# automl/mdp-playground

Measured on AMD Instinct MI355X. Metric: env-steps/sec, higher is better.
Workload: dtype u8; 1 GPU; cfg2: BASELINE configs[1]: discrete 8x8, delay 4, sequence_length 3; 65536 envs/GPU, random actions, same-step autoreset; 1 bench step = 1 fused launch of 512 env steps; envs_per_gpu=65536, fuse=512, env_steps_per_bench_step=33554432, rng=numpy, collective=all_gather_into_tensor(nccl, 1 rank) after every launch

## Files before the change

### mdp_playground_amd/build.py

```python
import os
import subprocess
import sys
from concurrent.futures import ThreadPoolExecutor

HERE = os.path.dirname(os.path.abspath(__file__))
CSRC = os.path.join(HERE, "csrc")
OUT = os.path.join(CSRC, "libmdpp_hip.so")
SOURCES = ["mdpp_capi.hip", "mdpp_discrete.hip", "mdpp_discrete_wide.hip", "mdpp_discrete_long.hip", "mdpp_discrete_fast.hip", "mdpp_discrete_step1.hip", "mdpp_discrete_pipe.hip", "mdpp_discrete_lean.hip", "mdpp_discrete_lean_next.hip", "mdpp_discrete_lean_noise.hip", "mdpp_discrete_lean_npnoise.hip",
           "mdpp_discrete_quiet.hip", "mdpp_discrete_quiet_nu.hip", "mdpp_discrete_policy.hip", "mdpp_discrete_learn.hip",
           "mdpp_discrete_learn_pe.hip", "mdpp_discrete_learn_double.hip", "mdpp_discrete_learn_double_pe.hip",
           "mdpp_discrete_learn_summary.hip", "mdpp_discrete_learn_pe_summary.hip", "mdpp_discrete_learn_double_summary.hip",
           "mdpp_discrete_learn_double_pe_summary.hip", "mdpp_discrete_eval.hip", "mdpp_discrete_eval_summary.hip",
           "mdpp_discrete_learn_pe_nlev.hip", "mdpp_discrete_learn_double_pe_nlev.hip", "mdpp_discrete_learn_pe_nlev_summary.hip",
           "mdpp_discrete_learn_double_pe_nlev_summary.hip", "mdpp_discrete_eval_nlev.hip", "mdpp_discrete_eval_nlev_summary.hip",
           "mdpp_discrete_learn_pe_pm.hip", "mdpp_discrete_learn_double_pe_pm.hip", "mdpp_discrete_learn_pe_pm_summary.hip",
           "mdpp_discrete_learn_double_pe_pm_summary.hip", "mdpp_discrete_eval_pm.hip", "mdpp_discrete_eval_pm_summary.hip",
           "mdpp_discrete_learn_pe_pm_nlev.hip", "mdpp_discrete_learn_double_pe_pm_nlev.hip", "mdpp_discrete_learn_pe_pm_nlev_summary.hip",
           "mdpp_discrete_learn_double_pe_pm_nlev_summary.hip", "mdpp_discrete_eval_pm_nlev.hip", "mdpp_discrete_eval_pm_nlev_summary.hip",
           "mdpp_continuous.hip", "mdpp_continuous_line8.hip",
           "mdpp_continuous_fast.hip", "mdpp_continuous_step1.hip", "mdpp_continuous_line.hip", "mdpp_image.hip", "mdpp_grid.hip", "mdpp_imagec.hip", "mdpp_post.hip", "mdpp_peer.hip",
           "mdpp_generate.hip"]
HEADERS = ["mdpp_internal.hpp", "mdpp_rng.hpp", "mdpp_discrete_closed.hpp", "mdpp_pcg64_limbs.inc", "np_ziggurat_tables.inc",
           os.path.join("..", "..", "include", "mdpp.h")]
INCLUDED_SOURCES = {"mdpp_discrete_wide.hip": ["mdpp_discrete.hip"], "mdpp_discrete_long.hip": ["mdpp_discrete.hip"], "mdpp_discrete_lean_next.hip": ["mdpp_discrete_lean.hip"], "mdpp_discrete_lean_noise.hip": ["mdpp_discrete_lean.hip"], "mdpp_discrete_lean_npnoise.hip": ["mdpp_discrete_lean.hip"],
                    "mdpp_continuous_line8.hip": ["mdpp_continuous.hip"], "mdpp_continuous_step1.hip": ["mdpp_continuous_fast.hip"], "mdpp_discrete_quiet_nu.hip": ["mdpp_discrete_quiet.hip"],
                    **{u: ["mdpp_discrete_learn.hpp"] for u in SOURCES if u.startswith("mdpp_discrete_learn")},
                    **{u: ["mdpp_discrete_eval.hpp"] for u in SOURCES if u.startswith("mdpp_discrete_eval")}}
FLAGS = ["--offload-arch=gfx950", "-O3", "-fPIC", "-std=c++17", "-ffp-contract=off",
         "-fno-fast-math", "-Wall", "-Wno-unused-function"]
SPILL_SAFE = ["-mllvm", "-amdgpu-spill-sgpr-to-vgpr=0"]
EXTRA_FLAGS = {s: SPILL_SAFE for s in ("mdpp_continuous.hip", "mdpp_continuous_line8.hip", "mdpp_discrete.hip", "mdpp_discrete_wide.hip",
                                       "mdpp_discrete_long.hip", "mdpp_discrete_quiet.hip", "mdpp_discrete_quiet_nu.hip")}


def _hipcc():
    for c in (os.environ.get("HIPCC"), "/opt/rocm/bin/hipcc", "hipcc"):
        if c and (os.path.isabs(c) and os.path.exists(c) or not os.path.isabs(c)):
            return c
    raise RuntimeError("hipcc not found")


def _stale(target, deps, cmd=None):
    if not os.path.exists(target):
        return True
    t = os.path.getmtime(target)
    if any(os.path.getmtime(d) > t for d in deps):
        return True
    return cmd is not None and _stamp(target) != _cmd_text(cmd)


def _cmd_text(cmd):
    return " ".join(cmd) + "\n"


def _stamp(target):
    try:
        with open(target + ".cmd") as f:
            return f.read()
    except OSError:
        return None


def _write_stamp(target, cmd):
    with open(target + ".cmd", "w") as f:
        f.write(_cmd_text(cmd))


def build(force=False, verbose=False):
    hipcc = _hipcc()
    srcs = [s for s in SOURCES if os.path.exists(os.path.join(CSRC, s))]
    hdrs = [os.path.join(CSRC, h) for h in HEADERS]
    objs, jobs = [], []
    for s in srcs:
        src = os.path.join(CSRC, s)
        obj = os.path.join(CSRC, s.replace(".hip", ".o"))
        objs.append(obj)
        extra = [os.path.join(CSRC, d) for d in INCLUDED_SOURCES.get(s, []) if os.path.exists(os.path.join(CSRC, d))]
        cmd = [hipcc] + FLAGS + EXTRA_FLAGS.get(s, []) + ["-c", src, "-o", obj]
        if force or _stale(obj, [src] + extra + hdrs, cmd):
            jobs.append(cmd)

    def run(cmd):
        if verbose:
            print(" ".join(cmd), flush=True)
        out = cmd[cmd.index("-o") + 1]
        if os.path.exists(out + ".cmd"):
            os.remove(out + ".cmd")
        r = subprocess.run(cmd, stdout=subprocess.PIPE, stderr=subprocess.STDOUT, text=True)
        if r.returncode != 0:
            raise RuntimeError("hipcc failed:\n" + " ".join(cmd) + "\n" + r.stdout)
        _write_stamp(out, cmd)
        return r.stdout

    if jobs:
        heavy = ("mdpp_continuous_fast", "mdpp_discrete_lean", "mdpp_discrete_quiet", "mdpp_grid", "mdpp_continuous.", "mdpp_continuous_step1")
        jobs.sort(key=lambda c: next((k for k, h in enumerate(heavy) if h in c[-3]), len(heavy)))
        with ThreadPoolExecutor(max_workers=max(1, min(len(jobs), (os.cpu_count() or 4) - 1, 7))) as ex:
            for out in ex.map(run, jobs):
                if verbose and out.strip():
                    print(out)
    link = [hipcc, "--offload-arch=gfx950", "-shared", "-o", OUT] + objs
    if jobs or force or _stale(OUT, objs, link):
        run(link)
    return OUT


if __name__ == "__main__":
    print(build(force="--force" in sys.argv, verbose=True))
```

### mdp_playground_amd/csrc/mdpp_capi.hip

```cpp
#include <float.h>
#include <math.h>
#include <stdio.h>
#include <stdlib.h>
#include <string.h>
#include <time.h>

#include <algorithm>
#include <utility>
#include <vector>

#include "mdpp_internal.hpp"
#include "mdpp_rng.hpp"

using namespace mdpp;

static std::string g_create_err;

#define HIPCHK(h, expr)                                                                  \
    do {                                                                                 \
        hipError_t e_ = (expr);                                                          \
        if (e_ != hipSuccess) {                                                          \
            (h)->err = std::string(#expr) + ": " + hipGetErrorString(e_);                \
            return MDPP_EHIP;                                                            \
        }                                                                                \
    } while (0)

static int fail(mdpp_env *h, int code, const std::string &msg) {
    if (h) h->err = msg; else g_create_err = msg;
    return code;
}

static uint32_t align16(uint32_t x) { return (x + 15u) & ~15u; }

static unsigned __int128 pcg_mult_inverse() {
    static unsigned __int128 inv = 0;
    if (inv == 0) {
        const unsigned __int128 m = (((unsigned __int128)0x2360ED051FC65DA4ULL) << 64) | 0x4385DF649FCCF645ULL;
        unsigned __int128 x = m;
        for (int it = 0; it < 7; it++) x *= 2 - m * x;
        inv = x;
    }
    return inv;
}

extern "C" int mdpp_abi_version(void) { return MDPP_ABI_VERSION; }

extern "C" const char *mdpp_last_error(const mdpp_env *h) {
    return h ? h->err.c_str() : g_create_err.c_str();
}

static void free_all(mdpp_env *h) {
    void *ptrs[] = {h->d_P, h->d_rtable, h->d_rbits, h->d_is_term, h->d_init_cdf, h->d_noise_cdf,
                    h->d_state, h->d_ring, h->d_status, h->d_sd, h->d_cur, h->d_meta, h->d_rng_half,
                    h->d_P1, h->d_init_cdf1, h->d_noise_cdf1, h->d_irr_state,
                    h->d_img_tpl, h->d_img_tplp, h->d_img_clsx, h->d_img_clsy, h->d_img_rot, h->d_img_state_out,
                    h->d_img_state_final, h->d_img_rec, h->d_img_ctr, h->d_line_hist, h->d_line_ws, h->d_ring64, h->d_est_cur, h->d_est_last, h->d_tick_off,
                    h->d_img_near, h->d_s1_blob, h->d_imgc_boxes, h->d_hist_hi, h->d_policy_thr, h->d_learn_q, h->d_learn_carry,
                    h->d_learn_alpha, h->d_learn_gamma, h->d_learn_E,
                    h->d_nl_level, h->d_nl_sigma, h->d_nl_cdf, h->d_nl_T, h->d_nl_M};
    for (void *p : ptrs) if (p) (void)hipFree(p);
    for (int s = 0; s < MDPP_NUM_STREAMS; s++) {
        if (h->d_rng_s[s]) (void)hipFree(h->d_rng_s[s]);
        if (h->d_rng_inc[s]) (void)hipFree(h->d_rng_inc[s]);
    }
    if (h->ev0) (void)hipEventDestroy(h->ev0);
    if (h->side_stream) (void)hipStreamDestroy(h->side_stream);
    for (hipEvent_t e : {h->ev_entry, h->ev_side[0], h->ev_side[1], h->ev_render[0], h->ev_render[1]})
        if (e) (void)hipEventDestroy(e);
    if (h->ev1) (void)hipEventDestroy(h->ev1);
}

extern "C" void mdpp_destroy(mdpp_env *h) {
    if (!h) return;
    (void)hipSetDevice(h->device);
    free_all(h);
    delete h;
}

static int alloc_zero(mdpp_env *h, void **p, size_t bytes) {
    if (bytes == 0) bytes = 16;
    HIPCHK(h, hipMalloc(p, bytes));
    HIPCHK(h, hipMemset(*p, 0, bytes));
    return MDPP_OK;
}

extern "C" int mdpp_create(const mdpp_config *cfg, int device, mdpp_env **out) {
    if (!cfg || !out) return fail(nullptr, MDPP_EINVAL, "mdpp_create: null argument");
    if (cfg->abi_version != MDPP_ABI_VERSION)
        return fail(nullptr, MDPP_EINVAL, "mdpp_create: abi_version mismatch");
    if (cfg->num_envs <= 0) return fail(nullptr, MDPP_EINVAL, "mdpp_create: num_envs <= 0");
    if (cfg->delay < 0 || cfg->every_n < 1)
        return fail(nullptr, MDPP_EINVAL, "mdpp_create: need delay >= 0 and reward_every_n_steps >= 1");
    if (cfg->autoreset < MDPP_AUTORESET_DISABLED || cfg->autoreset > MDPP_AUTORESET_NEXT_STEP)
        return fail(nullptr, MDPP_EINVAL, "mdpp_create: unknown autoreset mode");
    hipError_t e = hipSetDevice(device);
    if (e != hipSuccess)
        return fail(nullptr, MDPP_EHIP, std::string("hipSetDevice: ") + hipGetErrorString(e));
    mdpp_env *h = new mdpp_env();
    memset(&h->cfg, 0, sizeof(h->cfg));
    h->cfg = *cfg;
    h->device = device;
    h->tick = 0; h->reset_tick = 0;
    h->opts = 0; h->kname[0] = 0;
    h->d_P = h->d_rtable = h->d_rbits = h->d_is_term = h->d_init_cdf = h->d_noise_cdf = nullptr;
    h->d_state = h->d_ring = h->d_status = h->d_sd = h->d_cur = h->d_meta = h->d_rng_half = nullptr;
    h->d_P1 = h->d_init_cdf1 = h->d_noise_cdf1 = h->d_irr_state = nullptr;
    h->d_line_hist = h->d_line_ws = h->d_ring64 = nullptr;
    h->d_est_cur = h->d_est_last = nullptr; h->est_nk = 0;
    h->irr_ready = false;
    h->line_hist_stale = false;
    h->graph_capture = false;
    h->d_tick_off = nullptr;
    h->d_img_tpl = h->d_img_tplp = h->d_img_clsx = h->d_img_clsy = h->d_img_rot = nullptr;
    h->d_img_near = nullptr;
    h->d_s1_blob = nullptr;
    memset(&h->s1args, 0, sizeof(h->s1args));
    h->d_policy_thr = nullptr; h->policy_seed = 0; h->policy_ready = false;
    h->d_learn_q = h->d_learn_carry = nullptr; h->learn_seed = 0; h->learn_E = 0; h->learn_alpha = h->learn_gamma = 0.0f;
    h->learn_algo = MDPP_LEARN_Q_LEARNING; h->learn_ready = false;
    h->learn_q_tables = 0; h->d_learn_alpha = h->d_learn_gamma = h->d_learn_E = nullptr; h->learn_pe = h->learn_pe_stale = 0;
    h->learn_pm = false;
    h->nl_on = false; h->nl_pm = false; h->nl_levels = 0; h->nl_fill_valid = false; h->nl_fill_alpha = h->nl_fill_gamma = 0.0f; h->nl_fill_E = 0;
    h->d_nl_level = h->d_nl_sigma = h->d_nl_cdf = h->d_nl_T = h->d_nl_M = nullptr;
    h->d_img_state_out = h->d_img_state_final = h->d_img_rec = h->d_img_ctr = nullptr;
    h->d_imgc_boxes = nullptr;
    h->d_hist_hi = nullptr;
    {
        const size_t imgs = (size_t)cfg->num_envs * (cfg->irrelevant ? 2 : 1);
        h->img_chunk = imgs <= 32768 ? 64 : imgs <= 65536 ? 32 : 16;
    }
    h->img_ready = false; h->img_fast_ok = false; h->img_lines_ready = false; h->img_colb = 64;
    for (int r = 0; r < 32; r++) h->imgc_disc_rows[r] = 0;
    h->img_n_radii = h->img_n_cls_x = h->img_n_cls_y = 0;
    for (int s = 0; s < MDPP_NUM_STREAMS; s++) { h->d_rng_s[s] = h->d_rng_inc[s] = nullptr; h->streams_ready[s] = false; }
    h->tables_ready = false;
    h->ev0 = h->ev1 = nullptr;
    h->side_stream = nullptr;
    h->ev_entry = h->ev_side[0] = h->ev_side[1] = h->ev_render[0] = h->ev_render[1] = nullptr;
    const size_t N = (size_t)cfg->num_envs;
    int rc = MDPP_OK;
#define TRY(x) do { rc = (x); if (rc != MDPP_OK) { g_create_err = h->err; free_all(h); delete h; return rc; } } while (0)
#define TRYHIP(x) do { hipError_t e2_ = (x); if (e2_ != hipSuccess) { g_create_err = std::string(#x) + ": " + hipGetErrorString(e2_); free_all(h); delete h; return MDPP_EHIP; } } while (0)
    TRYHIP(hipEventCreate(&h->ev0));
    TRYHIP(hipEventCreate(&h->ev1));
    TRY(alloc_zero(h, &h->d_status, N * sizeof(uint32_t)));
    TRY(alloc_zero(h, &h->d_tick_off, sizeof(uint64_t)));
    if (cfg->episode_stats) {
        h->est_nk = 3 + (cfg->kind == MDPP_KIND_CONTINUOUS ? cfg->D : 0);
        TRY(alloc_zero(h, &h->d_est_cur, (size_t)h->est_nk * N * sizeof(double)));
        TRY(alloc_zero(h, &h->d_est_last, (size_t)(h->est_nk + 1) * N * sizeof(double)));
    }
    if (cfg->rng_mode == MDPP_RNG_NUMPY_PCG64) {
        for (int s = 0; s < MDPP_NUM_STREAMS; s++) {
            if (s == MDPP_STREAM_IMAGE && !(cfg->image && cfg->kind == MDPP_KIND_DISCRETE)) continue;
            if (s == MDPP_STREAM_SPACE_IRR && !(cfg->kind == MDPP_KIND_DISCRETE && cfg->irrelevant)) continue;
            if (s == MDPP_STREAM_ACTION && cfg->kind != MDPP_KIND_GRID) continue;
            TRY(alloc_zero(h, &h->d_rng_s[s], N * 16));
            TRY(alloc_zero(h, &h->d_rng_inc[s], N * 16));
        }
        if (cfg->kind == MDPP_KIND_GRID) TRY(alloc_zero(h, &h->d_rng_half, N * 8));
        if (cfg->image && cfg->kind == MDPP_KIND_DISCRETE) TRY(alloc_zero(h, &h->d_rng_half, N * 8));
    } else if (cfg->rng_mode != MDPP_RNG_PHILOX) {
        g_create_err = "mdpp_create: unknown rng_mode"; free_all(h); delete h; return MDPP_EINVAL;
    }
    if (cfg->image && cfg->kind == MDPP_KIND_DISCRETE) {
        const size_t sub = cfg->irrelevant ? 2 : 1;
        TRY(alloc_zero(h, &h->d_img_state_out, 2 * (size_t)h->img_chunk * N * 4 * sub));
        TRY(alloc_zero(h, &h->d_img_state_final, 2 * (size_t)h->img_chunk * N * 4 * sub));
        TRY(alloc_zero(h, &h->d_img_rec, 2 * 2 * (size_t)h->img_chunk * N * 64 * sub));
        TRY(alloc_zero(h, &h->d_img_ctr, 2 * 2 * 64 * 128));
    }

    if (cfg->image && cfg->kind == MDPP_KIND_DISCRETE && (cfg->img_w < 1 || cfg->img_h < 1 || cfg->img_tpl_size < 1)) {
        g_create_err = "mdpp_create: image observations of a discrete env need img_w, img_h, img_tpl_size >= 1";
        free_all(h); delete h; return MDPP_EUNSUPPORTED;
    }
    if (cfg->image && cfg->kind == MDPP_KIND_CONTINUOUS &&
        ((cfg->D != 2 && cfg->D != 4) || !isfinite(cfg->state_space_max) || cfg->img_w < 1 || cfg->img_h < 1 ||
         cfg->img_r0 < 1 || cfg->img_r0 > 15)) {
        g_create_err = "mdpp_create: ImageContinuous observations need 2 or 4 bounded state dimensions "
                       "and a disc radius of 1..15";
        free_all(h); delete h; return MDPP_EUNSUPPORTED;
    }
    if (cfg->image) {
        {
            int lo = 0, hi = 0;
            TRYHIP(hipDeviceGetStreamPriorityRange(&lo, &hi));
            TRYHIP(hipStreamCreateWithPriority(&h->side_stream, hipStreamNonBlocking, hi));
        }
        for (hipEvent_t *e : {&h->ev_entry, &h->ev_side[0], &h->ev_side[1], &h->ev_render[0], &h->ev_render[1]})
            TRYHIP(hipEventCreateWithFlags(e, hipEventDisableTiming));
    }
    if (cfg->kind == MDPP_KIND_DISCRETE) {
        const bool wide = cfg->S > 255, lng = cfg->L > 7;
        if (cfg->S < 2 || cfg->S > 65535 || cfg->A < 1 || cfg->L < 1 || cfg->L > 15 || ((wide || lng) && cfg->image) || (wide && lng)) {
            g_create_err = "mdpp_create: discrete needs 2 <= S <= 65535, A >= 1, 1 <= L <= 15 (S <= 255 and L <= 7 with image observations; "
                           "not S > 255 together with L > 7)";
            free_all(h); delete h; return MDPP_EUNSUPPORTED;
        }
        if (cfg->has_transition_noise && cfg->S > 8192) {
            g_create_err = "mdpp_create: transition noise needs S <= 8192 (the S x S cdf table)";
            free_all(h); delete h; return MDPP_EUNSUPPORTED;
        }
        if (cfg->num_tables != 1 && cfg->num_tables != cfg->num_envs) {
            g_create_err = "mdpp_create: num_tables must be 1 or num_envs"; free_all(h); delete h; return MDPP_EINVAL;
        }
        const bool rew_sa = cfg->reward_kind == MDPP_REWARD_STATE_ACTION;
        if ((cfg->reward_kind != MDPP_REWARD_SEQUENCES && !rew_sa) || (rew_sa && cfg->unit_rewards)) {
            g_create_err = "mdpp_create: reward_kind must be MDPP_REWARD_SEQUENCES or, with unit_rewards = 0, MDPP_REWARD_STATE_ACTION";
            free_all(h); delete h; return MDPP_EINVAL;
        }
        double nk = rew_sa ? (double)cfg->S * (double)cfg->A : pow((double)cfg->S, (double)cfg->L);
        if (nk > 4.0e9) { g_create_err = "mdpp_create: S^L too large"; free_all(h); delete h; return MDPP_EUNSUPPORTED; }
        if (cfg->unit_rewards && cfg->delay > 32) {
            g_create_err = "mdpp_create: unit_rewards needs delay <= 32"; free_all(h); delete h; return MDPP_EINVAL;
        }
        h->nkeys = (uint32_t)nk;
        h->rbits_stride = (h->nkeys + 7u) / 8u;
        const size_t T = (size_t)cfg->num_tables;
        if (cfg->irrelevant) {
            if (cfg->S_irr < 2 || cfg->S_irr > 255 || cfg->A_irr < 1) {
                g_create_err = "mdpp_create: irrelevant sub-space needs 2 <= S_irr <= 255, A_irr >= 1";
                free_all(h); delete h; return MDPP_EUNSUPPORTED;
            }
            TRY(alloc_zero(h, &h->d_P1, T * cfg->S_irr * cfg->A_irr));
            TRY(alloc_zero(h, &h->d_init_cdf1, T * cfg->S_irr * sizeof(double)));
            if (cfg->has_transition_noise)
                TRY(alloc_zero(h, &h->d_noise_cdf1, (size_t)cfg->S_irr * cfg->S_irr * sizeof(double)));
            TRY(alloc_zero(h, &h->d_irr_state, N * sizeof(uint32_t)));
        }
        TRY(alloc_zero(h, &h->d_P, T * cfg->S * cfg->A * (wide ? 2 : 1)));
        if (wide || lng) {
            TRY(alloc_zero(h, &h->d_hist_hi, N * sizeof(uint64_t)));
            TRYHIP(hipMemset(h->d_hist_hi, 0xFF, N * sizeof(uint64_t)));
        }
        TRY(alloc_zero(h, &h->d_is_term, T * cfg->S));
        TRY(alloc_zero(h, &h->d_init_cdf, T * cfg->S * sizeof(double)));
        if (cfg->unit_rewards) TRY(alloc_zero(h, &h->d_rbits, T * h->rbits_stride));
        else TRY(alloc_zero(h, &h->d_rtable, T * (size_t)h->nkeys * sizeof(double)));
        if (cfg->has_transition_noise) TRY(alloc_zero(h, &h->d_noise_cdf, (size_t)cfg->S * cfg->S * sizeof(double)));
        TRY(alloc_zero(h, &h->d_state, N * sizeof(uint4)));
        if (!cfg->unit_rewards && cfg->delay > 0) {
            TRY(alloc_zero(h, &h->d_ring, (size_t)cfg->delay * N * sizeof(uint32_t)));
            TRYHIP(hipMemset(h->d_ring, 0xFF, (size_t)cfg->delay * N * sizeof(uint32_t)));
        }
        DiscreteArgs &a = h->dargs;
        memset(&a, 0, sizeof(a));
        a.N = cfg->num_envs; a.S = cfg->S; a.A = cfg->A; a.L = cfg->L; a.delay = cfg->delay;
        a.every_n = cfg->every_n; a.shared_tables = (cfg->num_tables == 1); a.unit_rewards = cfg->unit_rewards;
        a.rew_sa = rew_sa ? 1 : 0;
        a.has_p_noise = cfg->has_transition_noise; a.has_r_noise = cfg->has_reward_noise;
        a.pn_T = cfg->has_transition_noise ? philox_pnoise_threshold(cfg->transition_noise) : 0u;
        a.pn_M = philox_pnoise_magic(a.pn_T, (uint32_t)cfg->S);
        a.pn_M1 = cfg->irrelevant ? philox_pnoise_magic(a.pn_T, (uint32_t)cfg->S_irr) : 0ull;
        a.autoreset = cfg->autoreset; a.max_steps = cfg->max_episode_steps;
        a.obs_i32 = (cfg->obs_dtype == MDPP_OBS_I32 || cfg->image);
        a.philox = (cfg->rng_mode == MDPP_RNG_PHILOX);
        a.nkeys = h->nkeys; a.philox_seed = cfg->philox_seed; a.env_id_offset = cfg->env_id_offset;
        a.r_noise = cfg->reward_noise; a.scale = cfg->reward_scale; a.shift = cfg->reward_shift;
        a.term_add = cfg->term_state_reward * cfg->reward_scale;
        a.P = (const uint8_t *)h->d_P; a.rtable = (const double *)h->d_rtable;
        a.rbits = (const uint8_t *)h->d_rbits; a.is_term = (const uint8_t *)h->d_is_term;
        a.init_cdf = (const double *)h->d_init_cdf; a.noise_cdf = (const double *)h->d_noise_cdf;
        a.rbits_stride = h->rbits_stride;
        uint32_t off = 0;
        a.lds_P = off; off = align16(off + cfg->S * cfg->A);
        a.lds_term = off; off = align16(off + cfg->S);
        a.lds_init = off; off = align16(off + cfg->S * 8);
// ... 27 lines not shown
            g_create_err = "mdpp_create: move_along_a_line needs 1 <= L <= 64 and no image observations";
            free_all(h); delete h; return MDPP_EUNSUPPORTED;
        }
        const size_t D = (size_t)cfg->D;
        if (cfg->target_f64) {
            bool all_rel = !line && cfg->n_rel == cfg->D && cfg->D < 16;
            for (int j = 0; all_rel && j < cfg->n_rel; j++) all_rel = cfg->rel_idx[j] == j && cfg->target[j] == 0.0f;
            if (!all_rel) {
                g_create_err = "mdpp_create: target_f64 (the default target_point) needs move_to_a_point, every dimension relevant, state_space_dim < 16";
                free_all(h); delete h; return MDPP_EUNSUPPORTED;
            }
        }
        const bool rew64 = line || (cfg->target_f64 && cfg->make_denser);
        const bool line_big = line && (cfg->n_rel > 8 || (cfg->n_rel > 4 && cfg->D > 12));
        const size_t line_nl = line_big ? (size_t)cfg->n_rel : cfg->n_rel > 4 ? 8 : 4;
        if (line) TRY(alloc_zero(h, &h->d_line_hist, (size_t)cfg->L * line_nl * N * sizeof(float)));
        if (line_big) TRY(alloc_zero(h, &h->d_line_ws, (size_t)(2 * cfg->n_rel * cfg->n_rel + 3 * cfg->n_rel) * N * sizeof(double)));
        if (rew64 && cfg->delay > 0) TRY(alloc_zero(h, &h->d_ring64, (size_t)cfg->delay * N * sizeof(double)));
        TRY(alloc_zero(h, &h->d_sd, (size_t)(cfg->order + 1) * D * N * sizeof(float)));
        TRY(alloc_zero(h, &h->d_cur, D * N * sizeof(float)));
        TRY(alloc_zero(h, &h->d_meta, N * sizeof(uint2)));
        if (cfg->delay > 0) {
            std::vector<uint32_t> init((size_t)cfg->delay * N, kRingPyZero);
            TRY(alloc_zero(h, &h->d_ring, init.size() * sizeof(uint32_t)));
            TRYHIP(hipMemcpy(h->d_ring, init.data(), init.size() * sizeof(uint32_t), hipMemcpyHostToDevice));
        }
        ContinuousArgs &a = h->cargs;
        memset(&a, 0, sizeof(a));
        a.N = cfg->num_envs; a.D = cfg->D; a.n_rel = cfg->n_rel; a.order = cfg->order;
        a.delay = cfg->delay; a.every_n = cfg->every_n; a.make_denser = cfg->make_denser;
        a.has_p_noise = cfg->has_p_noise; a.has_r_noise = cfg->has_reward_noise;
        a.bounded = isfinite(cfg->state_space_max) ? 1 : 0;
        a.autoreset = cfg->autoreset; a.max_steps = cfg->max_episode_steps;
        a.philox = (cfg->rng_mode == MDPP_RNG_PHILOX); a.n_boxes = cfg->n_boxes;
        a.philox_seed = cfg->philox_seed; a.env_id_offset = cfg->env_id_offset;
        a.inertia32 = (float)cfg->inertia; a.amax32 = (float)cfg->action_space_max;
        a.smax32 = (float)cfg->state_space_max; a.radius32 = (float)cfg->target_radius;
        a.alw32 = (float)cfg->action_loss_weight;
        a.scale = cfg->reward_scale; a.shift = cfg->reward_shift;
        a.term_add = cfg->term_state_reward * cfg->reward_scale;
        a.scale32 = (float)a.scale; a.shift32 = (float)a.shift; a.term_add32 = (float)a.term_add;
        double f = 1.0;
        for (int k = 1; k <= cfg->order; k++) {
            f *= (double)k; a.fact[k] = f;
            a.tpow32[k] = (float)pow(cfg->time_unit, (double)k);
        }
        a.p_noise = cfg->p_noise; a.r_noise = cfg->reward_noise;
        a.reset_lo = (double)(-a.smax32); a.reset_range = (double)a.smax32 - (double)(-a.smax32);
        a.rel_prefix = 1;
        for (int j = 0; j < cfg->n_rel; j++) {
            if (cfg->rel_idx[j] < 0 || cfg->rel_idx[j] >= cfg->D) {
                g_create_err = "mdpp_create: relevant index out of range"; free_all(h); delete h; return MDPP_EINVAL;
            }
            a.rel[j] = cfg->rel_idx[j]; a.target[j] = cfg->target[j];
            if (cfg->rel_idx[j] != j) a.rel_prefix = 0;
        }
        for (int b = 0; b < cfg->n_boxes * cfg->n_rel; b++) { a.box_lo[b] = cfg->box_lo[b]; a.box_hi[b] = cfg->box_hi[b]; }
        {
            auto is_pow2 = [](double v) { int e; return v > 0 && isfinite(v) && frexp(v, &e) == 0.5; };
            a.inertia_pow2 = is_pow2((double)a.inertia32) ? 1u : 0u;
            a.inv_inertia32 = 1.0f / a.inertia32;
            a.fact_pow2_mask = 0;
            for (int k = 1; k <= cfg->order; k++) {
                a.inv_fact[k] = 1.0 / a.fact[k];
                if (is_pow2(a.fact[k])) a.fact_pow2_mask |= 1u << k;
            }
            const bool next_ok = cfg->autoreset != MDPP_AUTORESET_NEXT_STEP || cfg->rng_mode != MDPP_RNG_NUMPY_PCG64 ||
                                 (!cfg->has_p_noise && !cfg->has_reward_noise);
            const bool pen_ok = a.alw32 != 0.0f || a.amax32 <= 1.0e18f;
            a.fast_ok = (a.rel_prefix && !cfg->image && !line && !cfg->target_f64 && next_ok && cfg->n_boxes <= MDPP_MAX_BOXES && pen_ok &&
                         (a.bounded || isfinite(cfg->action_space_max))) ? 1u : 0u;
            a.image_quirk = cfg->image ? 1 : 0;
        }
        if (cfg->image) {
            TRY(alloc_zero(h, &h->d_img_state_out, 2 * (size_t)h->img_chunk * N * D * sizeof(float)));
            {
                std::vector<float> bx((size_t)(cfg->n_boxes > 0 ? cfg->n_boxes : 1) * 4, 0.0f);
                for (int b = 0; b < cfg->n_boxes; b++)
                    for (int d = 0; d < 2 && d < cfg->n_rel; d++) {
                        bx[4 * b + d] = cfg->box_lo[b * cfg->n_rel + d];
                        bx[4 * b + 2 + d] = cfg->box_hi[b * cfg->n_rel + d];
                    }
                TRY(alloc_zero(h, &h->d_imgc_boxes, bx.size() * sizeof(float)));
                TRYHIP(hipMemcpy(h->d_imgc_boxes, bx.data(), bx.size() * sizeof(float), hipMemcpyHostToDevice));
            }
            TRY(alloc_zero(h, &h->d_img_state_final, 2 * (size_t)h->img_chunk * N * D * sizeof(float)));
        }
        a.sd = (float *)h->d_sd; a.cur = (float *)h->d_cur; a.meta = (uint2 *)h->d_meta;
        a.ring = (uint32_t *)h->d_ring;
        a.line_L = line ? cfg->L : 0; a.line_NL = (int32_t)line_nl; a.line_hist = (float *)h->d_line_hist; a.line_ws = (double *)h->d_line_ws; a.ring64 = (double *)h->d_ring64;
        a.target64 = cfg->target_f64 ? 1 : 0; a.rew64 = rew64 ? 1 : 0; a.radius = cfg->target_radius;
        a.est = mdpp::EpisodeStatsDev{(double *)h->d_est_cur, (double *)h->d_est_last, h->est_nk};
        if (cfg->episode_stats) a.fast_ok = 0;
        a.env_s = (ulonglong2 *)h->d_rng_s[MDPP_STREAM_ENV]; a.env_inc = (ulonglong2 *)h->d_rng_inc[MDPP_STREAM_ENV];
        a.sp_s = (ulonglong2 *)h->d_rng_s[MDPP_STREAM_SPACE]; a.sp_inc = (ulonglong2 *)h->d_rng_inc[MDPP_STREAM_SPACE];
        a.status = (uint32_t *)h->d_status;
        h->tables_ready = true;
    } else if (cfg->kind == MDPP_KIND_GRID) {
        bool ok = (cfg->grid_dims == 2 || cfg->grid_dims == 4) && cfg->delay == 0;
        for (int d = 0; ok && d < cfg->grid_dims; d++) ok = cfg->grid_shape[d] >= 1 && cfg->grid_shape[d] <= 254;
        if (ok && cfg->image)
            ok = cfg->img_w >= 1 && cfg->img_h >= 1 &&
                 cfg->img_r0 >= 1 && cfg->img_r0 <= 15 && cfg->n_boxes >= 0 && cfg->n_boxes <= (MDPP_MAX_BOXES * MDPP_MAX_DIM) / 2;
        if (!ok) {
            g_create_err = "mdpp_create: grid needs 2 (or 4) dimensions of 1..254 cells and delay 0; with image "
                           "observations also a disc radius of 1..15 and <= 128 terminal cells";
            free_all(h); delete h; return MDPP_EUNSUPPORTED;
        }
        TRY(alloc_zero(h, &h->d_state, N * sizeof(uint4)));
        if (cfg->image) {
            TRY(alloc_zero(h, &h->d_img_state_out, 2 * (size_t)h->img_chunk * N * cfg->grid_dims * 4));
            {
                std::vector<float> bx((size_t)(cfg->n_boxes > 0 ? cfg->n_boxes : 1) * 4, 0.0f);
                for (int b = 0; b < cfg->n_boxes; b++) { bx[4 * b] = cfg->box_lo[2 * b]; bx[4 * b + 1] = cfg->box_lo[2 * b + 1]; }
                TRY(alloc_zero(h, &h->d_imgc_boxes, bx.size() * sizeof(float)));
                TRYHIP(hipMemcpy(h->d_imgc_boxes, bx.data(), bx.size() * sizeof(float), hipMemcpyHostToDevice));
            }
            TRY(alloc_zero(h, &h->d_img_state_final, 2 * (size_t)h->img_chunk * N * cfg->grid_dims * 4));
            TRY(alloc_zero(h, &h->d_img_tpl, (((size_t)(cfg->grid_dims / 2) * cfg->img_w * cfg->img_h + 15) / 16) * 2));
        }
        GridArgs &a = h->gargs;
        memset(&a, 0, sizeof(a));
        a.N = cfg->num_envs; a.G = cfg->grid_dims;
        for (int d = 0; d < cfg->grid_dims; d++) a.shape[d] = cfg->grid_shape[d];
        a.target[0] = cfg->grid_target[0]; a.target[1] = cfg->grid_target[1];
        a.make_denser = cfg->make_denser; a.has_p_noise = cfg->has_transition_noise;
        a.has_r_noise = cfg->has_reward_noise; a.every_n = cfg->every_n;
        a.autoreset = cfg->autoreset; a.max_steps = cfg->max_episode_steps;
        a.obs_i32 = (cfg->obs_dtype == MDPP_OBS_I32 || cfg->image);
        a.philox = (cfg->rng_mode == MDPP_RNG_PHILOX);
        a.philox_seed = cfg->philox_seed; a.env_id_offset = cfg->env_id_offset;
        a.p_noise = cfg->transition_noise; a.r_noise = cfg->reward_noise;
        a.scale = cfg->reward_scale; a.shift = cfg->reward_shift;
        a.term_add = cfg->term_state_reward * cfg->reward_scale;
        a.state = (uint4 *)h->d_state;
        a.env_s = (ulonglong2 *)h->d_rng_s[MDPP_STREAM_ENV]; a.env_inc = (ulonglong2 *)h->d_rng_inc[MDPP_STREAM_ENV];
        a.sp_s = (ulonglong2 *)h->d_rng_s[MDPP_STREAM_SPACE]; a.sp_inc = (ulonglong2 *)h->d_rng_inc[MDPP_STREAM_SPACE];
        a.act_s = (ulonglong2 *)h->d_rng_s[MDPP_STREAM_ACTION]; a.act_inc = (ulonglong2 *)h->d_rng_inc[MDPP_STREAM_ACTION];
        a.act_half = (uint2 *)h->d_rng_half;
        a.status = (uint32_t *)h->d_status;
        a.est = mdpp::EpisodeStatsDev{(double *)h->d_est_cur, (double *)h->d_est_last, h->est_nk};
        a.minv_lo = (uint64_t)pcg_mult_inverse(); a.minv_hi = (uint64_t)(pcg_mult_inverse() >> 64);
        h->tables_ready = true;
    } else {
        g_create_err = "mdpp_create: unknown kind"; free_all(h); delete h; return MDPP_EINVAL;
    }
#undef TRY
#undef TRYHIP
    *out = h;
    return MDPP_OK;
}

static inline bool t_fits53(uint64_t t) { return t <= (1ULL << 53) - 1; }

static int discrete_derived(mdpp_env *h, const uint8_t *P, const double *rtable, const uint8_t *rbits,
                            const uint8_t *is_term, const double *init_cdf, const double *noise_cdf) {
    const size_t T = (size_t)h->cfg.num_tables, S = (size_t)h->cfg.S, A = (size_t)h->cfg.A;
    const bool wide = S > 255;
    if (wide || h->cfg.L > 7) {
        DiscreteArgs &a = h->dargs;
        a.shape_ok = a.fast_ok = a.shape_ok_irr = a.lean_next_ok = a.shape_ok_noise = a.shape_ok_noise_np = 0u;
        a.minv_lo = (uint64_t)pcg_mult_inverse(); a.minv_hi = (uint64_t)(pcg_mult_inverse() >> 64);
        memset(&h->s1args, 0, sizeof(h->s1args));
        h->tables_ready = true;
        return MDPP_OK;
    }
    {
        DiscreteArgs &a = h->dargs;
        const mdpp_config &c = h->cfg;
        a.shape_ok = (T == 1 && c.unit_rewards && !c.has_transition_noise && !c.has_reward_noise &&
                      c.L <= 3 && c.S <= 16 && c.delay <= 32 && c.autoreset != MDPP_AUTORESET_NEXT_STEP &&
                      a.rew_in_lds && !c.irrelevant) ? 1u : 0u;
        a.fast_ok = (a.shape_ok && c.rng_mode == MDPP_RNG_NUMPY_PCG64) ? 1u : 0u;
        a.shape_ok_irr = (T == 1 && c.unit_rewards && !c.has_transition_noise && !c.has_reward_noise &&
                          c.L <= 3 && c.S <= 8 && c.delay <= 32 && c.autoreset != MDPP_AUTORESET_NEXT_STEP &&
                          a.rew_in_lds && c.irrelevant && !c.image) ? 1u : 0u;
        a.lean_next_ok = (T == 1 && c.unit_rewards && !c.has_transition_noise && !c.has_reward_noise &&
                          c.L <= 3 && c.S <= 8 && c.delay <= 32 && c.autoreset == MDPP_AUTORESET_NEXT_STEP &&
                          a.rew_in_lds && !c.image) ? 1u : 0u;
        a.shape_ok_noise = (T == 1 && c.unit_rewards && (c.has_transition_noise || c.has_reward_noise) &&
                            c.rng_mode == MDPP_RNG_PHILOX && c.L <= 3 && c.S <= 8 && c.S >= 2 && c.delay <= 32 &&
                            c.autoreset != MDPP_AUTORESET_NEXT_STEP && a.rew_in_lds && !c.irrelevant && !c.image) ? 1u : 0u;
        a.shape_ok_noise_np = (T == 1 && c.unit_rewards && (c.has_transition_noise || c.has_reward_noise) &&
                               c.rng_mode == MDPP_RNG_NUMPY_PCG64 && c.L <= 3 && c.S <= 8 && c.S >= 2 && c.delay <= 32 &&
                               c.autoreset != MDPP_AUTORESET_NEXT_STEP && a.rew_in_lds && !c.irrelevant && !c.image) ? 1u : 0u;
        for (int j = 0; j < 8; j++) a.pn_TL[j] = a.pn_TU[j] = ~0ULL;
        if (a.shape_ok_noise_np && c.has_transition_noise) {
            bool same = true;
            for (size_t j = 0; j < S; j++) {
                uint64_t tl = 0, tu = 0;
                bool hl = false, hu = false;
                for (size_t n = 0; n < S; n++) {
                    const uint64_t t = (uint64_t)ceil(ldexp(noise_cdf[n * S + j], 53));
                    if (n > j) { if (hl && tl != t) same = false; tl = t; hl = true; }
                    else { if (hu && tu != t) same = false; tu = t; hu = true; }
                }
                if (t_fits53(tl) && hl) a.pn_TL[j] = tl << 11;
                if (hu) a.pn_TU[j] = tu > (1ULL << 53) - 1 ? ~0ULL : tu << 11;
            }
            if (!same) a.shape_ok_noise_np = 0u;
        }
        if (c.episode_stats) a.shape_ok = a.fast_ok = a.shape_ok_irr = a.lean_next_ok = a.shape_ok_noise = a.shape_ok_noise_np = 0u;
        a.s_shift = 0xFFFFFFFFu;
        for (uint32_t b = 1; b < 8; b++) if ((1u << b) == (uint32_t)c.S) a.s_shift = b;
        a.key_mask = h->nkeys - 1u;
        a.spow = 1; for (int j = 0; j < c.L - 1; j++) a.spow *= (uint32_t)c.S;
        a.term_mask = 0;
        if (c.S <= 64) for (size_t s = 0; s < S; s++) if (is_term[s]) a.term_mask |= 1ULL << s;
        for (int j = 0; j < 16; j++) a.init_thr[j] = ~0ULL;
        if (c.S <= 16)
            for (size_t j = 0; j < S; j++) a.init_thr[j] = (uint64_t)ceil(ldexp(init_cdf[j], 53));
        a.minv_lo = (uint64_t)pcg_mult_inverse(); a.minv_hi = (uint64_t)(pcg_mult_inverse() >> 64);
        for (int q = 0; q < 4; q++) {
            double r = (q & 2) ? 1.0 : 0.0;
            r *= a.scale; r += a.shift;
            if (q & 1) r += a.term_add;
            a.rsel[q] = (float)r;
        }
        Step1Args &s1 = h->s1args;
        memset(&s1, 0, sizeof(s1));
        const bool rew_sa_ = c.reward_kind == MDPP_REWARD_STATE_ACTION;
        if (a.shape_ok && c.every_n < (1 << 20)) {
            std::vector<uint32_t> blob(256, 0u);
            for (size_t act = 0; act < A && act < 16; act++) {
                uint64_t col = 0;
                for (size_t st = 0; st < S; st++) col |= (uint64_t)(P[st * A + act] & 0xF) << (4 * st);
                blob[2 * act] = (uint32_t)col; blob[2 * act + 1] = (uint32_t)(col >> 32);
            }
            for (int j = 0; j < 16; j++) { blob[32 + 2 * j] = (uint32_t)a.init_thr[j]; blob[32 + 2 * j + 1] = (uint32_t)(a.init_thr[j] >> 32); }
            for (uint32_t b = 0; b < h->rbits_stride && b < 512; b++) blob[64 + b / 4] |= (uint32_t)rbits[b] << (8 * (b % 4));
            for (size_t j = 0; j < 16; j++) {
                const double t = j < S ? ceil(ldexp(init_cdf[j], 31)) : 4294967295.0;
                blob[192 + j] = t >= 4294967295.0 ? 4294967295u : (uint32_t)t;
            }
            if (h->d_s1_blob) { (void)hipFree(h->d_s1_blob); h->d_s1_blob = nullptr; }
            HIPCHK(h, hipMalloc(&h->d_s1_blob, (size_t)kS1Replicas * 1024));
            for (int r = 0; r < kS1Replicas; r++)
                HIPCHK(h, hipMemcpy((char *)h->d_s1_blob + (size_t)r * 1024, blob.data(), 1024, hipMemcpyHostToDevice));
            s1.N = c.num_envs; s1.A = (uint32_t)c.A; s1.S = (uint32_t)c.S; s1.L = (uint32_t)c.L;
            s1.every_n = (uint32_t)c.every_n; s1.inv_every_n = 1.0 / (double)c.every_n;
            s1.max_steps = c.max_episode_steps > 0 ? (uint32_t)c.max_episode_steps : 0u;
            s1.delay = (uint32_t)c.delay; s1.autoreset = c.autoreset != MDPP_AUTORESET_DISABLED ? 1u : 0u;
            s1.term32 = (uint32_t)a.term_mask; s1.nan_mask = 0xFFu << (8 * c.L);
            s1.topup_rounds = 1; s1.topup_fill = 6;
            s1.philox_seed = a.philox_seed; s1.env_id_offset = a.env_id_offset;
            for (int q = 0; q < 4; q++) s1.rsel[q] = a.rsel[q];
            s1.blob = (const uint4 *)h->d_s1_blob;
            s1.state = a.state; s1.env_s = a.env_s; s1.env_inc = a.env_inc; s1.status = a.status;
        } else if (T == 1 && (c.unit_rewards ? c.delay <= 32 : (!rew_sa_ && !c.has_transition_noise && !c.has_reward_noise)) && c.L <= 3 &&
                   c.autoreset != MDPP_AUTORESET_NEXT_STEP && !c.irrelevant && !c.episode_stats && c.every_n < (1 << 20)) {
            const uint32_t S8 = ((uint32_t)S + 7u) & ~7u;
            const uint32_t off_term = align16((uint32_t)(S * A)), off_thr = align16(off_term + (uint32_t)S);
            const uint32_t off_thr31 = off_thr + S8 * 8u, off_rew = align16(off_thr31 + S8 * 4u);
            const uint32_t rew_bytes = c.unit_rewards ? h->rbits_stride : h->nkeys * 8u;
            const uint32_t off_bk = align16(off_rew + rew_bytes);
            const bool np_streams = c.rng_mode == MDPP_RNG_NUMPY_PCG64;
            const uint32_t off_tn = off_bk + 512u;
            const uint32_t off_zig = off_tn + ((c.has_transition_noise && np_streams) ? (uint32_t)S * S8 * 8u : 0u);
            const uint32_t bytes = (off_zig + ((c.has_reward_noise && np_streams) ? 6144u : 0u) + 1023u) & ~1023u;
            const uint32_t max_rounds = (c.has_transition_noise || c.has_reward_noise) ? kS1wRoundsNoise : kS1wRounds;
            if (bytes <= max_rounds * 1024u) {
                std::vector<uint8_t> blob(bytes, 0);
                memcpy(blob.data(), P, S * A);
                memcpy(blob.data() + off_term, is_term, S);
                for (uint32_t j = 0; j < S8; j++) {
                    const uint64_t t64 = j < S ? (uint64_t)ceil(ldexp(init_cdf[j], 53)) : ~0ULL;
                    const double t31 = j < S ? ceil(ldexp(init_cdf[j], 31)) : 4294967295.0;
                    const uint32_t t32 = t31 >= 4294967295.0 ? 4294967295u : (uint32_t)t31;
                    memcpy(blob.data() + off_thr + 8u * j, &t64, 8);
                    memcpy(blob.data() + off_thr31 + 4u * j, &t32, 4);
                }
                if (c.unit_rewards) memcpy(blob.data() + off_rew, rbits, h->rbits_stride);
                else memcpy(blob.data() + off_rew, rtable, (size_t)h->nkeys * 8u);
                {
                    const bool ph = c.rng_mode == MDPP_RNG_PHILOX;
                    const int shift = ph ? 23 : 45;
                    for (uint32_t b = 0; b < 256u; b++) {
                        const uint64_t lo = (uint64_t)b << shift, hi = lo + (1ULL << shift);
                        uint32_t c0 = 0, nin = 0;
                        for (uint32_t j = 0; j < S; j++) {
                            uint64_t t;
                            if (ph) { uint32_t t32; memcpy(&t32, blob.data() + off_thr31 + 4u * j, 4); t = t32; }
                            else memcpy(&t, blob.data() + off_thr + 8u * j, 8);
                            c0 += t <= lo ? 1u : 0u;
                            nin += (t > lo && t < hi) ? 1u : 0u;
                        }
                        const uint16_t e = (uint16_t)(c0 | (nin << 8));
                        memcpy(blob.data() + off_bk + 2u * b, &e, 2);
                    }
                }
                if (c.has_transition_noise && np_streams)
                    for (uint32_t row = 0; row < S; row++)
                        for (uint32_t j = 0; j < S8; j++) {
                            const uint64_t t64 = j < S ? (uint64_t)ceil(ldexp(noise_cdf[row * S + j], 53)) : ~0ULL;
                            memcpy(blob.data() + off_tn + 8u * (row * S8 + j), &t64, 8);
                        }
                if (c.has_reward_noise && np_streams) {
                    static const uint64_t ki[256] = NPZ_KI_INIT;
                    static const double wi[256] = NPZ_WI_INIT, fi[256] = NPZ_FI_INIT;
                    memcpy(blob.data() + off_zig, ki, 2048); memcpy(blob.data() + off_zig + 2048, wi, 2048);
                    memcpy(blob.data() + off_zig + 4096, fi, 2048);
                }
                if (h->d_s1_blob) { (void)hipFree(h->d_s1_blob); h->d_s1_blob = nullptr; }
                HIPCHK(h, hipMalloc(&h->d_s1_blob, (size_t)kS1Replicas * bytes));
                for (int r = 0; r < kS1Replicas; r++)
                    HIPCHK(h, hipMemcpy((char *)h->d_s1_blob + (size_t)r * bytes, blob.data(), bytes, hipMemcpyHostToDevice));
                s1.N = c.num_envs; s1.A = (uint32_t)c.A; s1.S = (uint32_t)c.S; s1.L = (uint32_t)c.L;
                s1.every_n = (uint32_t)c.every_n; s1.inv_every_n = 1.0 / (double)c.every_n;
                s1.max_steps = c.max_episode_steps > 0 ? (uint32_t)c.max_episode_steps : 0u;
                s1.delay = (uint32_t)c.delay; s1.autoreset = c.autoreset != MDPP_AUTORESET_DISABLED ? 1u : 0u;
                s1.nan_mask = 0xFFu << (8 * c.L);
                s1.philox_seed = a.philox_seed; s1.env_id_offset = a.env_id_offset;
                for (int q = 0; q < 4; q++) s1.rsel[q] = a.rsel[q];
                s1.blob = (const uint4 *)h->d_s1_blob;
                s1.wide = 1; s1.blob_rounds = bytes / 1024u; s1.off_term = off_term; s1.off_thr = off_thr; s1.off_thr31 = off_thr31;
                s1.off_rew = off_rew; s1.S8 = S8; s1.off_bk = off_bk;
                s1.has_p_noise = c.has_transition_noise ? 1u : 0u; s1.has_r_noise = c.has_reward_noise ? 1u : 0u;
                s1.off_tn = off_tn; s1.off_zig = off_zig; s1.pn_T = a.pn_T; s1.pn_M = a.pn_M; s1.r_noise = a.r_noise;
                s1.sp_s = a.sp_s; s1.sp_inc = a.sp_inc;
                s1.unit = c.unit_rewards ? 1u : 0u; s1.ring_keys = a.ring_keys;
                s1.scale = a.scale; s1.shift = a.shift; s1.term_add = a.term_add;
                s1.state = a.state; s1.env_s = a.env_s; s1.env_inc = a.env_inc; s1.status = a.status;
            }
        }
    }
    h->tables_ready = true;
    return MDPP_OK;
}

extern "C" int mdpp_upload_discrete_tables(mdpp_env *h, const uint8_t *P, const double *rtable,
                                           const uint8_t *rbits, const uint8_t *is_term,
                                           const double *init_cdf, const double *noise_cdf) {
    if (!h) return MDPP_EINVAL;
    if (h->cfg.kind != MDPP_KIND_DISCRETE) return fail(h, MDPP_EINVAL, "upload_discrete_tables: not a discrete handle");
    if (!P || !is_term || !init_cdf) return fail(h, MDPP_EINVAL, "upload_discrete_tables: null table");
    if (h->cfg.unit_rewards ? !rbits : !rtable) return fail(h, MDPP_EINVAL, "upload_discrete_tables: reward table missing");
    if (h->cfg.has_transition_noise && !noise_cdf) return fail(h, MDPP_EINVAL, "upload_discrete_tables: noise_cdf missing");
    HIPCHK(h, hipSetDevice(h->device));
    const size_t T = (size_t)h->cfg.num_tables, S = (size_t)h->cfg.S, A = (size_t)h->cfg.A;
    const bool wide = S > 255;
    for (size_t k = 0; k < T * S * A; k++)
        if ((wide ? (size_t)((const uint16_t *)P)[k] : (size_t)P[k]) >= S) return fail(h, MDPP_EINVAL, "upload_discrete_tables: P entry out of range");
    HIPCHK(h, hipMemcpy(h->d_P, P, T * S * A * (wide ? 2 : 1), hipMemcpyHostToDevice));
    HIPCHK(h, hipMemcpy(h->d_is_term, is_term, T * S, hipMemcpyHostToDevice));
    HIPCHK(h, hipMemcpy(h->d_init_cdf, init_cdf, T * S * sizeof(double), hipMemcpyHostToDevice));
    if (h->cfg.unit_rewards)
        HIPCHK(h, hipMemcpy(h->d_rbits, rbits, T * h->rbits_stride, hipMemcpyHostToDevice));
    else
        HIPCHK(h, hipMemcpy(h->d_rtable, rtable, T * (size_t)h->nkeys * sizeof(double), hipMemcpyHostToDevice));
    if (h->cfg.has_transition_noise)
        HIPCHK(h, hipMemcpy(h->d_noise_cdf, noise_cdf, S * S * sizeof(double), hipMemcpyHostToDevice));
    return discrete_derived(h, P, rtable, rbits, is_term, init_cdf, noise_cdf);
}

struct DevTemp {
    std::vector<void *> ptrs;
    ~DevTemp() { for (void *p : ptrs) (void)hipFree(p); }
    hipError_t alloc(void **p, size_t bytes) {
        hipError_t e = hipMalloc(p, bytes ? bytes : 16);
        if (e == hipSuccess) ptrs.push_back(*p);
        return e;
    }
};

extern "C" int mdpp_generate_discrete(mdpp_env *h, const uint64_t *seeds, const mdpp_gen_params *p,
                                      const uint8_t *is_term, const double *init_cdf, const double *noise_cdf) {
    if (!h) return MDPP_EINVAL;
    const mdpp_config &c = h->cfg;
    if (c.kind != MDPP_KIND_DISCRETE) return fail(h, MDPP_EINVAL, "generate_discrete: not a discrete handle");
    if (!seeds || !p || !is_term || !init_cdf) return fail(h, MDPP_EINVAL, "generate_discrete: null argument");
    if (c.has_transition_noise && !noise_cdf) return fail(h, MDPP_EINVAL, "generate_discrete: noise_cdf missing");
    if (c.num_tables != c.num_envs || c.irrelevant || c.S > 255 || c.reward_kind != MDPP_REWARD_SEQUENCES)
        return fail(h, MDPP_EUNSUPPORTED, "generate_discrete: needs one table per env, no irrelevant sub-space, S <= 255 and "
                                          "rewardable sequences");
    GenArgs a;
    const char *err = nullptr;
    const int prc = gen_args_init(p, c.S, c.A, c.L, c.image != 0, c.unit_rewards != 0, h->nkeys, h->rbits_stride, a, &err);
    if (prc != MDPP_OK) return fail(h, prc, err);
    const size_t per_env = (size_t)a.scratch_words * 8u;
    HIPCHK(h, hipSetDevice(h->device));
    const size_t N = (size_t)c.num_envs, S = (size_t)c.S, A = (size_t)c.A;
    const int chunk = (int)std::min(N, std::max<size_t>(1, kGenScratchCap / std::max<size_t>(per_env, 8)));
    DevTemp tmp;
    uint64_t *d_seeds = nullptr, *d_sd = nullptr, *d_scr = nullptr;
    double *d_rews = nullptr;
    HIPCHK(h, tmp.alloc((void **)&d_seeds, N * 8));
    HIPCHK(h, hipMemcpy(d_seeds, seeds, N * 8, hipMemcpyHostToDevice));
    if (p->rews) {
        HIPCHK(h, tmp.alloc((void **)&d_rews, (size_t)p->n_rews * 8));
        HIPCHK(h, hipMemcpy(d_rews, p->rews, (size_t)p->n_rews * 8, hipMemcpyHostToDevice));
    }
    if (p->seed_dicts) HIPCHK(h, tmp.alloc((void **)&d_sd, N * 64));
    HIPCHK(h, tmp.alloc((void **)&d_scr, (size_t)chunk * per_env));
    HIPCHK(h, hipMemset(h->d_P, 0, N * S * A));
    if (c.unit_rewards) HIPCHK(h, hipMemset(h->d_rbits, 0, N * h->rbits_stride));
    else HIPCHK(h, hipMemset(h->d_rtable, 0, N * (size_t)h->nkeys * sizeof(double)));
    a.rews = d_rews;
    a.seeds = d_seeds; a.P = (uint8_t *)h->d_P; a.rbits = (uint8_t *)h->d_rbits; a.rtable = (double *)h->d_rtable;
    a.sd = d_sd;
    if (c.rng_mode == MDPP_RNG_NUMPY_PCG64) {
        a.env_s = (ulonglong2 *)h->d_rng_s[MDPP_STREAM_ENV]; a.env_inc = (ulonglong2 *)h->d_rng_inc[MDPP_STREAM_ENV];
        a.sp_s = (ulonglong2 *)h->d_rng_s[MDPP_STREAM_SPACE]; a.sp_inc = (ulonglong2 *)h->d_rng_inc[MDPP_STREAM_SPACE];
        if (c.image) {
            a.im_s = (ulonglong2 *)h->d_rng_s[MDPP_STREAM_IMAGE]; a.im_inc = (ulonglong2 *)h->d_rng_inc[MDPP_STREAM_IMAGE];
            a.im_half = (uint2 *)h->d_rng_half;
        }
    }
    a.scratch = d_scr;
    for (size_t first = 0; first < N; first += (size_t)chunk)
        HIPCHK(h, launch_generate_discrete(a, (int)first, (int)std::min((size_t)chunk, N - first)));
    HIPCHK(h, hipDeviceSynchronize());
    if (p->seed_dicts) HIPCHK(h, hipMemcpy(p->seed_dicts, d_sd, N * 64, hipMemcpyDeviceToHost));
    {
        std::vector<uint8_t> term(N * S);
        std::vector<double> cdf(N * S);
        for (size_t i = 0; i < N; i++) {
            memcpy(term.data() + i * S, is_term, S);
            memcpy(cdf.data() + i * S, init_cdf, S * sizeof(double));
        }
        HIPCHK(h, hipMemcpy(h->d_is_term, term.data(), N * S, hipMemcpyHostToDevice));
        HIPCHK(h, hipMemcpy(h->d_init_cdf, cdf.data(), N * S * sizeof(double), hipMemcpyHostToDevice));
    }
    if (c.has_transition_noise)
        HIPCHK(h, hipMemcpy(h->d_noise_cdf, noise_cdf, S * S * sizeof(double), hipMemcpyHostToDevice));
    int rc;
    if (N == 1) {
        std::vector<uint8_t> P(S * A), rbits(c.unit_rewards ? h->rbits_stride : 0);
        std::vector<double> rtable(c.unit_rewards ? 0 : h->nkeys);
        HIPCHK(h, hipMemcpy(P.data(), h->d_P, S * A, hipMemcpyDeviceToHost));
        if (c.unit_rewards) HIPCHK(h, hipMemcpy(rbits.data(), h->d_rbits, h->rbits_stride, hipMemcpyDeviceToHost));
        else HIPCHK(h, hipMemcpy(rtable.data(), h->d_rtable, (size_t)h->nkeys * sizeof(double), hipMemcpyDeviceToHost));
        rc = discrete_derived(h, P.data(), c.unit_rewards ? nullptr : rtable.data(), c.unit_rewards ? rbits.data() : nullptr,
                              is_term, init_cdf, noise_cdf);
    } else {
        rc = discrete_derived(h, nullptr, nullptr, nullptr, is_term, init_cdf, noise_cdf);
    }
    if (rc != MDPP_OK) return rc;
    if (c.rng_mode == MDPP_RNG_NUMPY_PCG64) {
        if (h->dargs.fast_ok)
            HIPCHK(h, hipMemset2D((char *)h->d_state + 4, 16, 0, 4, N));
        h->streams_ready[MDPP_STREAM_ENV] = h->streams_ready[MDPP_STREAM_SPACE] = true;
        if (c.image) h->streams_ready[MDPP_STREAM_IMAGE] = true;
    }
    return MDPP_OK;
}

extern "C" int mdpp_get_discrete_tables(mdpp_env *h, uint8_t *P, double *rtable, uint8_t *rbits, uint8_t *is_term,
                                        double *init_cdf) {
    if (!h) return MDPP_EINVAL;
    if (h->cfg.kind != MDPP_KIND_DISCRETE) return fail(h, MDPP_EINVAL, "get_discrete_tables: not a discrete handle");
    if (!h->tables_ready) return fail(h, MDPP_ESTATE, "get_discrete_tables: tables not uploaded");
    if ((rtable && !h->d_rtable) || (rbits && !h->d_rbits))
        return fail(h, MDPP_EINVAL, "get_discrete_tables: this handle keeps the other reward table (unit_rewards)");
    HIPCHK(h, hipSetDevice(h->device));
    HIPCHK(h, hipDeviceSynchronize());
    const size_t T = (size_t)h->cfg.num_tables, S = (size_t)h->cfg.S, A = (size_t)h->cfg.A;
    if (P) HIPCHK(h, hipMemcpy(P, h->d_P, T * S * A * (S > 255 ? 2 : 1), hipMemcpyDeviceToHost));
    if (rtable) HIPCHK(h, hipMemcpy(rtable, h->d_rtable, T * (size_t)h->nkeys * sizeof(double), hipMemcpyDeviceToHost));
    if (rbits) HIPCHK(h, hipMemcpy(rbits, h->d_rbits, T * h->rbits_stride, hipMemcpyDeviceToHost));
    if (is_term) HIPCHK(h, hipMemcpy(is_term, h->d_is_term, T * S, hipMemcpyDeviceToHost));
    if (init_cdf) HIPCHK(h, hipMemcpy(init_cdf, h->d_init_cdf, T * S * sizeof(double), hipMemcpyDeviceToHost));
    return MDPP_OK;
}

extern "C" int mdpp_seed_streams_seedseq(mdpp_env *h, int stream, const uint64_t *seeds) {
    if (!h || !seeds) return MDPP_EINVAL;
    if (h->cfg.rng_mode != MDPP_RNG_NUMPY_PCG64) return fail(h, MDPP_ESTATE, "seed_streams_seedseq: handle is in Philox mode");
    if (stream < 0 || stream >= MDPP_NUM_STREAMS || !h->d_rng_s[stream]) return fail(h, MDPP_EINVAL, "seed_streams_seedseq: bad stream");
    HIPCHK(h, hipSetDevice(h->device));
    const size_t N = (size_t)h->cfg.num_envs;
    DevTemp tmp;
    uint64_t *d_seeds = nullptr;
    HIPCHK(h, tmp.alloc((void **)&d_seeds, N * 8));
    HIPCHK(h, hipMemcpy(d_seeds, seeds, N * 8, hipMemcpyHostToDevice));
    const bool half = (stream == MDPP_STREAM_IMAGE || stream == MDPP_STREAM_ACTION) && h->d_rng_half;
    HIPCHK(h, hipDeviceSynchronize());
    HIPCHK(h, launch_seed_streams_seedseq(d_seeds, (int)N, h->d_rng_s[stream], h->d_rng_inc[stream], half ? h->d_rng_half : nullptr));
    if (stream == MDPP_STREAM_ENV && h->cfg.kind == MDPP_KIND_DISCRETE && h->dargs.fast_ok)
        HIPCHK(h, hipMemset2D((char *)h->d_state + 4, 16, 0, 4, N));
    HIPCHK(h, hipDeviceSynchronize());
    h->streams_ready[stream] = true;
    return MDPP_OK;
}

extern "C" int mdpp_upload_discrete_irrelevant(mdpp_env *h, const uint8_t *P1, const double *init_cdf1,
                                               const double *noise_cdf1) {
    if (!h) return MDPP_EINVAL;
    if (h->cfg.kind != MDPP_KIND_DISCRETE || !h->cfg.irrelevant)
        return fail(h, MDPP_EINVAL, "upload_discrete_irrelevant: not a handle with an irrelevant sub-space");
    if (!P1 || !init_cdf1) return fail(h, MDPP_EINVAL, "upload_discrete_irrelevant: null table");
    if (h->cfg.has_transition_noise && !noise_cdf1) return fail(h, MDPP_EINVAL, "upload_discrete_irrelevant: noise_cdf missing");
    HIPCHK(h, hipSetDevice(h->device));
    const size_t T = (size_t)h->cfg.num_tables, S1 = (size_t)h->cfg.S_irr, A1 = (size_t)h->cfg.A_irr;
    for (size_t k = 0; k < T * S1 * A1; k++)
        if (P1[k] >= S1) return fail(h, MDPP_EINVAL, "upload_discrete_irrelevant: P entry out of range");
    HIPCHK(h, hipMemcpy(h->d_P1, P1, T * S1 * A1, hipMemcpyHostToDevice));
    HIPCHK(h, hipMemcpy(h->d_init_cdf1, init_cdf1, T * S1 * sizeof(double), hipMemcpyHostToDevice));
    if (h->cfg.has_transition_noise)
        HIPCHK(h, hipMemcpy(h->d_noise_cdf1, noise_cdf1, S1 * S1 * sizeof(double), hipMemcpyHostToDevice));
    h->irr_ready = true;
    return MDPP_OK;
}

extern "C" int mdpp_upload_image_disc(mdpp_env *h, const uint8_t *disc) {
    if (!h || !disc) return MDPP_EINVAL;
    if ((h->cfg.kind != MDPP_KIND_CONTINUOUS && h->cfg.kind != MDPP_KIND_GRID) || !h->cfg.image)
        return fail(h, MDPP_EINVAL, "upload_image_disc: not a continuous / grid handle with image observations");
    const int T = 2 * h->cfg.img_r0 + 1;
    for (int r = 0; r < 32; r++) h->imgc_disc_rows[r] = 0;
    for (int dy = 0; dy < T; dy++)
        for (int dx = 0; dx < T; dx++)
            if (disc[dy * T + dx]) h->imgc_disc_rows[dy] |= 1u << dx;
    h->img_ready = h->cfg.kind == MDPP_KIND_CONTINUOUS || h->img_lines_ready;
    return MDPP_OK;
}

extern "C" int mdpp_upload_image_lines(mdpp_env *h, const uint8_t *lines) {
    if (!h || !lines) return MDPP_EINVAL;
    if (h->cfg.kind != MDPP_KIND_GRID || !h->cfg.image)
        return fail(h, MDPP_EINVAL, "upload_image_lines: not a grid handle with image observations");
    const size_t npix = (size_t)(h->cfg.grid_dims / 2) * h->cfg.img_w * h->cfg.img_h;
    std::vector<uint16_t> bits((npix + 15) / 16, 0);
    for (size_t p = 0; p < npix; p++)
        if (lines[p]) bits[p >> 4] |= (uint16_t)(1u << (p & 15));
    HIPCHK(h, hipSetDevice(h->device));
    HIPCHK(h, hipMemcpy(h->d_img_tpl, bits.data(), bits.size() * 2, hipMemcpyHostToDevice));
    h->img_lines_ready = true;
    bool disc = false;
    for (int r = 0; r < 32; r++) disc = disc || h->imgc_disc_rows[r] != 0;
    h->img_ready = disc;
    return MDPP_OK;
}

extern "C" int mdpp_get_state_grid(mdpp_env *h, int32_t *cells, int32_t *steps, uint8_t *reached) {
    if (!h || !cells || !steps || !reached) return MDPP_EINVAL;
    if (h->cfg.kind != MDPP_KIND_GRID) return fail(h, MDPP_EINVAL, "get_state_grid: not a grid handle");
    HIPCHK(h, hipSetDevice(h->device));
    HIPCHK(h, hipDeviceSynchronize());
    const size_t N = (size_t)h->cfg.num_envs;
    const int G = h->cfg.grid_dims;
    std::vector<uint32_t> st(4 * N);
    HIPCHK(h, hipMemcpy(st.data(), h->d_state, N * 16, hipMemcpyDeviceToHost));
    for (size_t i = 0; i < N; i++) {
        for (int d = 0; d < G; d++) cells[i * G + d] = (int32_t)((st[4 * i] >> (8 * d)) & 0xFF);
        steps[i] = (int32_t)st[4 * i + 1];
        reached[i] = (uint8_t)(st[4 * i + 2] & 1u);
    }
    return MDPP_OK;
}

extern "C" int mdpp_set_state_grid(mdpp_env *h, const int32_t *cells, const int32_t *steps, const uint8_t *reached) {
    if (!h || !cells || !steps) return MDPP_EINVAL;
    if (h->cfg.kind != MDPP_KIND_GRID) return fail(h, MDPP_EINVAL, "set_state_grid: not a grid handle");
    const size_t N = (size_t)h->cfg.num_envs;
    const int G = h->cfg.grid_dims;
    std::vector<uint32_t> st(4 * N, 0);
    for (size_t i = 0; i < N; i++) {
        for (int d = 0; d < G; d++) {
            if (cells[i * G + d] < 0 || cells[i * G + d] > h->cfg.grid_shape[d])
                return fail(h, MDPP_EINVAL, "set_state_grid: cell out of range");
            st[4 * i] |= (uint32_t)cells[i * G + d] << (8 * d);
        }
        st[4 * i + 1] = (uint32_t)steps[i];
        st[4 * i + 2] = reached ? (uint32_t)(reached[i] & 1u) : 0u;
    }
    HIPCHK(h, hipSetDevice(h->device));
    HIPCHK(h, hipDeviceSynchronize());
    HIPCHK(h, hipMemcpy(h->d_state, st.data(), N * 16, hipMemcpyHostToDevice));
    return MDPP_OK;
}

extern "C" int mdpp_get_state_irrelevant(mdpp_env *h, int32_t *irr) {
    if (!h || !irr) return MDPP_EINVAL;
    if (h->cfg.kind != MDPP_KIND_DISCRETE || !h->cfg.irrelevant) return fail(h, MDPP_EINVAL, "get_state_irrelevant: no irrelevant sub-space");
    HIPCHK(h, hipSetDevice(h->device));
    HIPCHK(h, hipDeviceSynchronize());
    HIPCHK(h, hipMemcpy(irr, h->d_irr_state, (size_t)h->cfg.num_envs * 4, hipMemcpyDeviceToHost));
    return MDPP_OK;
}

extern "C" int mdpp_set_state_irrelevant(mdpp_env *h, const int32_t *irr) {
    if (!h || !irr) return MDPP_EINVAL;
    if (h->cfg.kind != MDPP_KIND_DISCRETE || !h->cfg.irrelevant) return fail(h, MDPP_EINVAL, "set_state_irrelevant: no irrelevant sub-space");
    for (int i = 0; i < h->cfg.num_envs; i++)
        if (irr[i] < 0 || irr[i] >= h->cfg.S_irr) return fail(h, MDPP_EINVAL, "set_state_irrelevant: state out of range");
    HIPCHK(h, hipSetDevice(h->device));
    HIPCHK(h, hipDeviceSynchronize());
    HIPCHK(h, hipMemcpy(h->d_irr_state, irr, (size_t)h->cfg.num_envs * 4, hipMemcpyHostToDevice));
    return MDPP_OK;
}

extern "C" int mdpp_seed_streams(mdpp_env *h, int stream, const uint64_t *words) {
    if (!h || !words) return MDPP_EINVAL;
    if (h->cfg.rng_mode != MDPP_RNG_NUMPY_PCG64) return fail(h, MDPP_ESTATE, "seed_streams: handle is in Philox mode");
    if (stream < 0 || stream >= MDPP_NUM_STREAMS || !h->d_rng_s[stream]) return fail(h, MDPP_EINVAL, "seed_streams: bad stream");
    HIPCHK(h, hipSetDevice(h->device));
    const size_t N = (size_t)h->cfg.num_envs;
    std::vector<uint64_t> st(2 * N), inc(2 * N);
    std::vector<uint32_t> half(2 * N);
    for (size_t i = 0; i < N; i++) {
        st[2 * i] = words[6 * i]; st[2 * i + 1] = words[6 * i + 1];
        inc[2 * i] = words[6 * i + 2]; inc[2 * i + 1] = words[6 * i + 3];
        half[2 * i] = (uint32_t)words[6 * i + 4]; half[2 * i + 1] = (uint32_t)words[6 * i + 5];
    }
    HIPCHK(h, hipMemcpy(h->d_rng_s[stream], st.data(), N * 16, hipMemcpyHostToDevice));
    HIPCHK(h, hipMemcpy(h->d_rng_inc[stream], inc.data(), N * 16, hipMemcpyHostToDevice));
    if ((stream == MDPP_STREAM_IMAGE || stream == MDPP_STREAM_ACTION) && h->d_rng_half)
        HIPCHK(h, hipMemcpy(h->d_rng_half, half.data(), N * 8, hipMemcpyHostToDevice));
    if (stream == MDPP_STREAM_ENV && h->cfg.kind == MDPP_KIND_DISCRETE && h->dargs.fast_ok) {
        HIPCHK(h, hipDeviceSynchronize());
        HIPCHK(h, hipMemset2D((char *)h->d_state + 4, 16, 0, 4, N));
    }
    h->streams_ready[stream] = true;
    return MDPP_OK;
}

extern "C" int mdpp_get_streams(mdpp_env *h, int stream, uint64_t *words) {
    if (!h || !words) return MDPP_EINVAL;
    if (h->cfg.rng_mode != MDPP_RNG_NUMPY_PCG64) return fail(h, MDPP_ESTATE, "get_streams: handle is in Philox mode");
    if (stream < 0 || stream >= MDPP_NUM_STREAMS || !h->d_rng_s[stream]) return fail(h, MDPP_EINVAL, "get_streams: bad stream");
    HIPCHK(h, hipSetDevice(h->device));
    HIPCHK(h, hipDeviceSynchronize());
    const size_t N = (size_t)h->cfg.num_envs;
    std::vector<uint64_t> st(2 * N), inc(2 * N);
    std::vector<uint32_t> half(2 * N, 0);
    HIPCHK(h, hipMemcpy(st.data(), h->d_rng_s[stream], N * 16, hipMemcpyDeviceToHost));
    HIPCHK(h, hipMemcpy(inc.data(), h->d_rng_inc[stream], N * 16, hipMemcpyDeviceToHost));
    if ((stream == MDPP_STREAM_IMAGE || stream == MDPP_STREAM_ACTION) && h->d_rng_half)
        HIPCHK(h, hipMemcpy(half.data(), h->d_rng_half, N * 8, hipMemcpyDeviceToHost));
    std::vector<uint32_t> rec;
    const bool queued = stream == MDPP_STREAM_ENV && h->cfg.kind == MDPP_KIND_DISCRETE && h->dargs.fast_ok;
    if (queued) {
        rec.resize(4 * N);
        HIPCHK(h, hipMemcpy(rec.data(), h->d_state, N * 16, hipMemcpyDeviceToHost));
    }
    for (size_t i = 0; i < N; i++) {
        unsigned __int128 s = ((unsigned __int128)st[2 * i + 1] << 64) | st[2 * i];
        const unsigned __int128 c = ((unsigned __int128)inc[2 * i + 1] << 64) | inc[2 * i];
        if (queued)
            for (uint32_t q = (rec[4 * i + 1] >> 24) & 7u; q > 0; q--) s = (s - c) * pcg_mult_inverse();
        words[6 * i] = (uint64_t)s; words[6 * i + 1] = (uint64_t)(s >> 64);
        words[6 * i + 2] = inc[2 * i]; words[6 * i + 3] = inc[2 * i + 1];
        words[6 * i + 4] = half[2 * i]; words[6 * i + 5] = half[2 * i + 1];
    }
    return MDPP_OK;
}

extern "C" int mdpp_set_options(mdpp_env *h, uint32_t disable_mask) {
    if (!h) return MDPP_EINVAL;
    h->opts = disable_mask;
    return MDPP_OK;
}

extern "C" int mdpp_get_episode_stats(mdpp_env *h, double *current, double *last) {
// ... 1148 lines not shown
```

### mdp_playground_amd/csrc/mdpp_discrete_lean.hip

```cpp
#include <stdlib.h>

#include <stdio.h>

#include <type_traits>

#ifndef MDPP_LEAN_TU_NEXT
#define MDPP_LEAN_TU_NEXT 0
#endif
#ifndef MDPP_LEAN_TU_NOISE
#define MDPP_LEAN_TU_NOISE 0
#endif

#include "mdpp_internal.hpp"
#include "mdpp_rng.hpp"

namespace mdpp {

#ifndef MDPP_LEAN_CHUNK
#define MDPP_LEAN_CHUNK 8
#endif
#ifndef MDPP_LEAN_DEPTH
#define MDPP_LEAN_DEPTH 32
#endif
#ifndef MDPP_LEAN_AHEAD
#define MDPP_LEAN_AHEAD 4
#endif
#if defined(MDPP_LEAN_PRIO_E) || defined(MDPP_LEAN_PRIO_O) || defined(MDPP_LEAN_PRIO_H)
#define MDPP_LEAN_PRIO_FORCED 1
#else
#define MDPP_LEAN_PRIO_FORCED 0
#endif
#ifndef MDPP_LEAN_PRIO_E
#define MDPP_LEAN_PRIO_E 3
#endif
#ifndef MDPP_LEAN_PRIO_O
#define MDPP_LEAN_PRIO_O 2
#endif
#ifndef MDPP_LEAN_PRIO_H
#define MDPP_LEAN_PRIO_H 0
#endif
#ifndef MDPP_LEAN_PRIO_O2
#define MDPP_LEAN_PRIO_O2 -1
#endif
#ifndef MDPP_LEAN_ST_AUX
#define MDPP_LEAN_ST_AUX MDPP_ST_NT
#endif
#ifndef MDPP_LEAN_ST_AUX_BYTES
#define MDPP_LEAN_ST_AUX_BYTES MDPP_LEAN_ST_AUX
#endif
#ifndef MDPP_LEAN_LD_AUX
#define MDPP_LEAN_LD_AUX 0
#endif
#ifndef MDPP_LEAN_HMIN
#define MDPP_LEAN_HMIN 16
#endif
#ifndef MDPP_LEAN_HSLEEP
#define MDPP_LEAN_HSLEEP 8
#endif
namespace lean {
constexpr int kChunk = MDPP_LEAN_CHUNK;
constexpr int kDepth = MDPP_LEAN_DEPTH;
constexpr int kAhead = MDPP_LEAN_AHEAD;
constexpr int kPRsrc = 0x00020000;
constexpr uint32_t kSpinLimit = 1u << 22;
constexpr uint32_t kStatusInternal = 0x80000000u;
constexpr uint32_t kQueueCap = 6;
constexpr int kHChunks = 8;
constexpr int kHChunksNp = 4;
constexpr int kXR = 16;
constexpr int kXB = 4;
constexpr int kDepthNp = 16;
constexpr int kRoles = 4;
constexpr uint32_t kSelPad = 0x0c0c0c00u;
typedef unsigned int u32x2 __attribute__((ext_vector_type(2)));
typedef unsigned int u32x4 __attribute__((ext_vector_type(4)));

__device__ __forceinline__ uint32_t wg_load_acq(const uint32_t *p) {
    return __hip_atomic_load(p, __ATOMIC_ACQUIRE, __HIP_MEMORY_SCOPE_WORKGROUP);
}
__device__ __forceinline__ void wg_store_rel(uint32_t *p, uint32_t v) {
    __hip_atomic_store(p, v, __ATOMIC_RELEASE, __HIP_MEMORY_SCOPE_WORKGROUP);
}
__device__ __forceinline__ void chunk_words(uint64_t seed, uint64_t genv, uint64_t b0, uint32_t r4, uint32_t stream,
                                            uint32_t (&wd)[MDPP_LEAN_CHUNK]) {
    uint32_t o0[4], o1[4], o2[4] = {0u, 0u, 0u, 0u};
    philox_start_block(seed, genv, b0, stream, o0);
    philox_start_block(seed, genv, b0 + 1, stream, o1);
    if (r4 != 0u) philox_start_block(seed, genv, b0 + 2, stream, o2);
    const uint32_t all[12] = {o0[0], o0[1], o0[2], o0[3], o1[0], o1[1], o1[2], o1[3], o2[0], o2[1], o2[2], o2[3]};
#pragma unroll
    for (int u = 0; u < MDPP_LEAN_CHUNK; u++)
        wd[u] = r4 == 0u ? all[u] : r4 == 1u ? all[u + 1] : r4 == 2u ? all[u + 2] : all[u + 3];
}
__device__ __forceinline__ void chunk_normals(uint64_t seed, uint64_t genv, uint64_t b0, uint32_t r4, uint32_t stream,
                                              float (&z)[MDPP_LEAN_CHUNK]) {
    float all[12] = {0.0f, 0.0f, 0.0f, 0.0f, 0.0f, 0.0f, 0.0f, 0.0f, 0.0f, 0.0f, 0.0f, 0.0f};
    uint32_t o[4];
    philox_start_block(seed, genv, b0, stream, o);
    philox_box_muller2(o, all[0], all[1], all[2], all[3]);
    philox_start_block(seed, genv, b0 + 1, stream, o);
    philox_box_muller2(o, all[4], all[5], all[6], all[7]);
    if (r4 != 0u) {
        philox_start_block(seed, genv, b0 + 2, stream, o);
        philox_box_muller2(o, all[8], all[9], all[10], all[11]);
    }
#pragma unroll
    for (int u = 0; u < MDPP_LEAN_CHUNK; u++)
        z[u] = r4 == 0u ? all[u] : r4 == 1u ? all[u + 1] : r4 == 2u ? all[u + 2] : all[u + 3];
}
}
using namespace lean;

template <bool OBS64, bool DELAY, bool HASMAX, bool EVN, bool PHILOX, bool IRR, bool NEXT, int NZ = 0>
__global__ __launch_bounds__(kRoles * kBlock) void k_discrete_rollout_lean(DiscreteArgs a, int K,
                                                                      const int32_t *__restrict__ actions,
                                                                      void *__restrict__ obs,
                                                                      float *__restrict__ reward,
                                                                      uint8_t *__restrict__ term,
                                                                      uint8_t *__restrict__ trunc,
                                                                      void *__restrict__ final_obs) {
    const uint64_t ptick0 = tick_now(a);
    constexpr bool PN = (NZ & 1) != 0, RN = (NZ & 2) != 0;
    constexpr bool NPN = PN && !PHILOX, NRN = RN && !PHILOX;
    constexpr bool Z0 = (NZ & 4) != 0;
    static_assert(!Z0 || NRN, "sigma-0 draws: numpy streams with the reward_noise key");
    constexpr bool NRX = NRN && !Z0;
    constexpr int KD = NRN ? kDepthNp : kDepth;
    __shared__ __align__(16) uint32_t lds_rec[3][KD][kBlock];
    __shared__ __align__(16) uint32_t lds_V[2048];
    __shared__ __align__(16) uint2 lds_col[16];
    __shared__ __align__(16) uint32_t lds_R[128];
    __shared__ __align__(16) uint64_t lds_T[8];
    __shared__ __align__(16) float lds_rsel[EVN ? 4 * 64 : 4];
    __shared__ __align__(16) uint64_t lds_ring[kBlock];
    __shared__ uint32_t lds_head[kBlock];
    __shared__ uint32_t lds_prod[kBlock / 64];
    __shared__ __align__(8) uint32_t lds_cons[kBlock / 64][2];
    __shared__ uint32_t lds_done;
    constexpr bool ROWS2 = !IRR && NZ == 0;
    constexpr bool ROWS1 = ROWS2 && !PHILOX;
    constexpr int kRB = 4;
    __shared__ __align__(16) float lds_rw[ROWS1 ? kRB : 1][kChunk][ROWS1 ? kBlock : 4];
    __shared__ __align__(16) uint32_t lds_rprod[kBlock / 64], lds_rcons[kBlock / 64];
    typedef typename std::conditional<IRR, uint64_t, uint32_t>::type S0Word;
    __shared__ __align__(16) S0Word lds_s0[PHILOX ? kHChunks : 1][kBlock];
    __shared__ __align__(16) uint2 lds_col1[IRR ? 16 : 1];
    __shared__ __align__(16) uint64_t lds_T1[IRR ? 8 : 1];
    __shared__ uint32_t lds_hprod[kBlock / 64];
    __shared__ uint32_t lds_pprod[kBlock / 64];
    constexpr bool kNpNoise = !PHILOX && NZ != 0;
    constexpr bool kPhNoise = PHILOX && NZ != 0;
    constexpr int kPrioE = MDPP_LEAN_PRIO_FORCED ? MDPP_LEAN_PRIO_E : kNpNoise ? 2 : !PHILOX ? MDPP_LEAN_PRIO_E : 1;
    constexpr int kPrioO = MDPP_LEAN_PRIO_FORCED ? MDPP_LEAN_PRIO_O : kNpNoise ? 1 : !PHILOX ? MDPP_LEAN_PRIO_O : kPhNoise ? 2 : (PN ? 2 : 3);
    constexpr int kPrioH = MDPP_LEAN_PRIO_FORCED ? MDPP_LEAN_PRIO_H : kNpNoise ? 3 : !PHILOX ? MDPP_LEAN_PRIO_H : kPhNoise ? 2 : (PN ? 3 : 2);
    static_assert(NZ == 0 || (!IRR && !NEXT), "noise on the lean kernel: one sub-space, same-step autoreset");
    __shared__ __align__(16) uint32_t lds_pn[(PN && PHILOX) ? kHChunks : 1][kBlock];
    __shared__ __align__(16) uint32_t lds_pn2[NPN ? kHChunksNp : 1][2][kBlock];
    __shared__ __align__(16) double lds_x[NRX ? kXR : 1][kBlock];
    __shared__ uint16_t lds_meta[NRN ? kXR : 1][kBlock];
    __shared__ __align__(16) double lds_rx[NRX ? KD : 1][kBlock];
    __shared__ uint32_t lds_hhead[NRN ? kBlock : 1], lds_epos[NRN ? kBlock : 1];
    __shared__ uint8_t lds_sstab[(NRN || NPN) ? 2048 : 1];
    __shared__ uint8_t lds_pntab[NPN ? 4096 : 1];
    __shared__ ulonglong2 lds_kw[NRN ? 256 : 1];
    __shared__ double lds_fi[NRN ? 256 : 1];
    constexpr int kEN = IRR ? 2 : 1;
    constexpr bool nextmode = NEXT;
    const bool ar = a.autoreset != 0;
    const int tid = threadIdx.x;
    const int role = tid / kBlock;
    const int l = tid & (kBlock - 1);
    const int w = l >> 6;
    const uint32_t S = (uint32_t)a.S, L = (uint32_t)a.L;
    if (tid < 16) {
        uint64_t cs = 0;
        if (tid < a.A)
            for (uint32_t s = 0; s < S; s++) {
                const uint32_t nx = a.P[s * a.A + tid] & 7u;
                cs |= (uint64_t)(nx | 8u | ((uint32_t)((a.term_mask >> nx) & 1ULL) << 7)) << (8 * s);
            }
        lds_col[tid] = make_uint2((uint32_t)cs, (uint32_t)(cs >> 32));
        if (tid < 8) lds_T[tid] = a.init_thr[tid];
        if (IRR) {
            uint64_t c1 = 0;
            if (tid < a.A1)
                for (int s1 = 0; s1 < a.S1; s1++) c1 |= (uint64_t)(a.P1[s1 * a.A1 + tid] & 7u) << (8 * s1);
            lds_col1[tid] = make_uint2((uint32_t)c1, (uint32_t)(c1 >> 32));
            if (tid < 8) lds_T1[tid] = tid < a.S1 ? (uint64_t)ceil(a.init_cdf1[tid] * 9007199254740992.0) : ~0ULL;
        }
        if (!EVN && tid < 4) lds_rsel[tid] = a.rsel[tid];
    }
    if (EVN)
        for (int k = tid; k < 4 * a.every_n; k += kRoles * kBlock) lds_rsel[k] = a.rsel[k < 4 ? k : (k & 1)];
    for (uint32_t k = tid; k < 128; k += kRoles * kBlock) {
        uint32_t wd = 0;
        for (int b = 0; b < 4; b++) {
            uint32_t byte = 4 * k + b;
            if (byte < a.rbits_stride) wd |= (uint32_t)a.rbits[byte] << (8 * b);
        }
        lds_R[k] = wd;
    }
    if (tid < kBlock) { lds_ring[tid] = 0; lds_head[tid] = 0; if (NRN) { lds_hhead[tid] = 0; lds_epos[tid] = 0; } }
    if (NRN || NPN) {
        for (uint32_t k = tid; k < 2048u; k += kRoles * kBlock) {
            const uint64_t lo = (uint64_t)k << 53, hi = lo + ((1ULL << 53) - 1ULL);
            uint32_t c0 = 0, c1 = 0;
            for (int j = 0; j < 8; j++) {
                const uint64_t t = a.init_thr[j] > (1ULL << 53) - 1ULL ? ~0ULL : a.init_thr[j] << 11;
                c0 += (t <= lo) ? 1u : 0u; c1 += (t <= hi) ? 1u : 0u;
            }
            lds_sstab[k] = (uint8_t)(c0 == c1 ? c0 : 0xFFu);
        }
    }
    if (NPN) {
        for (uint32_t k = tid; k < 4096u; k += kRoles * kBlock) {
            const uint64_t lo = (uint64_t)k << 52, hi = lo + ((1ULL << 52) - 1ULL);
            uint32_t a0 = 0, a1 = 0, b0 = 0, b1 = 0;
            for (int j = 0; j < 7; j++) { a0 += (a.pn_TL[j] <= lo) ? 1u : 0u; a1 += (a.pn_TL[j] <= hi) ? 1u : 0u; }
            for (int j = 0; j < 8; j++) { b0 += (a.pn_TU[j] <= lo) ? 1u : 0u; b1 += (a.pn_TU[j] <= hi) ? 1u : 0u; }
            lds_pntab[k] = (uint8_t)((a0 == a1 && b0 == b1) ? (a0 | (b0 << 4)) : 0xFFu);
        }
    }
    if (NRN)
        for (int k = tid; k < 256; k += kRoles * kBlock) { lds_kw[k] = make_ulonglong2(d_zig_ki[k], (unsigned long long)(__double_as_longlong(d_zig_wi[k]) + (52LL << 52)));    lds_fi[k] = d_zig_fi[k]; }
    if (tid < kBlock / 64) { lds_prod[tid] = 0; lds_cons[tid][0] = 0; lds_cons[tid][1] = 0; lds_hprod[tid] = 0; lds_pprod[tid] = 0; lds_rprod[tid] = 0; lds_rcons[tid] = 0; }
    if (tid == 0) lds_done = 0;
    __syncthreads();
    {
        uint32_t dmask = 0;
        for (uint32_t j = 1; j <= L; j++) dmask |= 1u << (4 * j - 2);
        for (uint32_t d = tid; d < 2048; d += kRoles * kBlock) {
            uint32_t wd = 0;
            if ((d & dmask) == dmask) {
                for (uint32_t b = 8; b < 32; b++) {
                    if (!(b & 8u)) continue;
                    const uint32_t idx = d * 32u + b;
                    uint32_t key = 0, pw = 1;
                    for (uint32_t j = 0; j < L; j++) { key += ((idx >> (4 * j)) & 7u) * pw; pw *= S; }
                    if (key < a.nkeys) wd |= ((lds_R[key >> 5] >> (key & 31u)) & 1u) << b;
                }
            }
            lds_V[d] = wd;
        }
    }
    uint32_t steps_at_launch = 0;
    {
        const uint32_t eb0 = ((gridDim.x & 7u) == 0u) ? (blockIdx.x & 7u) * (gridDim.x >> 3) + (blockIdx.x >> 3) : blockIdx.x;
        const uint32_t i0 = eb0 * kBlock + l;
        if (EVN && role == 1 && i0 < (uint32_t)a.N) steps_at_launch = ((const uint32_t *)&a.state[i0])[2] & 0x7FFFFFFFu;
    }
    __syncthreads();

    const uint32_t eblk = ((gridDim.x & 7u) == 0u) ? (blockIdx.x & 7u) * (gridDim.x >> 3) + (blockIdx.x >> 3) : blockIdx.x;
    const uint32_t i = eblk * kBlock + l;
    const uint32_t N = (uint32_t)a.N;
    const bool rows = ROWS2 && (N % (uint32_t)kBlock) == 0u;
    const uint32_t blk0 = eblk * kBlock, ln = (uint32_t)l & 63u;
    const uint32_t ws = (uint32_t)__builtin_amdgcn_readfirstlane(w);
    auto min4 = [&](const uint32_t *p) -> uint32_t {
        const uint64_t x = __hip_atomic_load((const uint64_t *)p, __ATOMIC_ACQUIRE, __HIP_MEMORY_SCOPE_WORKGROUP);
        const uint64_t y = __hip_atomic_load((const uint64_t *)p + 1, __ATOMIC_ACQUIRE, __HIP_MEMORY_SCOPE_WORKGROUP);
        return min(min((uint32_t)x, (uint32_t)(x >> 32)), min((uint32_t)y, (uint32_t)(y >> 32)));
    };
    if (i >= N) {
        if (role == 0 && (l & 63) == 0) __hip_atomic_fetch_add(&lds_done, 1u, __ATOMIC_RELEASE, __HIP_MEMORY_SCOPE_WORKGROUP);
        return;
    }
    const uint32_t A = (uint32_t)a.A;
    constexpr int kMinLanes = MDPP_LEAN_HMIN;
    uint32_t status = 0;

    if (role == 3) {
        if (!ar && !PN && !NRN) return;
        __builtin_amdgcn_s_setprio(kPrioH);
        if constexpr (PHILOX) {
            const uint64_t genv = (uint64_t)(a.env_id_offset + (int64_t)i);
            const int nch = (K + kChunk - 1) / kChunk;
            static_assert(kChunk == 8, "two start-state blocks per chunk");
            uint32_t thr[8], thr1[8];
#pragma unroll
            for (int j = 0; j < 8; j++) {
                const uint64_t t53 = lds_T[j];
                thr[j] = __builtin_amdgcn_readfirstlane(t53 > (1ULL << 53) ? 0x80000000u : (uint32_t)((t53 + 0x3FFFFFULL) >> 22));
                const uint64_t u53 = IRR ? lds_T1[j] : ~0ULL;
                thr1[j] = __builtin_amdgcn_readfirstlane(u53 > (1ULL << 53) ? 0x80000000u : (uint32_t)((u53 + 0x3FFFFFULL) >> 22));
            }
            const uint32_t r4 = (uint32_t)ptick0 & 3u;
            for (int c = 0; c < nch; c++) {
                if (c >= kHChunks) {
                    const uint32_t must = (uint32_t)min((c - kHChunks + 1) * kChunk, K);
                    uint32_t spins = 0;
                    while (wg_load_acq(&lds_prod[w]) < must) {
                        __builtin_amdgcn_s_sleep(2);
                        if (++spins > kSpinLimit) { status |= kStatusInternal; break; }
                    }
                }
                const uint64_t b0 = (ptick0 + (uint64_t)(c * kChunk)) >> 2;
                auto words = [&](uint32_t stream, uint32_t (&wd)[kChunk]) { chunk_words(a.philox_seed, genv, b0, r4, stream, wd); };
                uint32_t wd[kChunk], wd1[kChunk];
                words(kPhiloxStartStream, wd);
                if (IRR) words(kPhiloxStartIrrStream, wd1);
                S0Word pk = 0;
#pragma unroll
                for (int u = 0; u < kChunk; u++) {
                    const uint32_t m = wd[u] >> 1;
                    uint32_t s0 = 0;
#pragma unroll
                    for (int j = 0; j < 7; j++) s0 += (thr[j] <= m) ? 1u : 0u;
                    if (IRR) {
                        const uint32_t m1 = wd1[u] >> 1;
                        uint32_t s1 = 0;
#pragma unroll
                        for (int j = 0; j < 7; j++) s1 += (thr1[j] <= m1) ? 1u : 0u;
                        s0 |= (s1 | 8u) << 4;
                    }
                    pk |= (S0Word)(s0 | 8u) << (kEN * 4 * u);
                }
                lds_s0[c % kHChunks][l] = pk;
                if ((l & 63) == 0) wg_store_rel(&lds_hprod[w], (uint32_t)(c + 1));
            }
            if (status) atomicOr(&a.status[i], status);
            return;
        }
        if constexpr (NPN || NRN) {
            Pcg64 g;
            g.load(a.env_s, a.env_inc, i);
            Pcg64LimbsLo ge;
            ge.from(g);
            uint32_t hq = 0;
            uint64_t look = 0;
            if (NRN) look = ge.next64();
            uint32_t vals = 0, tail = 0, spins = 0;
            auto start_of = [&](uint64_t r) __attribute__((always_inline)) -> uint32_t {
                uint32_t s0 = lds_sstab[(uint32_t)(r >> 53)];
                if (__builtin_expect(__builtin_amdgcn_ballot_w64(s0 == 0xFFu) != 0, 0)) {
                    if (s0 == 0xFFu) {
                        const uint64_t m = r >> 11;
                        s0 = 0;
#pragma unroll
                        for (int j = 0; j < 8; j++) s0 += (a.init_thr[j] <= m) ? 1u : 0u;
                    }
                }
                return s0;
            };
            for (;;) {
                if (wg_load_acq(&lds_done) == kBlock / 64) break;
                bool did = false;
                if constexpr (NRN) {
                    const uint32_t epos = __hip_atomic_load(&lds_epos[l], __ATOMIC_RELAXED, __HIP_MEMORY_SCOPE_WORKGROUP);
                    const bool go = hq + (uint32_t)kXB <= epos + (uint32_t)kXR;
                    if (__builtin_amdgcn_ballot_w64(go) != 0) {
                        uint32_t rej = 0;
                        uint64_t wdv[kXB + 1];
                        if (go) {
                            wdv[0] = look;
#pragma unroll
                            for (int u = 0; u < kXB; u++) {
                                const uint64_t wd = wdv[u];
                                wdv[u + 1] = ge.next64();
                                const uint64_t rabs = (wd >> 9) & 0x000fffffffffffffULL;
                                if constexpr (Z0) {
                                    const uint64_t ki = lds_kw[(uint32_t)wd & 0xffu].x;
                                    const bool ok = rabs < ki;
                                    rej |= ok ? 0u : (1u << u);
                                    lds_meta[(hq + (uint32_t)u) & (uint32_t)(kXR - 1)][l] = (uint16_t)(start_of(wd) | (ok ? 0u : (2u << 3)));
                                    continue;
                                }
                                const ulonglong2 kw = lds_kw[(uint32_t)wd & 0xffu];
                                const double W = __longlong_as_double((long long)kw.y);
                                const double x = __builtin_fma(__longlong_as_double((long long)(rabs | 0x3FF0000000000000ULL)), W, -W);
                                const uint64_t xb = (uint64_t)__double_as_longlong(x);
                                const double xs = __longlong_as_double((long long)(((uint64_t)(((uint32_t)(xb >> 32) & 0x7FFFFFFFu) |
                                                                                   (((uint32_t)wd << 23) & 0x80000000u)) << 32) | (uint32_t)xb));
                                const bool ok = rabs < kw.x;
                                rej |= ok ? 0u : (1u << u);
                                const uint32_t slot = (hq + (uint32_t)u) & (uint32_t)(kXR - 1);
                                lds_x[slot][l] = xs;
                                lds_meta[slot][l] = (uint16_t)(start_of(wd) | (ok ? 0u : (2u << 3)));
                            }
                            look = wdv[kXB];
                        }
                        while (__builtin_amdgcn_ballot_w64(rej != 0u) != 0) {
                            if (rej != 0u) {
                                const uint32_t j = (uint32_t)__builtin_ctz(rej);
                                rej &= rej - 1u;
                                uint64_t wd = 0, wn = 0;
#pragma unroll
                                for (int u = 0; u < kXB; u++)
                                    if (j == (uint32_t)u) { wd = wdv[u]; wn = wdv[u + 1]; }
                                const uint32_t idx = (uint32_t)wd & 0xffu;
                                const uint32_t slot = (hq + j) & (uint32_t)(kXR - 1);
                                const uint32_t ss = lds_meta[slot][l] & 7u;
                                if (__builtin_expect(idx == 0u, 0)) {
                                    const double nor_r = 3.6541528853610087963519472518, nor_inv_r = 0.27366123732975827203338247596;
                                    Pcg64LimbsLo t = ge;
                                    uint32_t have = (uint32_t)kXB - j, cnt = 1u;
                                    auto word = [&]() -> uint64_t {
                                        uint64_t r = 0;
                                        if (have != 0u) {
#pragma unroll
                                            for (int u = 1; u <= kXB; u++) if ((uint32_t)kXB - have + 1u == (uint32_t)u) r = wdv[u];
                                            have -= 1u;
                                        } else {
                                            r = t.next64();
                                        }
                                        cnt += 1u;
                                        return r;
                                    };
                                    double val = 0.0;
                                    for (;;) {
                                        const double u1 = (double)(word() >> 11) * (1.0 / 9007199254740992.0);
                                        const double u2 = (double)(word() >> 11) * (1.0 / 9007199254740992.0);
                                        const double xx = -nor_inv_r * log1p(-u1);
                                        const double yy = -log1p(-u2);
                                        if (yy + yy > xx * xx) { val = ((wd >> 17) & 0x1) ? -(nor_r + xx) : nor_r + xx; break; }
                                        if (cnt > 250u) { status |= kStatusInternal; break; }
                                    }
                                    if constexpr (!Z0) lds_x[slot][l] = val;
                                    const uint32_t words = cnt, ssb = start_of(word());
                                    lds_meta[slot][l] = (uint16_t)(ss | (3u << 3) | (ssb << 5) | (words << 8));
                                } else {
                                    double x;
                                    if constexpr (Z0) {
                                        const double W = __longlong_as_double((long long)lds_kw[idx].y);
                                        x = __builtin_fma(__longlong_as_double((long long)(((wd >> 9) & 0x000fffffffffffffULL) | 0x3FF0000000000000ULL)), W, -W);
                                    } else {
                                        x = lds_x[slot][l];
                                    }
                                    const double u1 = (double)(wn >> 11) * (1.0 / 9007199254740992.0);
                                    const double y = (lds_fi[idx - 1] - lds_fi[idx]) * u1 + lds_fi[idx];
                                    const double e = (double)__builtin_amdgcn_exp2f((float)(x * x * -0.72134752044448170368));
                                    bool acc = y < e;
                                    if (__builtin_expect(!(fabs(y - e) > 1.0e-5 * e), 0)) acc = y < exp(-0.5 * x * x);
                                    lds_meta[slot][l] = (uint16_t)(ss | ((acc ? 1u : 2u) << 3));
                                }
                            }
                        }
                        if (go) hq += (uint32_t)kXB;
                        __hip_atomic_store(&lds_hhead[l], hq, __ATOMIC_RELEASE, __HIP_MEMORY_SCOPE_WORKGROUP);
                        did = true;
                    }
                } else if (ar) {
                    const uint32_t head = wg_load_acq(&lds_head[l]);
                    const uint32_t cnt = tail - head;
                    const bool want = cnt + 1u <= 8u;
                    const uint64_t bw = __builtin_amdgcn_ballot_w64(want);
                    const bool urgent = __builtin_amdgcn_ballot_w64(want && cnt <= 2) != 0;
                    if (__builtin_popcountll(bw) >= kMinLanes || urgent) {
                        Pcg64LimbsLo n = ge;
                        const uint32_t s0 = start_of(n.next64()) | 8u;
                        if (want) {
                            const uint32_t sh = (tail & 7u) * 4u;
                            ge = n;
                            vals = (vals & ~(0xFu << sh)) | (s0 << sh);
                            tail += 1u;
                        }
                        __hip_atomic_store(&lds_ring[l], (uint64_t)vals | ((uint64_t)tail << 32), __ATOMIC_RELEASE,
                                           __HIP_MEMORY_SCOPE_WORKGROUP);
                        did = true;
                    }
                }
                if (__builtin_amdgcn_ballot_w64(did) == 0) {
                    __builtin_amdgcn_s_sleep(2);
                    if (++spins > kSpinLimit * 4u) { status |= kStatusInternal; break; }
                } else {
                    spins = 0;
                }
            }
            auto undraw = [&](Pcg64 &gg, uint32_t q) {
                for (; q > 0; q--) {
                    uint64_t lo = gg.s_lo - gg.inc_lo;
                    uint64_t hi = gg.s_hi - gg.inc_hi - (gg.s_lo < gg.inc_lo ? 1ULL : 0ULL);
                    gg.s_lo = lo * a.minv_lo;
                    gg.s_hi = __umul64hi(lo, a.minv_lo) + lo * a.minv_hi + hi * a.minv_lo;
                }
            };
            ge.to(g);
            if (NRN) undraw(g, hq + 1u - __hip_atomic_load(&lds_epos[l], __ATOMIC_ACQUIRE, __HIP_MEMORY_SCOPE_WORKGROUP));
            else undraw(g, tail - wg_load_acq(&lds_head[l]));
            g.store(a.env_s, i);
            if (status) atomicOr(&a.status[i], status);
            return;
        }
        Pcg64 g;
        g.load(a.env_s, a.env_inc, i);
        auto draw = [&](Pcg64 &gg) -> uint32_t {
            const uint64_t r0 = gg.next64();
            const uint64_t m = r0 >> 11;
            uint32_t s0 = 0;
#pragma unroll
            for (int j = 0; j < 8; j++) s0 += (lds_T[j] <= m) ? 1u : 0u;
            if (IRR) {
                const uint64_t m1 = gg.next64() >> 11;
                uint32_t s1 = 0;
#pragma unroll
                for (int j = 0; j < 8; j++) s1 += (lds_T1[j] <= m1) ? 1u : 0u;
                s0 |= (s1 | 8u) << 4;
            }
            return s0;
        };
        uint32_t vals = 0, tail = 0;
        for (;;) {
            if (wg_load_acq(&lds_done) == kBlock / 64) break;
            const uint32_t head = wg_load_acq(&lds_head[l]);
            const uint32_t cnt = tail - head;
            const bool want = cnt + (uint32_t)kEN <= 8u;
            const uint64_t bw = __builtin_amdgcn_ballot_w64(want);
            const bool urgent = __builtin_amdgcn_ballot_w64(want && cnt <= 2) != 0;
            if (__builtin_popcountll(bw) >= kMinLanes || urgent) {
                Pcg64 n = g;
                const uint32_t s0 = draw(n) | 8u;
                if (want) {
                    const uint32_t sh = (tail & 7u) * 4u;
                    g = n;
                    vals = (vals & ~((IRR ? 0xFFu : 0xFu) << sh)) | (s0 << sh);
                    tail += (uint32_t)kEN;
                }
                __hip_atomic_store(&lds_ring[l], (uint64_t)vals | ((uint64_t)tail << 32), __ATOMIC_RELEASE,
                                   __HIP_MEMORY_SCOPE_WORKGROUP);
            } else {
                __builtin_amdgcn_s_sleep(MDPP_LEAN_HSLEEP);
            }
        }
        const uint32_t head = wg_load_acq(&lds_head[l]);
        for (uint32_t q = tail - head; q > 0; q--) {
            uint64_t lo = g.s_lo - g.inc_lo;
            uint64_t hi = g.s_hi - g.inc_hi - (g.s_lo < g.inc_lo ? 1ULL : 0ULL);
            g.s_lo = lo * a.minv_lo;
            g.s_hi = __umul64hi(lo, a.minv_lo) + lo * a.minv_hi + hi * a.minv_lo;
        }
        g.store(a.env_s, i);
        return;
    }

    const uint32_t total = (uint32_t)K * N;
    const int nchunks = (K + kChunk - 1) / kChunk;

    if (role == 1) {
        __builtin_amdgcn_s_setprio(kPrioO);
        auto r_rew = __builtin_amdgcn_make_buffer_rsrc((void *)reward, 0, total * 4u, kPRsrc);
        const uint32_t v4 = i * 4u;
        const uint32_t dsh = (uint32_t)(a.delay > 0 ? a.delay - 1 : 0);
        uint32_t ring = ((const uint32_t *)&a.state[i])[3];
        const uint8_t *rselb = (const uint8_t *)lds_rsel;

        const uint32_t ph_full = 16u * (uint32_t)a.every_n;
        uint32_t ph = EVN ? ph_full - 16u * (steps_at_launch % (uint32_t)a.every_n) : 0u;
        const uint64_t genv = (uint64_t)(a.env_id_offset + (int64_t)i);
        const uint32_t r4 = (uint32_t)ptick0 & 3u;
        float zc[kChunk] = {0.0f, 0.0f, 0.0f, 0.0f, 0.0f, 0.0f, 0.0f, 0.0f};
        const bool plain = a.scale == 1.0 && a.shift == 0.0;
        auto emit = [&](uint32_t ra, uint32_t rb, uint32_t rc, uint32_t so, double z, float *stage) {
            uint32_t bit = lds_V[(ra >> 5) & 2047u] >> (ra & 31u);
            uint32_t out;
            if (DELAY) {
                out = (ring >> dsh) & 1u;
                ring = (ring << 1) | (bit & 1u);
                ring = (ra != rb) ? 0u : ring;
            } else {
                out = bit & 1u;
            }
            const uint32_t tb = (rc >> 7) & 1u;
            uint32_t rd = 0;
            if (EVN) {
                ph -= 16u;
                rd = ph;
                ph = (ra != rb || ph == 0u) ? ph_full : ph;
            }
            float rout;
            if constexpr (RN && !Z0) {
                double r = (out != 0u && (!EVN || rd == 0u)) ? 1.0 : 0.0;
                r += 0.0 + a.r_noise * z;
                if (!plain) {
                    r *= a.scale;
                    r += a.shift;
                }
                if (tb) r += a.term_add;
                rout = (float)r;
            } else {
                rout = EVN ? *(const float *)(rselb + (rd | (out << 3) | (tb << 2)))
                           : *(const float *)(rselb + (((out << 1) | tb) << 2));
            }
            if (nextmode) rout = (ra != rb) ? 0.0f : rout;
            if (stage) { *stage = rout; return; }
            __builtin_amdgcn_raw_buffer_store_b32(__float_as_uint(rout), r_rew, v4, so * 4u, MDPP_LEAN_ST_AUX);
        };
        for (int c = 0; c < nchunks; c++) {
            const int kbase = c * kChunk;
            const uint32_t upto = (uint32_t)min(kbase + kChunk, K);
            if constexpr (RN && PHILOX)
                chunk_normals(a.philox_seed, genv, (ptick0 + (uint64_t)kbase) >> 2, r4, kPhiloxRNoiseStream, zc);
            uint32_t spins = 0;
            while (wg_load_acq(&lds_prod[w]) < upto) {
                __builtin_amdgcn_s_sleep(1);
                if (++spins > kSpinLimit) { status |= kStatusInternal; break; }
            }
            const bool rowc = ROWS1 && rows && kbase + kChunk <= K;
            if (kbase + kChunk <= K) {
                uint32_t ra[kChunk], rb[kChunk], rc[kChunk];
#pragma unroll
                for (int u = 0; u < kChunk; u++) {
                    ra[u] = lds_rec[0][(kbase + u) % KD][l];
                    rb[u] = lds_rec[1][(kbase + u) % KD][l];
                    rc[u] = lds_rec[2][(kbase + u) % KD][l];
                }
                double zd[kChunk];
#pragma unroll
                for (int u = 0; u < kChunk; u++) zd[u] = NRX ? lds_rx[NRX ? (kbase + u) % KD : 0][l] : (double)zc[u];
                if (rowc && c >= kRB) {
                    uint32_t sp2 = 0;
                    while (min4(lds_rcons) < (uint32_t)(c - kRB + 1)) {
                        __builtin_amdgcn_s_sleep(1);
                        if (++sp2 > kSpinLimit) { status |= kStatusInternal; break; }
                    }
                }
#pragma unroll
                for (int u = 0; u < kChunk; u++)
                    emit(ra[u], rb[u], rc[u], (uint32_t)(kbase + u) * N, zd[u], rowc ? &lds_rw[ROWS1 ? (c % kRB) : 0][u][ROWS1 ? l : 0] : nullptr);
            } else {
#pragma unroll
                for (int u = 0; u < kChunk; u++)
                    if (kbase + u < K)
                        emit(lds_rec[0][(kbase + u) % KD][l], lds_rec[1][(kbase + u) % KD][l],
                             lds_rec[2][(kbase + u) % KD][l], (uint32_t)(kbase + u) * N,
                             NRX ? lds_rx[NRX ? (kbase + u) % KD : 0][l] : (double)zc[u], nullptr);
            }
            if ((l & 63) == 0) wg_store_rel(&lds_cons[w][0], upto);
            if constexpr (ROWS1) {
                if (rowc && (l & 63) == 0) wg_store_rel(&lds_rprod[w], (uint32_t)(c + 1));
            }
        }
        ((uint32_t *)&a.state[i])[3] = ring;
        if (status) atomicOr(&a.status[i], status);
        return;
    }

    if (role == 2) {
        __builtin_amdgcn_s_setprio(MDPP_LEAN_PRIO_O2 >= 0 ? MDPP_LEAN_PRIO_O2 : (NPN && !MDPP_LEAN_PRIO_FORCED) ? (NRN ? 2 : 3)
                                   : (PN && PHILOX && !MDPP_LEAN_PRIO_FORCED) ? (RN ? 2 : 3) : kPrioO);
        auto r_obs = __builtin_amdgcn_make_buffer_rsrc(obs, 0, total * (OBS64 ? 8u : 4u) * (uint32_t)kEN, kPRsrc);
        auto r_term = __builtin_amdgcn_make_buffer_rsrc((void *)term, 0, total, kPRsrc);
        auto r_rew2 = __builtin_amdgcn_make_buffer_rsrc((void *)reward, 0, total * 4u, kPRsrc);
        auto r_trunc = __builtin_amdgcn_make_buffer_rsrc((void *)trunc, 0, total, kPRsrc);
        const uint32_t v1 = i, v4 = i * 4u, v8 = i * 8u, v16 = i * 16u;
        auto emit = [&](uint32_t rb, uint32_t rc, uint32_t so) {
            const uint32_t o = rb & 7u;
            if (IRR) {
                const uint32_t o1 = (rc >> 8) & 7u;
                if (OBS64) __builtin_amdgcn_raw_buffer_store_b128(u32x4{o, 0u, o1, 0u}, r_obs, v16 + so * 16u, 0, MDPP_LEAN_ST_AUX);
                else __builtin_amdgcn_raw_buffer_store_b64(u32x2{o, o1}, r_obs, v8, so * 8u, MDPP_LEAN_ST_AUX);
            } else if (OBS64) __builtin_amdgcn_raw_buffer_store_b64(u32x2{o, 0u}, r_obs, v8, so * 8u, MDPP_LEAN_ST_AUX);
            else __builtin_amdgcn_raw_buffer_store_b32(o, r_obs, v4, so * 4u, MDPP_LEAN_ST_AUX);
            __builtin_amdgcn_raw_buffer_store_b8((uint8_t)((rc >> 7) & 1u), r_term, v1, so, MDPP_LEAN_ST_AUX_BYTES);
            __builtin_amdgcn_raw_buffer_store_b8(HASMAX ? (uint8_t)(rc >> 16) : (uint8_t)0, r_trunc, v1, so, MDPP_LEAN_ST_AUX_BYTES);
        };
        Pcg64 sp;
        Pcg64LimbsLo gs;
        int pc = 0;
        if constexpr (NPN) { sp.load(a.sp_s, a.sp_inc, i); gs.from(sp); }
        auto make_pn = [&](int upto_chunk) __attribute__((always_inline)) {
            for (; pc < nchunks && pc < upto_chunk; pc++) {
                uint32_t pk[2] = {0u, 0u};
#pragma unroll
                for (int u = 0; u < kChunk; u++) {
                    const uint64_t r = gs.next64();
                    uint32_t by = lds_pntab[(uint32_t)(r >> 52)];
                    if (__builtin_expect(__builtin_amdgcn_ballot_w64(by == 0xFFu) != 0, 0)) {
                        if (by == 0xFFu) {
                            uint32_t na = 0, nb = 0;
#pragma unroll
                            for (int j = 0; j < 7; j++) na += (a.pn_TL[j] <= r) ? 1u : 0u;
#pragma unroll
                            for (int j = 0; j < 8; j++) nb += (a.pn_TU[j] <= r) ? 1u : 0u;
                            by = na | (nb << 4);
                        }
                    }
                    pk[u >> 2] |= by << (8 * (u & 3));
                }
                lds_pn2[pc % kHChunksNp][0][l] = pk[0];
                lds_pn2[pc % kHChunksNp][1][l] = pk[1];
                if ((l & 63) == 0) wg_store_rel(&lds_hprod[w], (uint32_t)(pc + 1));
            }
        };
        constexpr bool PPN = PN && PHILOX;
        const uint64_t genv2 = (uint64_t)(a.env_id_offset + (int64_t)i);
        int ppc = 0;
        auto make_ppn = [&](int upto_chunk) __attribute__((always_inline)) {
            for (; ppc < nchunks && ppc < upto_chunk; ppc++) {
                uint32_t wp[kChunk], pn = 0;
                chunk_words(a.philox_seed, genv2, (ptick0 + (uint64_t)(ppc * kChunk)) >> 2, (uint32_t)ptick0 & 3u, kPhiloxPNoiseStream, wp);
#pragma unroll
                for (int u = 0; u < kChunk; u++) {
                    const uint32_t e = philox_pnoise_index(wp[u], a.pn_T, a.pn_M);
                    pn |= ((e & 7u) | ((e >> 5) & 8u)) << (4 * u);
                }
                lds_pn[ppc % kHChunks][l] = pn;
                if ((l & 63) == 0) wg_store_rel(&lds_pprod[w], (uint32_t)(ppc + 1));
            }
        };
        if constexpr (PPN) make_ppn(kHChunks);
        if constexpr (NPN) make_pn(kHChunksNp);
        for (int c = 0; c < nchunks; c++) {
            const int kbase = c * kChunk;
            const uint32_t upto = (uint32_t)min(kbase + kChunk, K);
            uint32_t spins = 0;
            while (wg_load_acq(&lds_prod[w]) < upto) {
                __builtin_amdgcn_s_sleep(1);
                if (++spins > kSpinLimit) { status |= kStatusInternal; break; }
            }
            if constexpr (NPN) make_pn(c + 1 + kHChunksNp);
            if constexpr (PPN) make_ppn(c + 1 + kHChunks);
            if (ROWS2 && rows && kbase + kChunk <= K) {
                uint32_t sp2 = 0;
                while (min4(lds_prod) < upto) {
                    __builtin_amdgcn_s_sleep(1);
                    if (++sp2 > kSpinLimit) { status |= kStatusInternal; break; }
                }
                if constexpr (ROWS1) {
                    while (min4(lds_rprod) < (uint32_t)(c + 1)) {
                        __builtin_amdgcn_s_sleep(1);
                        if (++sp2 > kSpinLimit) { status |= kStatusInternal; break; }
                    }
                }
#pragma unroll
                for (int h = 0; h < kChunk / 4; h++) {
                    const uint32_t kk = (uint32_t)kbase + ws + 4u * (uint32_t)h, slot = kk % (uint32_t)KD;
                    if constexpr (ROWS1) {
                        const u32x4 v = *(const u32x4 *)&lds_rw[c % kRB][ws + 4u * (uint32_t)h][4u * ln];
                        __builtin_amdgcn_raw_buffer_store_b128(v, r_rew2, (blk0 + 4u * ln) * 4u + kk * N * 4u, 0, MDPP_LEAN_ST_AUX);
                    }
                    if (OBS64) {
                        const u32x2 b0 = *(const u32x2 *)&lds_rec[1][slot][2u * ln];
                        const u32x2 b1 = *(const u32x2 *)&lds_rec[1][slot][128u + 2u * ln];
                        __builtin_amdgcn_raw_buffer_store_b128(u32x4{b0.x & 7u, 0u, b0.y & 7u, 0u}, r_obs, (blk0 + 2u * ln) * 8u + kk * N * 8u, 0, MDPP_LEAN_ST_AUX);
                        __builtin_amdgcn_raw_buffer_store_b128(u32x4{b1.x & 7u, 0u, b1.y & 7u, 0u}, r_obs, (blk0 + 128u + 2u * ln) * 8u + kk * N * 8u, 0, MDPP_LEAN_ST_AUX);
                    } else {
                        const u32x4 b = *(const u32x4 *)&lds_rec[1][slot][4u * ln];
                        __builtin_amdgcn_raw_buffer_store_b128(u32x4{b.x & 7u, b.y & 7u, b.z & 7u, b.w & 7u}, r_obs, (blk0 + 4u * ln) * 4u + kk * N * 4u, 0, MDPP_LEAN_ST_AUX);
                    }
                    const u32x4 c4 = *(const u32x4 *)&lds_rec[2][slot][4u * ln];
                    const uint32_t t01 = __builtin_amdgcn_perm(c4.y, c4.x, 0x0c0c0400u), t23 = __builtin_amdgcn_perm(c4.w, c4.z, 0x04000c0cu);
                    const uint32_t tw = ((t01 | t23) >> 7) & 0x01010101u;
                    __builtin_amdgcn_raw_buffer_store_b32(tw, r_term, blk0 + 4u * ln, kk * N, MDPP_LEAN_ST_AUX_BYTES);
                    uint32_t uw = 0u;
                    if (HASMAX) uw = __builtin_amdgcn_perm(c4.y, c4.x, 0x0c0c0602u) | __builtin_amdgcn_perm(c4.w, c4.z, 0x06020c0cu);
                    __builtin_amdgcn_raw_buffer_store_b32(uw, r_trunc, blk0 + 4u * ln, kk * N, MDPP_LEAN_ST_AUX_BYTES);
                }
            } else if (kbase + kChunk <= K) {
                uint32_t rb[kChunk], rc[kChunk];
#pragma unroll
                for (int u = 0; u < kChunk; u++) {
                    rb[u] = lds_rec[1][(kbase + u) % KD][l];
                    rc[u] = lds_rec[2][(kbase + u) % KD][l];
                }
#pragma unroll
                for (int u = 0; u < kChunk; u++) emit(rb[u], rc[u], (uint32_t)(kbase + u) * N);
            } else {
                for (int k = kbase; k < K; k++) emit(lds_rec[1][k % KD][l], lds_rec[2][k % KD][l], (uint32_t)k * N);
            }
            if ((l & 63) == 0) {
                wg_store_rel(&lds_cons[w][1], upto);
                if (ROWS1) wg_store_rel(&lds_rcons[w], (uint32_t)(c + 1));
            }
        }
        if constexpr (NPN) {
            gs.to(sp);
            for (uint32_t q = (uint32_t)(pc * kChunk) - (uint32_t)K; q > 0; q--) {
                uint64_t lo = sp.s_lo - sp.inc_lo;
                uint64_t hi = sp.s_hi - sp.inc_hi - (sp.s_lo < sp.inc_lo ? 1ULL : 0ULL);
                sp.s_lo = lo * a.minv_lo;
                sp.s_hi = __umul64hi(lo, a.minv_lo) + lo * a.minv_hi + hi * a.minv_lo;
            }
            sp.store(a.sp_s, i);
        }
        if (status) atomicOr(&a.status[i], status);
        return;
    }

    __builtin_amdgcn_s_setprio(kPrioE);
    uint32_t k2, qv, cnt, steps0, last_reset = 0, badq[2] = {0u, 0u};
    bool pend = false;
    {
        uint4 st = a.state[i];
        k2 = 0;
        for (int j = 3; j >= 0; j--) {
            const uint32_t b = (st.x >> (8 * j)) & 0xFFu;
            k2 = (k2 << 4) | (b == 0xFFu ? 0u : ((b & 7u) | 8u));
        }
        const bool own_q = !PHILOX && !IRR && !nextmode && NZ == 0;
        const uint32_t qc = own_q ? (st.y >> 24) & 7u : 0u;
        qv = own_q ? (st.y & 0x00777777u) | (0x00888888u & ((1u << (4u * qc)) - 1u)) : 0u;
        steps0 = st.z & 0x7FFFFFFFu;
        pend = nextmode && (st.z >> 31) != 0u;
        const uint32_t ms = (uint32_t)a.max_steps;
        cnt = HASMAX ? (0x10000u - ms) + (steps0 < ms ? steps0 : ms) : 0u;
    }
    const uint32_t c0 = HASMAX ? 0x10000u - (uint32_t)a.max_steps : 0u;
    auto r_act = __builtin_amdgcn_make_buffer_rsrc((void *)actions, 0, total * 4u * (uint32_t)kEN, kPRsrc);
    const uint32_t v4 = i * 4u * (uint32_t)kEN;
    uint32_t head_local = 0;
    S0Word s0c = 0;
    uint32_t sel = (k2 & 7u) | kSelPad;
    uint32_t c1 = IRR ? (a.irr_state[i] & 7u) : 0u;
    const uint32_t A1 = IRR ? (uint32_t)a.A1 : 1u;

    uint32_t pnc = 0, pnc_hi = 0;
    uint32_t ep = 0, hh = 0, m0 = 0, m1 = 0, m2 = 0;
    double xv = 0.0;
    auto ensure = [&](uint32_t upto) __attribute__((always_inline)) {
        if (__builtin_expect(__builtin_amdgcn_ballot_w64(upto > hh) != 0, 0)) {
            uint32_t spins = 0;
            hh = __hip_atomic_load(&lds_hhead[l], __ATOMIC_ACQUIRE, __HIP_MEMORY_SCOPE_WORKGROUP);
            while (__builtin_amdgcn_ballot_w64(upto > hh) != 0) {
                __hip_atomic_store(&lds_epos[l], ep, __ATOMIC_RELAXED, __HIP_MEMORY_SCOPE_WORKGROUP);
                __builtin_amdgcn_s_sleep(1);
                hh = __hip_atomic_load(&lds_hhead[l], __ATOMIC_ACQUIRE, __HIP_MEMORY_SCOPE_WORKGROUP);
                if (++spins > kSpinLimit) { status |= kStatusInternal; hh = upto; break; }
            }
        }
    };
    auto fetch = [&]() __attribute__((always_inline)) {
        ensure(ep + 3u);
        m0 = lds_meta[ep & (uint32_t)(kXR - 1)][l];
        m1 = lds_meta[(ep + 1u) & (uint32_t)(kXR - 1)][l];
        m2 = lds_meta[(ep + 2u) & (uint32_t)(kXR - 1)][l];
        if constexpr (NRX) xv = lds_x[ep & (uint32_t)(kXR - 1)][l];
    };
    if constexpr (NRN) fetch();
    uint32_t enc_lo = 0, enc_hi = 0;
    if constexpr (PN) {
        uint64_t enc = 0;
        for (uint32_t s_ = 0; s_ < 8u; s_++) enc |= (uint64_t)(s_ | 8u | ((uint32_t)((a.term_mask >> s_) & 1ULL) << 7)) << (8 * s_);
        enc_lo = (uint32_t)enc; enc_hi = (uint32_t)(enc >> 32);
    }
    auto pull = [&](int c) {
        if (!ar && !PN) return;
        if (NPN && c >= 0) {
            uint32_t spins = 0;
            while (wg_load_acq(&lds_hprod[w]) < (uint32_t)(c + 1)) {
                __builtin_amdgcn_s_sleep(1);
                if (++spins > kSpinLimit) { status |= kStatusInternal; break; }
            }
            pnc = lds_pn2[c % kHChunksNp][0][l];
            pnc_hi = lds_pn2[c % kHChunksNp][1][l];
        }
        if constexpr (NRN) return;
        if (!PHILOX && !ar) return;
        if constexpr (PHILOX) {
            uint32_t spins = 0;
            while (wg_load_acq(&lds_hprod[w]) < (uint32_t)(c + 1)) {
                __builtin_amdgcn_s_sleep(1);
                if (++spins > kSpinLimit) { status |= kStatusInternal; break; }
            }
            s0c = lds_s0[c % kHChunks][l];
            if constexpr (PN) {
                spins = 0;
                while (wg_load_acq(&lds_pprod[w]) < (uint32_t)(c + 1)) {
                    __builtin_amdgcn_s_sleep(1);
                    if (++spins > kSpinLimit) { status |= kStatusInternal; break; }
                }
                pnc = lds_pn[c % kHChunks][l];
            }
            return;
        }
        const uint64_t rt = __hip_atomic_load(&lds_ring[l], __ATOMIC_ACQUIRE, __HIP_MEMORY_SCOPE_WORKGROUP);
        const uint32_t vals = (uint32_t)rt, tail = (uint32_t)(rt >> 32);
        const uint32_t qc = (uint32_t)__builtin_popcount(qv & 0x88888888u);
        const uint32_t avail = tail - head_local, room = kQueueCap - qc;
        const uint32_t take = avail < room ? avail : room;
        const uint32_t rot = __builtin_amdgcn_alignbit(vals, vals, (head_local & 7u) * 4u);
        const uint32_t m = (1u << (4u * take)) - 1u;
        qv |= (rot & m) << (4u * qc);
        head_local += take;
        __hip_atomic_store(&lds_head[l], head_local, __ATOMIC_RELAXED, __HIP_MEMORY_SCOPE_WORKGROUP);
    };
    typedef typename std::conditional<IRR, uint2, int>::type Act;
    typedef typename std::conditional<IRR, uint4, uint2>::type Col;
    auto column = [&](Act act, uint32_t &badm, int u) -> Col {
        int action;
        if constexpr (IRR) action = (int)act.x; else action = act;
        uint32_t ua = (uint32_t)action;
        if (__builtin_expect(__builtin_amdgcn_ballot_w64(ua >= A) != 0, 0)) {
            ua = (uint32_t)(action + ((action >> 31) & (int)A));
            const bool bad = ua >= A;
            if (nextmode) badm |= bad ? (1u << u) : 0u; else status |= bad ? (uint32_t)MDPP_STATUS_BAD_ACTION : 0u;
            ua = bad ? 0u : ua;
        }
        if constexpr (IRR) {
            const int action1 = (int)act.y;
            uint32_t ub = (uint32_t)action1;
            if (__builtin_expect(__builtin_amdgcn_ballot_w64(ub >= A1) != 0, 0)) {
                ub = (uint32_t)(action1 + ((action1 >> 31) & (int)A1));
                const bool bad = ub >= A1;
                if (nextmode) badm |= bad ? (1u << u) : 0u; else status |= bad ? (uint32_t)MDPP_STATUS_BAD_ACTION : 0u;
                ub = bad ? 0u : ub;
            }
            const uint2 ca = lds_col[ua], cb = lds_col1[ub];
            return make_uint4(ca.x, ca.y, cb.x, cb.y);
        } else {
            return lds_col[ua];
        }
    };
    auto stepE = [&](const Col &col, int k, uint32_t badbit) {
        uint32_t entry = __builtin_amdgcn_perm(col.y, col.x, sel);
        if constexpr (PN && PHILOX) {
            const uint32_t nib = (pnc >> (4 * (k % kChunk))) & 0xFu, j = nib & 7u, nx = entry & 7u;
            const uint32_t ns = nib > 7u ? j + (j >= nx ? 1u : 0u) : nx;
            entry = __builtin_amdgcn_perm(enc_hi, enc_lo, ns | kSelPad);
        }
        if constexpr (NPN) {
            const uint32_t by = (((k % kChunk) < 4 ? pnc : pnc_hi) >> (8 * (k & 3))) & 0xFFu, nx = entry & 7u;
            const uint32_t ns = min(by & 15u, nx) + (uint32_t)max((int)(by >> 4) - (int)nx, 0);
            entry = __builtin_amdgcn_perm(enc_hi, enc_lo, ns | kSelPad);
        }
        const uint32_t k2n = (k2 << 4) | entry;
        bool need = entry > 0x7Fu;
        uint32_t rc = entry;
        if (HASMAX) {
            cnt += 1;
            need = need || cnt >= 0x10000u;
            rc = __builtin_amdgcn_perm(cnt, entry, 0x0c060c00u);
        }
        need = need && ar;
        uint32_t rec_a = k2n;
        if (nextmode) {
            const bool ended = need && !pend;
            need = pend;
            rc = pend ? 0u : rc;
            rec_a = pend ? 0u : k2n;
            status |= (badbit != 0u && !pend) ? (uint32_t)MDPP_STATUS_BAD_ACTION : 0u;
            pend = ended;
        }
        uint32_t s0v = PHILOX ? (uint32_t)(s0c >> (kEN * 4 * (k % kChunk))) & (IRR ? 0xFFu : 0xFu) : qv & (IRR ? 0xFFu : 0xFu);
        if constexpr (NRN) {
            uint32_t kind = (m0 >> 3) & 3u;
            if (__builtin_expect(__builtin_amdgcn_ballot_w64(kind >= 2u) != 0, 0)) {
                uint32_t guard = 0;
                while (__builtin_amdgcn_ballot_w64(kind == 2u) != 0) {
                    const bool red = kind == 2u;
                    ep += red ? 2u : 0u;
                    uint32_t o0 = m0, o1 = m1, o2 = m2;
                    double ox = xv;
                    fetch();
                    if (!red) { m0 = o0; m1 = o1; m2 = o2; xv = ox; }
                    kind = (m0 >> 3) & 3u;
                    if (++guard > 64u) { status |= kStatusInternal; break; }
                }
            }
            uint32_t cntw = kind == 0u ? 1u : 2u, ssm = kind == 0u ? m1 : m2;
            if (kind == 3u) { cntw = m0 >> 8; ssm = m0 >> 5; }
            if constexpr (NRX) lds_rx[k % KD][l] = xv;
            s0v = (ssm & 7u) | 8u;
            ep += cntw + (need ? 1u : 0u);
            __hip_atomic_store(&lds_epos[l], ep, __ATOMIC_RELAXED, __HIP_MEMORY_SCOPE_WORKGROUP);
            fetch();
        }
        if (!PHILOX && !NRN && __builtin_expect(__builtin_amdgcn_ballot_w64(need && s0v == 0u) != 0, 0)) {
            uint32_t spins = 0;
            while (__builtin_amdgcn_ballot_w64(need && (qv & 0xFu) == 0u) != 0) {
                pull(-1);
                __builtin_amdgcn_s_sleep(1);
                if (++spins > kSpinLimit) { status |= kStatusInternal; qv |= 8u; break; }
            }
            s0v = qv & (IRR ? 0xFFu : 0xFu);
        }
        if constexpr (IRR) {
            const uint32_t n1 = __builtin_amdgcn_perm(col.w, col.z, c1 | kSelPad);
            c1 = need ? ((s0v >> 4) & 7u) : n1;
            rc |= c1 << 8;
            s0v &= 0xFu;
        }
        k2 = need ? s0v : k2n;
        if (!PHILOX && !NRN) qv = need ? (qv >> (4 * kEN)) : qv;
        if (HASMAX) cnt = need ? c0 : cnt;
        else last_reset = need ? (uint32_t)(k + 1) : last_reset;
        sel = (k2 & 7u) | kSelPad;
        lds_rec[0][k % KD][l] = rec_a;
        lds_rec[1][k % KD][l] = k2;
        lds_rec[2][k % KD][l] = rc;
    };

    auto load_act = [&](int k) -> Act {
        const uint32_t kk = (uint32_t)min(k, K - 1);
        if constexpr (IRR) {
            const u32x2 v = __builtin_amdgcn_raw_buffer_load_b64(r_act, v4, kk * N * 8u, MDPP_LEAN_LD_AUX);
            return make_uint2(v.x, v.y);
        } else {
            return __builtin_amdgcn_raw_buffer_load_b32(r_act, v4, kk * N * 4u, MDPP_LEAN_LD_AUX);
        }
    };
    constexpr int kAh = IRR ? 2 : kAhead;
    static_assert(kAh % 2 == 0, "the column double buffer alternates with the chunk index");
    Act actq[kAh][kChunk];
    Col colq[2][kChunk];
#pragma unroll
    for (int u = 0; u < kChunk; u++) colq[0][u] = column(load_act(u), badq[0], u);
#pragma unroll
    for (int q = 0; q < kAh; q++)
#pragma unroll
        for (int u = 0; u < kChunk; u++) actq[q][u] = load_act((q + 1) * kChunk + u);

    const int nfull = K / kChunk;
    auto wait_room = [&](int kend) {
        if (kend > KD) {
            const uint32_t must = (uint32_t)(kend - KD);
            uint32_t spins = 0;
            for (;;) {
                const uint64_t cc = __hip_atomic_load((const uint64_t *)&lds_cons[w][0], __ATOMIC_ACQUIRE,
                                                      __HIP_MEMORY_SCOPE_WORKGROUP);
                uint32_t have = min((uint32_t)cc, (uint32_t)(cc >> 32));
                if (rows) {
#pragma unroll
                    for (int j = 0; j < kBlock / 64; j++) have = min(have, wg_load_acq(&lds_cons[j][1]));
                }
                if (have >= must) break;
                __builtin_amdgcn_s_sleep(1);
                if (++spins > kSpinLimit) { status |= kStatusInternal; break; }
            }
        }
    };
    auto chunkE = [&](int c, int j, bool refill) {
        const int kbase = c * kChunk;
        badq[(j + 1) & 1] = 0u;
#pragma unroll
        for (int u = 0; u < kChunk; u++) colq[(j + 1) & 1][u] = column(actq[j][u], badq[(j + 1) & 1], u);
        if (refill) {
#pragma unroll
            for (int u = 0; u < kChunk; u++) actq[j][u] = load_act(kbase + (kAh + 1) * kChunk + u);
        }
        wait_room(kbase + kChunk);
        pull(c);
#pragma unroll
        for (int u = 0; u < kChunk; u++) stepE(colq[j & 1][u], kbase + u, (badq[j & 1] >> u) & 1u);
        if (NRN) __hip_atomic_store(&lds_epos[l], ep, __ATOMIC_RELAXED, __HIP_MEMORY_SCOPE_WORKGROUP);
        if ((l & 63) == 0) wg_store_rel(&lds_prod[w], (uint32_t)(kbase + kChunk));
    };
    const int ngrp = nfull / kAh;
    for (int g = 0; g < ngrp; g++) {
#pragma unroll
        for (int j = 0; j < kAh; j++) chunkE(g * kAh + j, j, true);
    }
#pragma unroll
    for (int j = 0; j < kAh - 1; j++)
        if (ngrp * kAh + j < nfull) chunkE(ngrp * kAh + j, j, false);
    if (K % kChunk) {
        const int kbase = nfull * kChunk;
        Act ta[kChunk];
#pragma unroll
        for (int u = 0; u < kChunk; u++) ta[u] = load_act(kbase + u);
        wait_room(kbase + kChunk);
        pull(nfull);
#pragma unroll
        for (int u = 0; u < kChunk; u++)
            if (kbase + u < K) {
                uint32_t bm = 0;
                const Col cc = column(ta[u], bm, 0);
                stepE(cc, kbase + u, bm);
            }
        if ((l & 63) == 0) wg_store_rel(&lds_prod[w], (uint32_t)K);
    }

    uint32_t hist = 0;
    for (int j = 3; j >= 0; j--) {
        const uint32_t nb = (k2 >> (4 * j)) & 0xFu;
        hist = (hist << 8) | ((nb & 8u) ? (nb & 7u) : 0xFFu);
    }
    const uint32_t qc = (uint32_t)__builtin_popcount(qv & 0x00888888u);
    const bool own_q = !PHILOX && !IRR && !nextmode && NZ == 0;
    if (NRN) __hip_atomic_store(&lds_epos[l], ep, __ATOMIC_RELEASE, __HIP_MEMORY_SCOPE_WORKGROUP);
    if (!own_q && !PHILOX && !NRN) {
        __hip_atomic_store(&lds_head[l], head_local - qc, __ATOMIC_RELEASE, __HIP_MEMORY_SCOPE_WORKGROUP);
    }
    if (IRR) a.irr_state[i] = c1;
    uint32_t steps;
    if (HASMAX) steps = cnt - c0;
    else steps = last_reset ? (uint32_t)K - last_reset : steps0 + (uint32_t)K;
    uint32_t *st = (uint32_t *)&a.state[i];
    st[0] = hist; st[2] = steps | (pend ? 0x80000000u : 0u);
    if (own_q) st[1] = (qv & 0x00777777u) | (qc << 24);
    if ((l & 63) == 0) __hip_atomic_fetch_add(&lds_done, 1u, __ATOMIC_RELEASE, __HIP_MEMORY_SCOPE_WORKGROUP);
    if (status) atomicOr(&a.status[i], status);
}

static bool lean_launch(const DiscreteArgs &a, const DiscreteIO &io, const int nz) {
    constexpr bool kNext = MDPP_LEAN_TU_NEXT;
    const int K = io.K;
    const bool ph = a.philox != 0, irr = a.irr != 0;
    if (io.final_obs) return false;
    const bool shape = a.autoreset == MDPP_AUTORESET_NEXT_STEP ? a.lean_next_ok != 0
                       : (nz && !ph) ? a.shape_ok_noise_np != 0
                       : nz ? a.shape_ok_noise != 0
                       : irr ? a.shape_ok_irr != 0 : (ph ? (a.shape_ok != 0 || (MDPP_LEAN_TU_NOISE == 0 && !MDPP_LEAN_TU_NEXT && a.shape_ok_noise != 0 && a.r_noise == 0.0 && !a.has_p_noise)) : a.fast_ok != 0);
    if (!shape || (ph && (a.opts & MDPP_OPT_NO_PHILOX_FAST)) || K < 32 || a.N < kBlock ||
        (a.opts & (MDPP_OPT_NO_PIPE | MDPP_OPT_NO_LEAN)))
        return false;
    if (nz && (a.opts & MDPP_OPT_NO_QUIET_NOISE)) return false;
    if (!a.autoreset && a.max_steps > 0) return false;
    if (a.S > 8 || a.A > 16 || a.every_n > 64 || a.max_steps >= 65536) return false;
    if (irr && (a.S1 > 8 || a.A1 > 16 || (8ULL * 2 * a.N * (unsigned long long)K) >= (1ULL << 32)))
        return false;
    const int grid = (a.N + kBlock - 1) / kBlock;
    auto go = [&](auto O64, auto DL, auto HM, auto EV, auto PH, auto IR, auto NZ) {
        if (io.name_out) {
            int n = snprintf(io.name_out, kNameLen, "k_discrete_rollout_lean<OBS64=%d,DELAY=%d,HASMAX=%d,EVN=%d,PHILOX=%d,IRR=%d,NEXT=%d", O64(), DL(),
                             HM(), EV(), PH(), IR(), kNext);
            if (NZ()) n += snprintf(io.name_out + n, kNameLen - n, ",PN=%d,RN=%d%s", NZ() & 1, (NZ() >> 1) & 1, (NZ() & 4) ? ",Z0=1" : "");
            snprintf(io.name_out + n, kNameLen - n, ">");
        } else {
            launch_rollout(k_discrete_rollout_lean<O64(), DL(), HM(), EV(), PH(), IR(), kNext, NZ()>, grid, kRoles * kBlock, 0, a, io);
        }
    };
#if MDPP_LEAN_TU_NOISE
    const bool z0 = MDPP_LEAN_TU_NOISE == 2 && (nz & 2) && a.r_noise == 0.0 && !(a.opts & MDPP_OPT_NO_SIGMA0);
    with_bools([&](auto O64, auto DL, auto HM, auto EV) {
        with_value<1, 2, 3, 6, 7>(nz | (z0 ? 4 : 0), [&](auto NZ) {
            if constexpr (NZ() < 4 || MDPP_LEAN_TU_NOISE == 2)
                go(O64, DL, HM, EV, std::bool_constant<MDPP_LEAN_TU_NOISE == 1>{}, std::false_type{}, NZ);
        });
    }, !a.obs_i32, a.delay > 0, a.max_steps > 0, a.every_n > 1);
#else
    with_bools([&](auto O64, auto DL, auto HM, auto EV, auto PH, auto IR) {
        go(O64, DL, HM, EV, PH, IR, std::integral_constant<int, 0>{});
    }, !a.obs_i32, a.delay > 0, a.max_steps > 0, a.every_n > 1, ph, irr);
#endif
    return true;
}

#if MDPP_LEAN_TU_NEXT
bool launch_discrete_lean_next(const DiscreteArgs &a, const DiscreteIO &io) {
    if (a.autoreset != MDPP_AUTORESET_NEXT_STEP) return false;
    return lean_launch(a, io, 0);
}
#elif MDPP_LEAN_TU_NOISE == 1
bool launch_discrete_lean_noise(const DiscreteArgs &a, const DiscreteIO &io) {
    const int nz = (a.has_p_noise ? 1 : 0) | (a.has_r_noise ? 2 : 0);
    if (nz == 0 || a.autoreset == MDPP_AUTORESET_NEXT_STEP || !a.philox || a.irr) return false;
    return lean_launch(a, io, nz);
}
#elif MDPP_LEAN_TU_NOISE == 2
bool launch_discrete_lean_npnoise(const DiscreteArgs &a, const DiscreteIO &io) {
    const int nz = (a.has_p_noise ? 1 : 0) | (a.has_r_noise ? 2 : 0);
    if (nz == 0 || a.autoreset == MDPP_AUTORESET_NEXT_STEP || a.philox || a.irr) return false;
    return lean_launch(a, io, nz);
}
#else
bool launch_discrete_lean_next(const DiscreteArgs &a, const DiscreteIO &io);
bool launch_discrete_lean_noise(const DiscreteArgs &a, const DiscreteIO &io);
bool launch_discrete_lean_npnoise(const DiscreteArgs &a, const DiscreteIO &io);
bool launch_discrete_lean(const DiscreteArgs &a, const DiscreteIO &io) {
    if (a.autoreset == MDPP_AUTORESET_NEXT_STEP) return launch_discrete_lean_next(a, io);
    if ((a.has_p_noise || a.has_r_noise) && !a.philox) return launch_discrete_lean_npnoise(a, io);
    const bool ph_sig0 = a.philox && !a.has_p_noise && a.has_r_noise && a.r_noise == 0.0 && !(a.opts & MDPP_OPT_NO_SIGMA0);
    if ((a.has_p_noise || a.has_r_noise) && !ph_sig0) return launch_discrete_lean_noise(a, io);
    return lean_launch(a, io, 0);
}
#endif

}
```

### mdp_playground_amd/csrc/mdpp_internal.hpp

```cpp
#pragma once
#include <hip/hip_runtime.h>
#include <stdint.h>
#include <stdio.h>
#include <string.h>

#include <string>
#include <type_traits>
#include <vector>

#include "../../include/mdpp.h"

namespace mdpp {

#ifndef MDPP_ST_NT
#define MDPP_ST_NT 2
#endif
constexpr int kBlock = 256;
constexpr uint32_t kNoKey = 0xFFFFFFFFu;
constexpr uint32_t kRingPyZero = 0x7FC0DE1Au;
constexpr uint32_t kPhiloxResetStream = 3;
constexpr uint32_t kPhiloxIrrStream = 4;
constexpr uint32_t kPhiloxActionStream = 5;
constexpr uint32_t kPhiloxStartStream = 9;
constexpr uint32_t kPhiloxStartIrrStream = 10;
constexpr uint32_t kPhiloxPNoiseStream = 12;
constexpr uint32_t kPhiloxRNoiseStream = 13;
constexpr uint32_t kPhiloxPolicyStream = 14;
constexpr uint32_t kPhiloxLearnExploreStream = 15;
constexpr uint32_t kPhiloxLearnActionStream = 16;
constexpr uint32_t kPhiloxLearnUpdateStream = 17;

struct EpisodeStatsDev {
    double *cur, *last;
    int32_t nk;
};
__device__ __forceinline__ void est_add(const EpisodeStatsDev &e, long N, long i, int k, double v) {
    e.cur[(size_t)k * N + i] += v;
}
__device__ __forceinline__ void est_roll(const EpisodeStatsDev &e, long N, long i, uint32_t steps) {
    for (int k = 0; k < e.nk; k++) {
        e.last[(size_t)k * N + i] = e.cur[(size_t)k * N + i];
        e.cur[(size_t)k * N + i] = 0.0;
    }
    e.last[(size_t)e.nk * N + i] = (double)steps;
}

struct DiscreteArgs {
    int32_t N;
    int32_t S, A, L, delay, every_n;
    int32_t shared_tables;
    int32_t unit_rewards;
    int32_t rew_sa;
    int32_t has_p_noise, has_r_noise;
    int32_t autoreset, max_steps, obs_i32;
    int32_t philox;
    uint32_t pn_T;
    uint64_t pn_M, pn_M1;
    uint32_t nkeys;
    uint32_t tick;
    uint64_t ptick;
    const uint64_t *dtick;
    uint32_t opts;
    uint64_t philox_seed;
    int64_t env_id_offset;
    double r_noise, scale, shift, term_add;
    const uint8_t *P;
    const double *rtable;
    const uint8_t *rbits;
    const uint8_t *is_term;
    const double *init_cdf;
    const double *noise_cdf;
    uint32_t rbits_stride;
    uint32_t lds_P, lds_term, lds_rew, lds_init, lds_noise, lds_bytes;
    uint32_t rew_in_lds, noise_in_lds;
    uint4 *state;
    uint64_t *hist_hi;
    uint32_t *ring_keys;
    ulonglong2 *env_s, *env_inc, *sp_s, *sp_inc;
    uint32_t *status;
    EpisodeStatsDev est;
    int32_t irr, S1, A1;
    const uint8_t *P1;
    const double *init_cdf1;
    const double *noise_cdf1;
    uint32_t *irr_state;
    ulonglong2 *sp1_s, *sp1_inc;
    uint32_t fast_ok;
    uint32_t shape_ok;
    uint32_t shape_ok_irr;
    uint32_t shape_ok_noise;
    uint32_t lean_next_ok;
    uint32_t shape_ok_noise_np;
    uint64_t pn_TL[8], pn_TU[8];
    uint32_t s_shift;
    uint32_t key_mask;
    uint32_t spow;
    uint64_t term_mask;
    uint64_t init_thr[16];
    float rsel[4];
    uint64_t minv_lo, minv_hi;
};

#ifndef MDPP_S1_REPLICAS
#define MDPP_S1_REPLICAS 1
#endif
constexpr uint32_t kS1wRounds = 8, kS1wRoundsNoise = 12;
constexpr int kS1Replicas = MDPP_S1_REPLICAS;
struct Step1Args {
    int32_t N;
    uint32_t A, S, L, every_n, max_steps, delay, autoreset;
    uint32_t term32;
    uint32_t nan_mask;
    uint32_t topup_rounds, topup_fill;
    float rsel[4];
    double inv_every_n;
    uint64_t ptick;
    const uint64_t *dtick;
    uint64_t philox_seed;
    int64_t env_id_offset;
    const uint4 *blob;
    uint32_t wide, blob_rounds, off_term, off_thr, off_thr31, off_rew, S8, off_bk;
    uint32_t unit, ring_head;
    uint32_t *ring_keys;
    double scale, shift, term_add;
    uint32_t has_p_noise, has_r_noise, off_tn, off_zig, pn_T;
    uint64_t pn_M;
    double r_noise;
    ulonglong2 *sp_s;
    const ulonglong2 *sp_inc;
    const int32_t *actions;
    void *obs;
    float *reward;
    uint8_t *term, *trunc;
    void *final_obs;
    uint4 *state;
    ulonglong2 *env_s;
    const ulonglong2 *env_inc;
    uint32_t *status;
};

struct ContinuousArgs {
    int32_t N, D, n_rel, order, delay, every_n;
    int32_t make_denser, has_p_noise, has_r_noise, bounded;
    int32_t autoreset, max_steps, philox, n_boxes, rel_prefix;
    uint32_t tick;
    uint64_t ptick;
    const uint64_t *dtick;
    uint32_t opts;
    uint64_t philox_seed;
    int64_t env_id_offset;
    float inertia32, amax32, smax32, radius32, alw32, scale32, shift32, term_add32;
    float tpow32[MDPP_MAX_ORDER + 1];
    double fact[MDPP_MAX_ORDER + 1];
    double p_noise, r_noise, scale, shift, term_add, reset_lo, reset_range;
    int32_t rel[MDPP_MAX_DIM];
    float target[MDPP_MAX_DIM];
    float box_lo[MDPP_MAX_BOXES * MDPP_MAX_DIM];
    float box_hi[MDPP_MAX_BOXES * MDPP_MAX_DIM];
    float *sd;
    float *cur;
    uint2 *meta;
    uint32_t *ring;
    int32_t line_L;
    int32_t line_NL;
    int32_t line_lds;
    float *line_hist;
    double *line_ws;
    double *ring64;
    int32_t target64, rew64;
    double radius;
    ulonglong2 *env_s, *env_inc, *sp_s, *sp_inc;
    uint32_t *status;
    EpisodeStatsDev est;
    int32_t park;
    int32_t image_quirk;
    uint32_t fast_ok;
    uint32_t inertia_pow2;
    float inv_inertia32;
    uint32_t fact_pow2_mask;
    double inv_fact[MDPP_MAX_ORDER + 1];
};

template <class A>
__device__ __forceinline__ uint64_t tick_now(const A &a) { return a.ptick + (a.dtick ? *a.dtick : 0ULL); }
template <class A>
__device__ __forceinline__ uint32_t ring_head_now(const A &a, uint64_t ptick) {
    return a.dtick ? (a.delay > 0 ? (uint32_t)(ptick % (uint64_t)a.delay) : 0u) : a.tick;
}

inline bool dynamic_lds_ok(const void *kernel, size_t dyn_bytes) {
    if (dyn_bytes <= 32 * 1024) return true;
    hipFuncAttributes fa;
    if (hipFuncGetAttributes(&fa, kernel) != hipSuccess) { (void)hipGetLastError(); return false; }
    int dev = 0, max_lds = 0;
    if (hipGetDevice(&dev) != hipSuccess ||
        hipDeviceGetAttribute(&max_lds, hipDeviceAttributeMaxSharedMemoryPerBlock, dev) != hipSuccess) { (void)hipGetLastError(); return false; }
    if (fa.sharedSizeBytes + dyn_bytes > (size_t)max_lds) return false;
    if (hipFuncSetAttribute(kernel, hipFuncAttributeMaxDynamicSharedMemorySize, (int)dyn_bytes) != hipSuccess) { (void)hipGetLastError(); return false; }
    return true;
}

struct GridArgs {
    int32_t N, G;
    int32_t shape[4], target[2];
    int32_t make_denser, has_p_noise, has_r_noise, every_n;
    int32_t autoreset, max_steps, obs_i32, philox;
    uint64_t ptick;
    const uint64_t *dtick;
    uint32_t opts;
    uint64_t philox_seed;
    int64_t env_id_offset;
    double p_noise, r_noise, scale, shift, term_add;
    uint4 *state;
    ulonglong2 *env_s, *env_inc, *sp_s, *sp_inc, *act_s, *act_inc;
    uint2 *act_half;
    uint64_t minv_lo, minv_hi;
    uint32_t *status;
    EpisodeStatsDev est;
};

}

struct mdpp_env {
    mdpp_config cfg;
    int device;
    std::string err;
    uint64_t tick;
    uint64_t reset_tick;
    uint32_t opts;
    char kname[192];
    void *d_P, *d_rtable, *d_rbits, *d_is_term, *d_init_cdf, *d_noise_cdf;
    void *d_state, *d_ring, *d_status;
    void *d_hist_hi;
    void *d_line_hist, *d_line_ws, *d_ring64;
    void *d_est_cur, *d_est_last;
    int32_t est_nk;
    void *d_P1, *d_init_cdf1, *d_noise_cdf1, *d_irr_state;
    bool irr_ready;
    bool graph_capture;
    void *d_tick_off;
    bool line_hist_stale;
    void *d_sd, *d_cur, *d_meta;
    void *d_rng_s[MDPP_NUM_STREAMS], *d_rng_inc[MDPP_NUM_STREAMS], *d_rng_half;
    void *d_img_tpl, *d_img_tplp, *d_img_clsx, *d_img_clsy, *d_img_rot, *d_img_state_out, *d_img_state_final;
    void *d_img_near;
    void *d_img_rec;
    void *d_img_ctr;
    int32_t img_chunk;
    uint32_t imgc_disc_rows[32];
    void *d_imgc_boxes;
    bool img_ready, img_fast_ok, img_lines_ready;
    int32_t img_n_radii, img_n_cls_x, img_n_cls_y;
    int32_t img_colb;
    uint32_t nkeys, rbits_stride;
    bool tables_ready, streams_ready[MDPP_NUM_STREAMS];
    hipEvent_t ev0, ev1;
    hipStream_t side_stream;
    hipEvent_t ev_entry, ev_side[2], ev_render[2];
    mdpp::DiscreteArgs dargs;
    mdpp::Step1Args s1args;
    void *d_s1_blob;
    void *d_policy_thr;
    uint64_t policy_seed;
    bool policy_ready;
    void *d_learn_q, *d_learn_carry;
    uint64_t learn_seed;
    uint32_t learn_E;
    float learn_alpha, learn_gamma;
    int32_t learn_algo;
    bool learn_ready;
    int32_t learn_q_tables;
    void *d_learn_alpha, *d_learn_gamma, *d_learn_E;
    uint32_t learn_pe, learn_pe_stale;
    bool learn_pm;
    bool nl_on, nl_pm;
    int32_t nl_levels;
    void *d_nl_level, *d_nl_sigma, *d_nl_cdf, *d_nl_T, *d_nl_M;
    std::vector<double> nl_tn, nl_rn;
    bool nl_fill_valid;
    float nl_fill_alpha, nl_fill_gamma;
    uint32_t nl_fill_E;
    mdpp::ContinuousArgs cargs;
    mdpp::GridArgs gargs;
};

namespace mdpp {
struct GenArgs {
    int32_t S, A, L, diameter, n_term, maxc, repeats, unit;
    uint64_t total;
    uint32_t n_sel;
    uint32_t radix[16];
    const double *rews;
    uint32_t n_rews;
    uint32_t nkeys, rbits_stride;
    const uint64_t *seeds;
    uint8_t *P;
    uint8_t *rbits;
    double *rtable;
    uint64_t *sd;
    ulonglong2 *env_s, *env_inc, *sp_s, *sp_inc, *im_s, *im_inc;
    uint2 *im_half;
    uint64_t *scratch;
    uint64_t scratch_words, set_words, perm_off;
};

constexpr size_t kGenScratchCap = (size_t)256 << 20;

inline int gen_args_init(const mdpp_gen_params *p, int S, int A, int L, bool image, bool unit, uint32_t nkeys,
                         uint32_t rbits_stride, GenArgs &a, const char **err) {
    const int d = p->diameter, n_term = p->n_term;
    const uint32_t nn = (uint32_t)(A - n_term);
    bool ok = d >= 1 && S == A * d && n_term >= 0 && n_term < A && p->n_sel >= 1 && p->n_sel <= p->total &&
              (p->image != 0) == image;
    if (ok && p->repeats) {
        uint64_t t = 1;
        for (int i = 0; i < L; i++) t *= nn;
        ok = p->total == t;
    } else if (ok) {
        uint64_t t = 1;
        ok = p->n_radices == L;
        for (int i = 0; ok && i < L; i++) {
            ok = p->radices[i] == nn - (uint32_t)(i / d) && p->radices[i] >= 1;
            t *= p->radices[i];
        }
        ok = ok && p->total == t;
    }
    const uint64_t n_seqs = (uint64_t)d * p->n_sel;
    if (ok && p->rews) ok = p->n_rews >= n_seqs && p->n_rews > 1;
    if (!ok) { *err = "generate_discrete: parameters do not match the handle"; return MDPP_EINVAL; }
    memset(&a, 0, sizeof(a));
    a.set_words = (p->total + 63u) / 64u;
    a.perm_off = a.set_words + (uint64_t)(p->repeats ? 1 : d) * p->n_sel;
    a.scratch_words = a.perm_off + (p->rews ? ((uint64_t)p->n_rews + 1u) / 2u : 0u);
    if ((size_t)a.scratch_words * 8u > kGenScratchCap) {
        *err = "generate_discrete: scratch per env above the cap";
        return MDPP_EUNSUPPORTED;
    }
    a.S = S; a.A = A; a.L = L; a.diameter = d; a.n_term = n_term; a.maxc = p->maximally_connected ? 1 : 0;
    a.repeats = p->repeats ? 1 : 0; a.unit = unit ? 1 : 0;
    a.total = p->total; a.n_sel = p->n_sel;
    for (int i = 0; i < 16; i++) a.radix[i] = p->repeats ? 0u : p->radices[i];
    a.n_rews = p->rews ? p->n_rews : 0u;
    a.nkeys = nkeys; a.rbits_stride = rbits_stride;
    return MDPP_OK;
}

template <class F> inline void with_bools(F &&f) { f(); }
template <class F, class... Bs> inline void with_bools(F &&f, bool b, Bs... rest) {
    if (b) with_bools([&](auto... cs) { f(std::true_type{}, cs...); }, rest...);
    else with_bools([&](auto... cs) { f(std::false_type{}, cs...); }, rest...);
}
template <int... Vs, class F> inline bool with_value(int v, F &&f) {
    return ((v == Vs ? (f(std::integral_constant<int, Vs>{}), true) : false) || ...);
}

constexpr int kNameLen = 192;
struct EpisodeSummaryArgs {
    double *ret;
    int32_t *len, *episodes;
    double *return_sum;
    int32_t *length_sum;
};
template <class Act, class Obs>
struct StepIO {
    int K;
    const Act *actions;
    Obs *obs;
    float *reward;
    uint8_t *term, *trunc;
    Obs *final_obs;
    hipStream_t s;
    char *name_out;
    const EpisodeSummaryArgs *summary = nullptr;
    StepIO piece(int k0, int kc, size_t N, size_t act_elems, size_t obs_bytes) const {
        const size_t off = (size_t)k0 * N;
        StepIO p = *this;
        p.K = kc;
        p.actions = actions + off * act_elems;
        p.obs = (Obs *)((char *)obs + off * obs_bytes);
        p.reward = reward + off; p.term = term + off; p.trunc = trunc + off;
        p.final_obs = final_obs ? (Obs *)((char *)final_obs + off * obs_bytes) : nullptr;
        return p;
    }
};
using DiscreteIO = StepIO<int32_t, void>;
using ContinuousIO = StepIO<float, float>;
inline DiscreteIO piece_of(const DiscreteArgs &a, const DiscreteIO &io, int k0, int kc) {
    const size_t w = a.irr ? 2 : 1;
    return io.piece(k0, kc, (size_t)a.N, w, w * (a.obs_i32 ? 4 : 8));
}
inline ContinuousIO piece_of(const ContinuousArgs &a, const ContinuousIO &io, int k0, int kc) {
    return io.piece(k0, kc, (size_t)a.N, (size_t)a.D, (size_t)a.D * sizeof(float));
}
template <class Kern, class A, class IO>
inline void launch_rollout(Kern kern, int grid, int block, size_t lds, const A &a, const IO &io) {
    hipLaunchKernelGGL(kern, dim3(grid), dim3(block), lds, io.s, a, io.K, io.actions, io.obs, io.reward, io.term, io.trunc,
                       io.final_obs);
}

inline void stamp_piece(GridArgs &a, const mdpp_env *h, int k0) { a.ptick = h->tick + (uint64_t)k0; }
template <class A> inline void stamp_piece(A &a, const mdpp_env *h, int k0) {
    a.ptick = h->tick + (uint64_t)k0;
    a.tick = a.delay > 0 ? (uint32_t)(a.ptick % (uint64_t)a.delay) : 0u;
}
template <class A> inline void stamp_step(A &a, const mdpp_env *h) {
    a.opts = h->opts;
    a.dtick = h->graph_capture ? (const uint64_t *)h->d_tick_off : nullptr;
    stamp_piece(a, h, 0);
}
template <class A, class IO, class Body>
inline bool for_each_piece(A &a, const mdpp_env *h, const IO &io, long long kmax, Body &&body) {
    for (int k0 = 0; k0 < io.K;) {
        const int kc = (int)((io.K - k0) < kmax ? (io.K - k0) : kmax);
        stamp_piece(a, h, k0);
        if (!body(piece_of(a, io, k0, kc), k0)) return false;
        if (io.name_out) return true;
        k0 += kc;
    }
    return true;
}
inline int step_done(mdpp_env *h, int K, const char *kernel) {
    hipError_t e = hipGetLastError();
    if (e != hipSuccess) { h->err = std::string(kernel) + " launch: " + hipGetErrorString(e); return MDPP_EHIP; }
    h->tick += (uint64_t)K;
    return MDPP_OK;
}

int launch_discrete_step(mdpp_env *h, const DiscreteIO &io);
int launch_discrete_reset(mdpp_env *h, const uint8_t *mask, void *obs, hipStream_t s);
int launch_discrete_step_wide(mdpp_env *h, const DiscreteIO &io);
int launch_discrete_reset_wide(mdpp_env *h, const uint8_t *mask, void *obs, hipStream_t s);
int launch_discrete_step_long(mdpp_env *h, const DiscreteIO &io);
int launch_discrete_reset_long(mdpp_env *h, const uint8_t *mask, void *obs, hipStream_t s);
bool launch_discrete_fast(const DiscreteArgs &a, const DiscreteIO &io);
int launch_continuous_step(mdpp_env *h, const ContinuousIO &io);
int launch_continuous_reset(mdpp_env *h, const uint8_t *mask, float *obs, hipStream_t s);
bool launch_discrete_step1(const DiscreteArgs &d, const Step1Args &proto, const DiscreteIO &io);
bool launch_discrete_quiet(const DiscreteArgs &a, const DiscreteIO &io);
bool launch_discrete_pipe(const DiscreteArgs &a, const DiscreteIO &io);
bool launch_discrete_lean(const DiscreteArgs &a, const DiscreteIO &io);
bool launch_continuous_fast(const ContinuousArgs &a, const ContinuousIO &io);
bool launch_continuous_step1(const ContinuousArgs &a, const ContinuousIO &io);
bool launch_continuous_line(const ContinuousArgs &a, const ContinuousIO &io);
int launch_imagec_obs(mdpp_env *h, int K, const void *states, const void *final_states, const uint8_t *term,
                      const uint8_t *trunc, const uint8_t *mask, uint8_t *img_out, uint8_t *img_final, hipStream_t s);
std::string discrete_policy_refusal(const mdpp_env *h);
int launch_discrete_policy(mdpp_env *h, const DiscreteIO &io);
std::string discrete_learn_refusal(const mdpp_env *h);
int launch_discrete_learn(mdpp_env *h, const DiscreteIO &io);
int launch_learn_q_copy(mdpp_env *h, float *user_q, bool to_handle, hipStream_t s);
int launch_discrete_eval(mdpp_env *h, const DiscreteIO &io);
int launch_discrete_current_obs(mdpp_env *h, void *obs, hipStream_t s);
int launch_grid_step(mdpp_env *h, const DiscreteIO &io);
int launch_grid_reset(mdpp_env *h, const uint8_t *mask, void *obs, hipStream_t s);
int launch_image_obs(mdpp_env *h, int K, const int32_t *state_out, const int32_t *state_final,
                     const uint8_t *term, const uint8_t *trunc, const uint8_t *mask,
                     uint8_t *img_out, uint8_t *img_final, hipStream_t s, int phase = 3, int buf = 0);
int launch_image_step1(mdpp_env *h, const int32_t *state_out, const int32_t *state_final, const uint8_t *term,
                       const uint8_t *trunc, uint8_t *img_out, uint8_t *img_final, hipStream_t s);
const char *image_obs_kernel_name(const mdpp_env *h, int K);
}
hipError_t launch_generate_discrete(const mdpp::GenArgs &a, int first, int count);
hipError_t launch_seed_streams_seedseq(const uint64_t *seeds, int N, void *st, void *inc, void *half);
```

Before: 266.0 billion env-steps/s.

## Precompute lean rollout lookup tables once into a device blob and copy per block

Adds a one-block builder kernel, run at table upload time, that computes the lean kernel's shared-memory lookup tables (reward-bit expansion V, transition columns, init thresholds, reward selectors) into a global blob. The rollout kernel then copies the precomputed units into LDS instead of rebuilding them in every block on every launch. The E role is split into an included file and starts without waiting on the table setup. This removes redundant per-launch prologue work across many blocks, at the cost of extra setup code, a new allocation, and a restructured role layout that could change register or LDS usage.

Result: faster. 281.1 billion env-steps/s, median of 6 (+5.7%).

```diff
diff --git a/mdp_playground_amd/build.py b/mdp_playground_amd/build.py
--- a/mdp_playground_amd/build.py
+++ b/mdp_playground_amd/build.py
@@ -22,7 +22,8 @@
            "mdpp_generate.hip"]
 HEADERS = ["mdpp_internal.hpp", "mdpp_rng.hpp", "mdpp_discrete_closed.hpp", "mdpp_pcg64_limbs.inc", "np_ziggurat_tables.inc",
            os.path.join("..", "..", "include", "mdpp.h")]
-INCLUDED_SOURCES = {"mdpp_discrete_wide.hip": ["mdpp_discrete.hip"], "mdpp_discrete_long.hip": ["mdpp_discrete.hip"], "mdpp_discrete_lean_next.hip": ["mdpp_discrete_lean.hip"], "mdpp_discrete_lean_noise.hip": ["mdpp_discrete_lean.hip"], "mdpp_discrete_lean_npnoise.hip": ["mdpp_discrete_lean.hip"],
+_LEAN_DEPS = ["mdpp_discrete_lean.hip", "mdpp_discrete_lean_e.inc"]
+INCLUDED_SOURCES = {"mdpp_discrete_lean.hip": ["mdpp_discrete_lean_e.inc"], "mdpp_discrete_wide.hip": ["mdpp_discrete.hip"], "mdpp_discrete_long.hip": ["mdpp_discrete.hip"], "mdpp_discrete_lean_next.hip": _LEAN_DEPS, "mdpp_discrete_lean_noise.hip": _LEAN_DEPS, "mdpp_discrete_lean_npnoise.hip": _LEAN_DEPS,
                     "mdpp_continuous_line8.hip": ["mdpp_continuous.hip"], "mdpp_continuous_step1.hip": ["mdpp_continuous_fast.hip"], "mdpp_discrete_quiet_nu.hip": ["mdpp_discrete_quiet.hip"],
                     **{u: ["mdpp_discrete_learn.hpp"] for u in SOURCES if u.startswith("mdpp_discrete_learn")},
                     **{u: ["mdpp_discrete_eval.hpp"] for u in SOURCES if u.startswith("mdpp_discrete_eval")}}
diff --git a/mdp_playground_amd/csrc/mdpp_capi.hip b/mdp_playground_amd/csrc/mdpp_capi.hip
--- a/mdp_playground_amd/csrc/mdpp_capi.hip
+++ b/mdp_playground_amd/csrc/mdpp_capi.hip
@@ -55,7 +55,7 @@
                     h->d_P1, h->d_init_cdf1, h->d_noise_cdf1, h->d_irr_state,
                     h->d_img_tpl, h->d_img_tplp, h->d_img_clsx, h->d_img_clsy, h->d_img_rot, h->d_img_state_out,
                     h->d_img_state_final, h->d_img_rec, h->d_img_ctr, h->d_line_hist, h->d_line_ws, h->d_ring64, h->d_est_cur, h->d_est_last, h->d_tick_off,
-                    h->d_img_near, h->d_s1_blob, h->d_imgc_boxes, h->d_hist_hi, h->d_policy_thr, h->d_learn_q, h->d_learn_carry,
+                    h->d_img_near, h->d_s1_blob, h->d_lean_blob, h->d_imgc_boxes, h->d_hist_hi, h->d_policy_thr, h->d_learn_q, h->d_learn_carry,
                     h->d_learn_alpha, h->d_learn_gamma, h->d_learn_E,
                     h->d_nl_level, h->d_nl_sigma, h->d_nl_cdf, h->d_nl_T, h->d_nl_M};
     for (void *p : ptrs) if (p) (void)hipFree(p);
@@ -114,6 +114,7 @@
     h->d_img_tpl = h->d_img_tplp = h->d_img_clsx = h->d_img_clsy = h->d_img_rot = nullptr;
     h->d_img_near = nullptr;
     h->d_s1_blob = nullptr;
+    h->d_lean_blob = nullptr;
     memset(&h->s1args, 0, sizeof(h->s1args));
     h->d_policy_thr = nullptr; h->policy_seed = 0; h->policy_ready = false;
     h->d_learn_q = h->d_learn_carry = nullptr; h->learn_seed = 0; h->learn_E = 0; h->learn_alpha = h->learn_gamma = 0.0f;
@@ -447,6 +448,20 @@
 }
 
 static inline bool t_fits53(uint64_t t) { return t <= (1ULL << 53) - 1; }
+
+static int lean_tables_build(mdpp_env *h) {
+    DiscreteArgs &a = h->dargs;
+    const mdpp_config &c = h->cfg;
+    a.lean_blob = nullptr;
+    const bool lean_shape = a.shape_ok || a.shape_ok_irr || a.lean_next_ok || a.shape_ok_noise || a.shape_ok_noise_np;
+    if (!lean_shape || !h->tables_ready || (c.irrelevant && !h->irr_ready)) return MDPP_OK;
+    if (c.S > 8 || c.A > 16 || c.L > 3 || c.every_n > 64 || (c.irrelevant && (c.S_irr > 8 || c.A_irr > 16))) return MDPP_OK;
+    if (!h->d_lean_blob) HIPCHK(h, hipMalloc(&h->d_lean_blob, (size_t)mdpp::kLeanTabUnits * 16));
+    HIPCHK(h, mdpp::launch_lean_build_tables(a, h->d_lean_blob, nullptr));
+    HIPCHK(h, hipStreamSynchronize(nullptr));
+    a.lean_blob = (const uint4 *)h->d_lean_blob;
+    return MDPP_OK;
+}
 
 static int discrete_derived(mdpp_env *h, const uint8_t *P, const double *rtable, const uint8_t *rbits,
                             const uint8_t *is_term, const double *init_cdf, const double *noise_cdf) {
@@ -620,7 +635,7 @@
         }
     }
     h->tables_ready = true;
-    return MDPP_OK;
+    return lean_tables_build(h);
 }
 
 extern "C" int mdpp_upload_discrete_tables(mdpp_env *h, const uint8_t *P, const double *rtable,
@@ -794,7 +809,7 @@
     if (h->cfg.has_transition_noise)
         HIPCHK(h, hipMemcpy(h->d_noise_cdf1, noise_cdf1, S1 * S1 * sizeof(double), hipMemcpyHostToDevice));
     h->irr_ready = true;
-    return MDPP_OK;
+    return lean_tables_build(h);
 }
 
 extern "C" int mdpp_upload_image_disc(mdpp_env *h, const uint8_t *disc) {
diff --git a/mdp_playground_amd/csrc/mdpp_discrete_lean.hip b/mdp_playground_amd/csrc/mdpp_discrete_lean.hip
--- a/mdp_playground_amd/csrc/mdpp_discrete_lean.hip
+++ b/mdp_playground_amd/csrc/mdpp_discrete_lean.hip
@@ -111,6 +111,74 @@
 }
 using namespace lean;
 
+#if !MDPP_LEAN_TU_NEXT && !MDPP_LEAN_TU_NOISE
+__global__ __launch_bounds__(kRoles * kBlock) void k_lean_build_tables(DiscreteArgs a, uint4 *__restrict__ blob) {
+    __shared__ __align__(16) uint4 lds_tab[kLeanTabUnits];
+    __shared__ __align__(16) uint32_t lds_R[128];
+    uint32_t *const lds_V = (uint32_t *)&lds_tab[kLeanTabV];
+    uint2 *const lds_col = (uint2 *)&lds_tab[kLeanTabCol], *const lds_col1 = (uint2 *)&lds_tab[kLeanTabCol1];
+    uint64_t *const lds_T = (uint64_t *)&lds_tab[kLeanTabT], *const lds_T1 = (uint64_t *)&lds_tab[kLeanTabT1];
+    float *const lds_rsel = (float *)&lds_tab[kLeanTabRsel];
+    const int tid = threadIdx.x;
+    if (tid < (int)kLeanTabUnits) lds_tab[tid] = make_uint4(0u, 0u, 0u, 0u);
+    __syncthreads();
+    const uint32_t S = (uint32_t)a.S, L = (uint32_t)a.L;
+    if (tid < 16) {
+        uint64_t cs = 0;
+        if (tid < a.A)
+            for (uint32_t s = 0; s < S; s++) {
+                const uint32_t nx = a.P[s * a.A + tid] & 7u;
+                cs |= (uint64_t)(nx | 8u | ((uint32_t)((a.term_mask >> nx) & 1ULL) << 7)) << (8 * s);
+            }
+        lds_col[tid] = make_uint2((uint32_t)cs, (uint32_t)(cs >> 32));
+        if (tid < 8) lds_T[tid] = a.init_thr[tid];
+        if (a.irr) {
+            uint64_t c1 = 0;
+            if (tid < a.A1)
+                for (int s1 = 0; s1 < a.S1; s1++) c1 |= (uint64_t)(a.P1[s1 * a.A1 + tid] & 7u) << (8 * s1);
+            lds_col1[tid] = make_uint2((uint32_t)c1, (uint32_t)(c1 >> 32));
+            if (tid < 8) lds_T1[tid] = tid < a.S1 ? (uint64_t)ceil(a.init_cdf1[tid] * 9007199254740992.0) : ~0ULL;
+        }
+    }
+    for (int k = tid; k < 4 * a.every_n; k += kRoles * kBlock) lds_rsel[k] = a.rsel[k < 4 ? k : (k & 1)];
+    for (uint32_t k = tid; k < 128; k += kRoles * kBlock) {
+        uint32_t wd = 0;
+        for (int b = 0; b < 4; b++) {
+            uint32_t byte = 4 * k + b;
+            if (byte < a.rbits_stride) wd |= (uint32_t)a.rbits[byte] << (8 * b);
+        }
+        lds_R[k] = wd;
+    }
+    __syncthreads();
+    {
+        uint32_t dmask = 0;
+        for (uint32_t j = 1; j <= L; j++) dmask |= 1u << (4 * j - 2);
+        for (uint32_t d = tid; d < 2048; d += kRoles * kBlock) {
+            uint32_t wd = 0;
+            if ((d & dmask) == dmask) {
+                for (uint32_t b = 8; b < 32; b++) {
+                    if (!(b & 8u)) continue;
+                    const uint32_t idx = d * 32u + b;
+                    uint32_t key = 0, pw = 1;
+                    for (uint32_t j = 0; j < L; j++) { key += ((idx >> (4 * j)) & 7u) * pw; pw *= S; }
+                    if (key < a.nkeys) wd |= ((lds_R[key >> 5] >> (key & 31u)) & 1u) << b;
+                }
+            }
+            lds_V[d] = wd;
+        }
+    }
+    __syncthreads();
+    if (tid < (int)kLeanTabUnits) blob[tid] = lds_tab[tid];
+}
+
+hipError_t launch_lean_build_tables(const DiscreteArgs &a, void *blob, hipStream_t s) {
+    static_assert(kLeanTabUnits <= (uint32_t)(kRoles * kBlock) && kLeanTabUnits - (kLeanTabRsel - kLeanTabCol1) <= (uint32_t)((kRoles - 1) * kBlock),
+                  "one unit per thread: the builder's, and the rollout kernel's copy by its O and H lanes");
+    hipLaunchKernelGGL(k_lean_build_tables, dim3(1), dim3(kRoles * kBlock), 0, s, a, (uint4 *)blob);
+    return hipGetLastError();
+}
+#endif
+
 template <bool OBS64, bool DELAY, bool HASMAX, bool EVN, bool PHILOX, bool IRR, bool NEXT, int NZ = 0>
 __global__ __launch_bounds__(kRoles * kBlock) void k_discrete_rollout_lean(DiscreteArgs a, int K,
                                                                       const int32_t *__restrict__ actions,
@@ -127,11 +195,21 @@
     constexpr bool NRX = NRN && !Z0;
     constexpr int KD = NRN ? kDepthNp : kDepth;
     __shared__ __align__(16) uint32_t lds_rec[3][KD][kBlock];
+#if MDPP_LEAN_TU_NOISE == 2
     __shared__ __align__(16) uint32_t lds_V[2048];
     __shared__ __align__(16) uint2 lds_col[16];
     __shared__ __align__(16) uint32_t lds_R[128];
     __shared__ __align__(16) uint64_t lds_T[8];
     __shared__ __align__(16) float lds_rsel[EVN ? 4 * 64 : 4];
+#else
+    constexpr uint32_t kTabSkip = IRR ? 0u : kLeanTabRsel - kLeanTabCol1;
+    constexpr uint32_t kTabUnits = kLeanTabRsel - kTabSkip + (EVN ? kLeanTabUnits - kLeanTabRsel : 1u);
+    __shared__ __align__(16) uint4 lds_tab[kTabUnits];
+    uint32_t *const lds_V = (uint32_t *)&lds_tab[kLeanTabV];
+    uint2 *const lds_col = (uint2 *)&lds_tab[kLeanTabCol];
+    uint64_t *const lds_T = (uint64_t *)&lds_tab[kLeanTabT];
+    float *const lds_rsel = (float *)&lds_tab[kLeanTabRsel - kTabSkip];
+#endif
     __shared__ __align__(16) uint64_t lds_ring[kBlock];
     __shared__ uint32_t lds_head[kBlock];
     __shared__ uint32_t lds_prod[kBlock / 64];
@@ -144,8 +222,13 @@
     __shared__ __align__(16) uint32_t lds_rprod[kBlock / 64], lds_rcons[kBlock / 64];
     typedef typename std::conditional<IRR, uint64_t, uint32_t>::type S0Word;
     __shared__ __align__(16) S0Word lds_s0[PHILOX ? kHChunks : 1][kBlock];
+#if MDPP_LEAN_TU_NOISE == 2
     __shared__ __align__(16) uint2 lds_col1[IRR ? 16 : 1];
     __shared__ __align__(16) uint64_t lds_T1[IRR ? 8 : 1];
+#else
+    uint2 *const lds_col1 = (uint2 *)&lds_tab[IRR ? kLeanTabCol1 : kLeanTabCol];
+    uint64_t *const lds_T1 = (uint64_t *)&lds_tab[IRR ? kLeanTabT1 : kLeanTabT];
+#endif
     __shared__ uint32_t lds_hprod[kBlock / 64];
     __shared__ uint32_t lds_pprod[kBlock / 64];
     constexpr bool kNpNoise = !PHILOX && NZ != 0;
@@ -171,6 +254,7 @@
     const int role = tid / kBlock;
     const int l = tid & (kBlock - 1);
     const int w = l >> 6;
+#if MDPP_LEAN_TU_NOISE == 2
     const uint32_t S = (uint32_t)a.S, L = (uint32_t)a.L;
     if (tid < 16) {
         uint64_t cs = 0;
@@ -270,6 +354,68 @@
     constexpr int kMinLanes = MDPP_LEAN_HMIN;
     uint32_t status = 0;
 
+#else
+    const uint32_t eblk = ((gridDim.x & 7u) == 0u) ? (blockIdx.x & 7u) * (gridDim.x >> 3) + (blockIdx.x >> 3) : blockIdx.x;
+    const uint32_t i = eblk * kBlock + l;
+    const uint32_t N = (uint32_t)a.N;
+    const bool rows = ROWS2 && (N % (uint32_t)kBlock) == 0u;
+    const uint32_t blk0 = eblk * kBlock, ln = (uint32_t)l & 63u;
+    const uint32_t ws = (uint32_t)__builtin_amdgcn_readfirstlane(w);
+    auto min4 = [&](const uint32_t *p) -> uint32_t {
+        const uint64_t x = __hip_atomic_load((const uint64_t *)p, __ATOMIC_ACQUIRE, __HIP_MEMORY_SCOPE_WORKGROUP);
+        const uint64_t y = __hip_atomic_load((const uint64_t *)p + 1, __ATOMIC_ACQUIRE, __HIP_MEMORY_SCOPE_WORKGROUP);
+        return min(min((uint32_t)x, (uint32_t)(x >> 32)), min((uint32_t)y, (uint32_t)(y >> 32)));
+    };
+    const uint32_t A = (uint32_t)a.A;
+    constexpr int kMinLanes = MDPP_LEAN_HMIN;
+    uint32_t status = 0;
+
+    const uint32_t total = (uint32_t)K * N;
+    typedef typename std::conditional<IRR, uint2, int>::type Act;
+    auto setup_shared = [&]() __attribute__((always_inline)) {
+        if (tid < kBlock) { lds_ring[tid] = 0; lds_head[tid] = 0; if (NRN) { lds_hhead[tid] = 0; lds_epos[tid] = 0; } }
+        if (NRN || NPN) {
+            for (uint32_t k = tid; k < 2048u; k += kRoles * kBlock) {
+                const uint64_t lo = (uint64_t)k << 53, hi = lo + ((1ULL << 53) - 1ULL);
+                uint32_t c0 = 0, c1 = 0;
+                for (int j = 0; j < 8; j++) {
+                    const uint64_t t = a.init_thr[j] > (1ULL << 53) - 1ULL ? ~0ULL : a.init_thr[j] << 11;
+                    c0 += (t <= lo) ? 1u : 0u; c1 += (t <= hi) ? 1u : 0u;
+                }
+                lds_sstab[k] = (uint8_t)(c0 == c1 ? c0 : 0xFFu);
+            }
+        }
+        if (NPN) {
+            for (uint32_t k = tid; k < 4096u; k += kRoles * kBlock) {
+                const uint64_t lo = (uint64_t)k << 52, hi = lo + ((1ULL << 52) - 1ULL);
+                uint32_t a0 = 0, a1 = 0, b0 = 0, b1 = 0;
+                for (int j = 0; j < 7; j++) { a0 += (a.pn_TL[j] <= lo) ? 1u : 0u; a1 += (a.pn_TL[j] <= hi) ? 1u : 0u; }
+                for (int j = 0; j < 8; j++) { b0 += (a.pn_TU[j] <= lo) ? 1u : 0u; b1 += (a.pn_TU[j] <= hi) ? 1u : 0u; }
+                lds_pntab[k] = (uint8_t)((a0 == a1 && b0 == b1) ? (a0 | (b0 << 4)) : 0xFFu);
+            }
+        }
+        if (NRN)
+            for (int k = tid; k < 256; k += kRoles * kBlock) { lds_kw[k] = make_ulonglong2(d_zig_ki[k], (unsigned long long)(__double_as_longlong(d_zig_wi[k]) + (52LL << 52)));    lds_fi[k] = d_zig_fi[k]; }
+        if (tid < kBlock / 64) { lds_prod[tid] = 0; lds_cons[tid][0] = 0; lds_cons[tid][1] = 0; lds_hprod[tid] = 0; lds_pprod[tid] = 0; lds_rprod[tid] = 0; lds_rcons[tid] = 0; }
+        if (tid == 0) lds_done = 0;
+    };
+
+    if (role == 0) {
+#include "mdpp_discrete_lean_e.inc"
+        return;
+    }
+
+    if (tid >= kBlock && (uint32_t)(tid - kBlock) < kTabUnits) {
+        const uint32_t c = (uint32_t)(tid - kBlock);
+        lds_tab[c] = a.lean_blob[c < kLeanTabCol1 ? c : c + kTabSkip];
+    }
+    setup_shared();
+    uint32_t steps_at_launch = 0;
+    if (EVN && role == 1 && i < N) steps_at_launch = ((const uint32_t *)&a.state[i])[2] & 0x7FFFFFFFu;
+    __syncthreads();
+    if (i >= N) return;
+
+#endif
     if (role == 3) {
         if (!ar && !PN && !NRN) return;
         __builtin_amdgcn_s_setprio(kPrioH);
@@ -533,7 +679,9 @@
         return;
     }
 
+#if MDPP_LEAN_TU_NOISE == 2
     const uint32_t total = (uint32_t)K * N;
+#endif
     const int nchunks = (K + kChunk - 1) / kChunk;
 
     if (role == 1) {
@@ -777,315 +925,16 @@
         return;
     }
 
-    __builtin_amdgcn_s_setprio(kPrioE);
-    uint32_t k2, qv, cnt, steps0, last_reset = 0, badq[2] = {0u, 0u};
-    bool pend = false;
-    {
-        uint4 st = a.state[i];
-        k2 = 0;
-        for (int j = 3; j >= 0; j--) {
-            const uint32_t b = (st.x >> (8 * j)) & 0xFFu;
-            k2 = (k2 << 4) | (b == 0xFFu ? 0u : ((b & 7u) | 8u));
-        }
-        const bool own_q = !PHILOX && !IRR && !nextmode && NZ == 0;
-        const uint32_t qc = own_q ? (st.y >> 24) & 7u : 0u;
-        qv = own_q ? (st.y & 0x00777777u) | (0x00888888u & ((1u << (4u * qc)) - 1u)) : 0u;
-        steps0 = st.z & 0x7FFFFFFFu;
-        pend = nextmode && (st.z >> 31) != 0u;
-        const uint32_t ms = (uint32_t)a.max_steps;
-        cnt = HASMAX ? (0x10000u - ms) + (steps0 < ms ? steps0 : ms) : 0u;
-    }
-    const uint32_t c0 = HASMAX ? 0x10000u - (uint32_t)a.max_steps : 0u;
-    auto r_act = __builtin_amdgcn_make_buffer_rsrc((void *)actions, 0, total * 4u * (uint32_t)kEN, kPRsrc);
-    const uint32_t v4 = i * 4u * (uint32_t)kEN;
-    uint32_t head_local = 0;
-    S0Word s0c = 0;
-    uint32_t sel = (k2 & 7u) | kSelPad;
-    uint32_t c1 = IRR ? (a.irr_state[i] & 7u) : 0u;
-    const uint32_t A1 = IRR ? (uint32_t)a.A1 : 1u;
-
-    uint32_t pnc = 0, pnc_hi = 0;
-    uint32_t ep = 0, hh = 0, m0 = 0, m1 = 0, m2 = 0;
-    double xv = 0.0;
-    auto ensure = [&](uint32_t upto) __attribute__((always_inline)) {
-        if (__builtin_expect(__builtin_amdgcn_ballot_w64(upto > hh) != 0, 0)) {
-            uint32_t spins = 0;
-            hh = __hip_atomic_load(&lds_hhead[l], __ATOMIC_ACQUIRE, __HIP_MEMORY_SCOPE_WORKGROUP);
-            while (__builtin_amdgcn_ballot_w64(upto > hh) != 0) {
-                __hip_atomic_store(&lds_epos[l], ep, __ATOMIC_RELAXED, __HIP_MEMORY_SCOPE_WORKGROUP);
-                __builtin_amdgcn_s_sleep(1);
-                hh = __hip_atomic_load(&lds_hhead[l], __ATOMIC_ACQUIRE, __HIP_MEMORY_SCOPE_WORKGROUP);
-                if (++spins > kSpinLimit) { status |= kStatusInternal; hh = upto; break; }
-            }
-        }
-    };
-    auto fetch = [&]() __attribute__((always_inline)) {
-        ensure(ep + 3u);
-        m0 = lds_meta[ep & (uint32_t)(kXR - 1)][l];
-        m1 = lds_meta[(ep + 1u) & (uint32_t)(kXR - 1)][l];
-        m2 = lds_meta[(ep + 2u) & (uint32_t)(kXR - 1)][l];
-        if constexpr (NRX) xv = lds_x[ep & (uint32_t)(kXR - 1)][l];
-    };
-    if constexpr (NRN) fetch();
-    uint32_t enc_lo = 0, enc_hi = 0;
-    if constexpr (PN) {
-        uint64_t enc = 0;
-        for (uint32_t s_ = 0; s_ < 8u; s_++) enc |= (uint64_t)(s_ | 8u | ((uint32_t)((a.term_mask >> s_) & 1ULL) << 7)) << (8 * s_);
-        enc_lo = (uint32_t)enc; enc_hi = (uint32_t)(enc >> 32);
-    }
-    auto pull = [&](int c) {
-        if (!ar && !PN) return;
-        if (NPN && c >= 0) {
-            uint32_t spins = 0;
-            while (wg_load_acq(&lds_hprod[w]) < (uint32_t)(c + 1)) {
-                __builtin_amdgcn_s_sleep(1);
-                if (++spins > kSpinLimit) { status |= kStatusInternal; break; }
-            }
-            pnc = lds_pn2[c % kHChunksNp][0][l];
-            pnc_hi = lds_pn2[c % kHChunksNp][1][l];
-        }
-        if constexpr (NRN) return;
-        if (!PHILOX && !ar) return;
-        if constexpr (PHILOX) {
-            uint32_t spins = 0;
-            while (wg_load_acq(&lds_hprod[w]) < (uint32_t)(c + 1)) {
-                __builtin_amdgcn_s_sleep(1);
-                if (++spins > kSpinLimit) { status |= kStatusInternal; break; }
-            }
-            s0c = lds_s0[c % kHChunks][l];
-            if constexpr (PN) {
-                spins = 0;
-                while (wg_load_acq(&lds_pprod[w]) < (uint32_t)(c + 1)) {
-                    __builtin_amdgcn_s_sleep(1);
-                    if (++spins > kSpinLimit) { status |= kStatusInternal; break; }
-                }
-                pnc = lds_pn[c % kHChunks][l];
-            }
-            return;
-        }
-        const uint64_t rt = __hip_atomic_load(&lds_ring[l], __ATOMIC_ACQUIRE, __HIP_MEMORY_SCOPE_WORKGROUP);
-        const uint32_t vals = (uint32_t)rt, tail = (uint32_t)(rt >> 32);
-        const uint32_t qc = (uint32_t)__builtin_popcount(qv & 0x88888888u);
-        const uint32_t avail = tail - head_local, room = kQueueCap - qc;
-        const uint32_t take = avail < room ? avail : room;
-        const uint32_t rot = __builtin_amdgcn_alignbit(vals, vals, (head_local & 7u) * 4u);
-        const uint32_t m = (1u << (4u * take)) - 1u;
-        qv |= (rot & m) << (4u * qc);
-        head_local += take;
-        __hip_atomic_store(&lds_head[l], head_local, __ATOMIC_RELAXED, __HIP_MEMORY_SCOPE_WORKGROUP);
-    };
-    typedef typename std::conditional<IRR, uint2, int>::type Act;
-    typedef typename std::conditional<IRR, uint4, uint2>::type Col;
-    auto column = [&](Act act, uint32_t &badm, int u) -> Col {
-        int action;
-        if constexpr (IRR) action = (int)act.x; else action = act;
-        uint32_t ua = (uint32_t)action;
-        if (__builtin_expect(__builtin_amdgcn_ballot_w64(ua >= A) != 0, 0)) {
-            ua = (uint32_t)(action + ((action >> 31) & (int)A));
-            const bool bad = ua >= A;
-            if (nextmode) badm |= bad ? (1u << u) : 0u; else status |= bad ? (uint32_t)MDPP_STATUS_BAD_ACTION : 0u;
-            ua = bad ? 0u : ua;
-        }
-        if constexpr (IRR) {
-            const int action1 = (int)act.y;
-            uint32_t ub = (uint32_t)action1;
-            if (__builtin_expect(__builtin_amdgcn_ballot_w64(ub >= A1) != 0, 0)) {
-                ub = (uint32_t)(action1 + ((action1 >> 31) & (int)A1));
-                const bool bad = ub >= A1;
-                if (nextmode) badm |= bad ? (1u << u) : 0u; else status |= bad ? (uint32_t)MDPP_STATUS_BAD_ACTION : 0u;
-                ub = bad ? 0u : ub;
-            }
-            const uint2 ca = lds_col[ua], cb = lds_col1[ub];
-            return make_uint4(ca.x, ca.y, cb.x, cb.y);
-        } else {
-            return lds_col[ua];
-        }
-    };
-    auto stepE = [&](const Col &col, int k, uint32_t badbit) {
-        uint32_t entry = __builtin_amdgcn_perm(col.y, col.x, sel);
-        if constexpr (PN && PHILOX) {
-            const uint32_t nib = (pnc >> (4 * (k % kChunk))) & 0xFu, j = nib & 7u, nx = entry & 7u;
-            const uint32_t ns = nib > 7u ? j + (j >= nx ? 1u : 0u) : nx;
-            entry = __builtin_amdgcn_perm(enc_hi, enc_lo, ns | kSelPad);
-        }
-        if constexpr (NPN) {
-            const uint32_t by = (((k % kChunk) < 4 ? pnc : pnc_hi) >> (8 * (k & 3))) & 0xFFu, nx = entry & 7u;
-            const uint32_t ns = min(by & 15u, nx) + (uint32_t)max((int)(by >> 4) - (int)nx, 0);
-            entry = __builtin_amdgcn_perm(enc_hi, enc_lo, ns | kSelPad);
-        }
-        const uint32_t k2n = (k2 << 4) | entry;
-        bool need = entry > 0x7Fu;
-        uint32_t rc = entry;
-        if (HASMAX) {
-            cnt += 1;
-            need = need || cnt >= 0x10000u;
-            rc = __builtin_amdgcn_perm(cnt, entry, 0x0c060c00u);
-        }
-        need = need && ar;
-        uint32_t rec_a = k2n;
-        if (nextmode) {
-            const bool ended = need && !pend;
-            need = pend;
-            rc = pend ? 0u : rc;
-            rec_a = pend ? 0u : k2n;
-            status |= (badbit != 0u && !pend) ? (uint32_t)MDPP_STATUS_BAD_ACTION : 0u;
-            pend = ended;
-        }
-        uint32_t s0v = PHILOX ? (uint32_t)(s0c >> (kEN * 4 * (k % kChunk))) & (IRR ? 0xFFu : 0xFu) : qv & (IRR ? 0xFFu : 0xFu);
-        if constexpr (NRN) {
-            uint32_t kind = (m0 >> 3) & 3u;
-            if (__builtin_expect(__builtin_amdgcn_ballot_w64(kind >= 2u) != 0, 0)) {
-                uint32_t guard = 0;
-                while (__builtin_amdgcn_ballot_w64(kind == 2u) != 0) {
-                    const bool red = kind == 2u;
-                    ep += red ? 2u : 0u;
-                    uint32_t o0 = m0, o1 = m1, o2 = m2;
-                    double ox = xv;
-                    fetch();
-                    if (!red) { m0 = o0; m1 = o1; m2 = o2; xv = ox; }
-                    kind = (m0 >> 3) & 3u;
-                    if (++guard > 64u) { status |= kStatusInternal; break; }
-                }
-            }
-            uint32_t cntw = kind == 0u ? 1u : 2u, ssm = kind == 0u ? m1 : m2;
-            if (kind == 3u) { cntw = m0 >> 8; ssm = m0 >> 5; }
-            if constexpr (NRX) lds_rx[k % KD][l] = xv;
-            s0v = (ssm & 7u) | 8u;
-            ep += cntw + (need ? 1u : 0u);
-            __hip_atomic_store(&lds_epos[l], ep, __ATOMIC_RELAXED, __HIP_MEMORY_SCOPE_WORKGROUP);
-            fetch();
-        }
-        if (!PHILOX && !NRN && __builtin_expect(__builtin_amdgcn_ballot_w64(need && s0v == 0u) != 0, 0)) {
-            uint32_t spins = 0;
-            while (__builtin_amdgcn_ballot_w64(need && (qv & 0xFu) == 0u) != 0) {
-                pull(-1);
-                __builtin_amdgcn_s_sleep(1);
-                if (++spins > kSpinLimit) { status |= kStatusInternal; qv |= 8u; break; }
-            }
-            s0v = qv & (IRR ? 0xFFu : 0xFu);
-        }
-        if constexpr (IRR) {
-            const uint32_t n1 = __builtin_amdgcn_perm(col.w, col.z, c1 | kSelPad);
-            c1 = need ? ((s0v >> 4) & 7u) : n1;
-            rc |= c1 << 8;
-            s0v &= 0xFu;
-        }
-        k2 = need ? s0v : k2n;
-        if (!PHILOX && !NRN) qv = need ? (qv >> (4 * kEN)) : qv;
-        if (HASMAX) cnt = need ? c0 : cnt;
-        else last_reset = need ? (uint32_t)(k + 1) : last_reset;
-        sel = (k2 & 7u) | kSelPad;
-        lds_rec[0][k % KD][l] = rec_a;
-        lds_rec[1][k % KD][l] = k2;
-        lds_rec[2][k % KD][l] = rc;
-    };
-
-    auto load_act = [&](int k) -> Act {
-        const uint32_t kk = (uint32_t)min(k, K - 1);
-        if constexpr (IRR) {
-            const u32x2 v = __builtin_amdgcn_raw_buffer_load_b64(r_act, v4, kk * N * 8u, MDPP_LEAN_LD_AUX);
-            return make_uint2(v.x, v.y);
-        } else {
-            return __builtin_amdgcn_raw_buffer_load_b32(r_act, v4, kk * N * 4u, MDPP_LEAN_LD_AUX);
-        }
-    };
-    constexpr int kAh = IRR ? 2 : kAhead;
-    static_assert(kAh % 2 == 0, "the column double buffer alternates with the chunk index");
-    Act actq[kAh][kChunk];
-    Col colq[2][kChunk];
-#pragma unroll
-    for (int u = 0; u < kChunk; u++) colq[0][u] = column(load_act(u), badq[0], u);
-#pragma unroll
-    for (int q = 0; q < kAh; q++)
-#pragma unroll
-        for (int u = 0; u < kChunk; u++) actq[q][u] = load_act((q + 1) * kChunk + u);
-
-    const int nfull = K / kChunk;
-    auto wait_room = [&](int kend) {
-        if (kend > KD) {
-            const uint32_t must = (uint32_t)(kend - KD);
-            uint32_t spins = 0;
-            for (;;) {
-                const uint64_t cc = __hip_atomic_load((const uint64_t *)&lds_cons[w][0], __ATOMIC_ACQUIRE,
-                                                      __HIP_MEMORY_SCOPE_WORKGROUP);
-                uint32_t have = min((uint32_t)cc, (uint32_t)(cc >> 32));
-                if (rows) {
-#pragma unroll
-                    for (int j = 0; j < kBlock / 64; j++) have = min(have, wg_load_acq(&lds_cons[j][1]));
-                }
-                if (have >= must) break;
-                __builtin_amdgcn_s_sleep(1);
-                if (++spins > kSpinLimit) { status |= kStatusInternal; break; }
-            }
-        }
-    };
-    auto chunkE = [&](int c, int j, bool refill) {
-        const int kbase = c * kChunk;
-        badq[(j + 1) & 1] = 0u;
-#pragma unroll
-        for (int u = 0; u < kChunk; u++) colq[(j + 1) & 1][u] = column(actq[j][u], badq[(j + 1) & 1], u);
-        if (refill) {
-#pragma unroll
-            for (int u = 0; u < kChunk; u++) actq[j][u] = load_act(kbase + (kAh + 1) * kChunk + u);
-        }
-        wait_room(kbase + kChunk);
-        pull(c);
-#pragma unroll
-        for (int u = 0; u < kChunk; u++) stepE(colq[j & 1][u], kbase + u, (badq[j & 1] >> u) & 1u);
-        if (NRN) __hip_atomic_store(&lds_epos[l], ep, __ATOMIC_RELAXED, __HIP_MEMORY_SCOPE_WORKGROUP);
-        if ((l & 63) == 0) wg_store_rel(&lds_prod[w], (uint32_t)(kbase + kChunk));
-    };
-    const int ngrp = nfull / kAh;
-    for (int g = 0; g < ngrp; g++) {
-#pragma unroll
-        for (int j = 0; j < kAh; j++) chunkE(g * kAh + j, j, true);
-    }
-#pragma unroll
-    for (int j = 0; j < kAh - 1; j++)
-        if (ngrp * kAh + j < nfull) chunkE(ngrp * kAh + j, j, false);
-    if (K % kChunk) {
-        const int kbase = nfull * kChunk;
-        Act ta[kChunk];
-#pragma unroll
-        for (int u = 0; u < kChunk; u++) ta[u] = load_act(kbase + u);
-        wait_room(kbase + kChunk);
-        pull(nfull);
-#pragma unroll
-        for (int u = 0; u < kChunk; u++)
-            if (kbase + u < K) {
-                uint32_t bm = 0;
-                const Col cc = column(ta[u], bm, 0);
-                stepE(cc, kbase + u, bm);
-            }
-        if ((l & 63) == 0) wg_store_rel(&lds_prod[w], (uint32_t)K);
-    }
-
-    uint32_t hist = 0;
-    for (int j = 3; j >= 0; j--) {
-        const uint32_t nb = (k2 >> (4 * j)) & 0xFu;
-        hist = (hist << 8) | ((nb & 8u) ? (nb & 7u) : 0xFFu);
-    }
-    const uint32_t qc = (uint32_t)__builtin_popcount(qv & 0x00888888u);
-    const bool own_q = !PHILOX && !IRR && !nextmode && NZ == 0;
-    if (NRN) __hip_atomic_store(&lds_epos[l], ep, __ATOMIC_RELEASE, __HIP_MEMORY_SCOPE_WORKGROUP);
-    if (!own_q && !PHILOX && !NRN) {
-        __hip_atomic_store(&lds_head[l], head_local - qc, __ATOMIC_RELEASE, __HIP_MEMORY_SCOPE_WORKGROUP);
-    }
-    if (IRR) a.irr_state[i] = c1;
-    uint32_t steps;
-    if (HASMAX) steps = cnt - c0;
-    else steps = last_reset ? (uint32_t)K - last_reset : steps0 + (uint32_t)K;
-    uint32_t *st = (uint32_t *)&a.state[i];
-    st[0] = hist; st[2] = steps | (pend ? 0x80000000u : 0u);
-    if (own_q) st[1] = (qv & 0x00777777u) | (qc << 24);
-    if ((l & 63) == 0) __hip_atomic_fetch_add(&lds_done, 1u, __ATOMIC_RELEASE, __HIP_MEMORY_SCOPE_WORKGROUP);
-    if (status) atomicOr(&a.status[i], status);
+#if MDPP_LEAN_TU_NOISE == 2
+#include "mdpp_discrete_lean_e.inc"
+#endif
 }
 
 static bool lean_launch(const DiscreteArgs &a, const DiscreteIO &io, const int nz) {
     constexpr bool kNext = MDPP_LEAN_TU_NEXT;
     const int K = io.K;
     const bool ph = a.philox != 0, irr = a.irr != 0;
+    if (!a.lean_blob) return false;
     if (io.final_obs) return false;
     const bool shape = a.autoreset == MDPP_AUTORESET_NEXT_STEP ? a.lean_next_ok != 0
                        : (nz && !ph) ? a.shape_ok_noise_np != 0
diff --git a/mdp_playground_amd/csrc/mdpp_discrete_lean_e.inc b/mdp_playground_amd/csrc/mdpp_discrete_lean_e.inc
--- /dev/null
+++ b/mdp_playground_amd/csrc/mdpp_discrete_lean_e.inc
@@ -0,0 +1,350 @@
+#if MDPP_LEAN_TU_NOISE != 2
+    const uint32_t ie = i < N ? i : N - 1u;
+    const uint4 st0 = a.state[ie];
+    auto r_act = __builtin_amdgcn_make_buffer_rsrc((void *)actions, 0, total * 4u * (uint32_t)kEN, kPRsrc);
+    const uint32_t v4 = ie * 4u * (uint32_t)kEN;
+    auto load_act = [&](int k) -> Act {
+        const uint32_t kk = (uint32_t)min(k, K - 1);
+        if constexpr (IRR) {
+            const u32x2 v = __builtin_amdgcn_raw_buffer_load_b64(r_act, v4, kk * N * 8u, MDPP_LEAN_LD_AUX);
+            return make_uint2(v.x, v.y);
+        } else {
+            return __builtin_amdgcn_raw_buffer_load_b32(r_act, v4, kk * N * 4u, MDPP_LEAN_LD_AUX);
+        }
+    };
+    constexpr int kAh = IRR ? 2 : kAhead;
+    static_assert(kAh % 2 == 0, "the column double buffer alternates with the chunk index");
+    Act act0[kChunk];
+    Act actq[kAh][kChunk];
+    auto first_loads = [&]() __attribute__((always_inline)) {
+#pragma unroll
+        for (int u = 0; u < kChunk; u++) act0[u] = load_act(u);
+#pragma unroll
+        for (int q = 0; q < kAh; q++)
+#pragma unroll
+            for (int u = 0; u < kChunk; u++) actq[q][u] = load_act((q + 1) * kChunk + u);
+    };
+    first_loads();
+    setup_shared();
+    __syncthreads();
+    if (i >= N) {
+        if ((l & 63) == 0) __hip_atomic_fetch_add(&lds_done, 1u, __ATOMIC_RELEASE, __HIP_MEMORY_SCOPE_WORKGROUP);
+        return;
+    }
+#endif
+    __builtin_amdgcn_s_setprio(kPrioE);
+    uint32_t k2, qv, cnt, steps0, last_reset = 0, badq[2] = {0u, 0u};
+    bool pend = false;
+    {
+#if MDPP_LEAN_TU_NOISE == 2
+        const uint4 st0 = a.state[i];
+#endif
+        k2 = 0;
+        for (int j = 3; j >= 0; j--) {
+            const uint32_t b = (st0.x >> (8 * j)) & 0xFFu;
+            k2 = (k2 << 4) | (b == 0xFFu ? 0u : ((b & 7u) | 8u));
+        }
+        const bool own_q = !PHILOX && !IRR && !nextmode && NZ == 0;
+        const uint32_t qc = own_q ? (st0.y >> 24) & 7u : 0u;
+        qv = own_q ? (st0.y & 0x00777777u) | (0x00888888u & ((1u << (4u * qc)) - 1u)) : 0u;
+        steps0 = st0.z & 0x7FFFFFFFu;
+        pend = nextmode && (st0.z >> 31) != 0u;
+        const uint32_t ms = (uint32_t)a.max_steps;
+        cnt = HASMAX ? (0x10000u - ms) + (steps0 < ms ? steps0 : ms) : 0u;
+    }
+    const uint32_t c0 = HASMAX ? 0x10000u - (uint32_t)a.max_steps : 0u;
+#if MDPP_LEAN_TU_NOISE == 2
+    auto r_act = __builtin_amdgcn_make_buffer_rsrc((void *)actions, 0, total * 4u * (uint32_t)kEN, kPRsrc);
+    const uint32_t v4 = i * 4u * (uint32_t)kEN;
+#endif
+    uint32_t head_local = 0;
+    S0Word s0c = 0;
+    uint32_t sel = (k2 & 7u) | kSelPad;
+    uint32_t c1 = IRR ? (a.irr_state[i] & 7u) : 0u;
+    const uint32_t A1 = IRR ? (uint32_t)a.A1 : 1u;
+
+    uint32_t pnc = 0, pnc_hi = 0;
+    uint32_t ep = 0, hh = 0, m0 = 0, m1 = 0, m2 = 0;
+    double xv = 0.0;
+    auto ensure = [&](uint32_t upto) __attribute__((always_inline)) {
+        if (__builtin_expect(__builtin_amdgcn_ballot_w64(upto > hh) != 0, 0)) {
+            uint32_t spins = 0;
+            hh = __hip_atomic_load(&lds_hhead[l], __ATOMIC_ACQUIRE, __HIP_MEMORY_SCOPE_WORKGROUP);
+            while (__builtin_amdgcn_ballot_w64(upto > hh) != 0) {
+                __hip_atomic_store(&lds_epos[l], ep, __ATOMIC_RELAXED, __HIP_MEMORY_SCOPE_WORKGROUP);
+                __builtin_amdgcn_s_sleep(1);
+                hh = __hip_atomic_load(&lds_hhead[l], __ATOMIC_ACQUIRE, __HIP_MEMORY_SCOPE_WORKGROUP);
+                if (++spins > kSpinLimit) { status |= kStatusInternal; hh = upto; break; }
+            }
+        }
+    };
+    auto fetch = [&]() __attribute__((always_inline)) {
+        ensure(ep + 3u);
+        m0 = lds_meta[ep & (uint32_t)(kXR - 1)][l];
+        m1 = lds_meta[(ep + 1u) & (uint32_t)(kXR - 1)][l];
+        m2 = lds_meta[(ep + 2u) & (uint32_t)(kXR - 1)][l];
+        if constexpr (NRX) xv = lds_x[ep & (uint32_t)(kXR - 1)][l];
+    };
+    if constexpr (NRN) fetch();
+    uint32_t enc_lo = 0, enc_hi = 0;
+    if constexpr (PN) {
+        uint64_t enc = 0;
+        for (uint32_t s_ = 0; s_ < 8u; s_++) enc |= (uint64_t)(s_ | 8u | ((uint32_t)((a.term_mask >> s_) & 1ULL) << 7)) << (8 * s_);
+        enc_lo = (uint32_t)enc; enc_hi = (uint32_t)(enc >> 32);
+    }
+    auto pull = [&](int c) {
+        if (!ar && !PN) return;
+        if (NPN && c >= 0) {
+            uint32_t spins = 0;
+            while (wg_load_acq(&lds_hprod[w]) < (uint32_t)(c + 1)) {
+                __builtin_amdgcn_s_sleep(1);
+                if (++spins > kSpinLimit) { status |= kStatusInternal; break; }
+            }
+            pnc = lds_pn2[c % kHChunksNp][0][l];
+            pnc_hi = lds_pn2[c % kHChunksNp][1][l];
+        }
+        if constexpr (NRN) return;
+        if (!PHILOX && !ar) return;
+        if constexpr (PHILOX) {
+            uint32_t spins = 0;
+            while (wg_load_acq(&lds_hprod[w]) < (uint32_t)(c + 1)) {
+                __builtin_amdgcn_s_sleep(1);
+                if (++spins > kSpinLimit) { status |= kStatusInternal; break; }
+            }
+            s0c = lds_s0[c % kHChunks][l];
+            if constexpr (PN) {
+                spins = 0;
+                while (wg_load_acq(&lds_pprod[w]) < (uint32_t)(c + 1)) {
+                    __builtin_amdgcn_s_sleep(1);
+                    if (++spins > kSpinLimit) { status |= kStatusInternal; break; }
+                }
+                pnc = lds_pn[c % kHChunks][l];
+            }
+            return;
+        }
+        const uint64_t rt = __hip_atomic_load(&lds_ring[l], __ATOMIC_ACQUIRE, __HIP_MEMORY_SCOPE_WORKGROUP);
+        const uint32_t vals = (uint32_t)rt, tail = (uint32_t)(rt >> 32);
+        const uint32_t qc = (uint32_t)__builtin_popcount(qv & 0x88888888u);
+        const uint32_t avail = tail - head_local, room = kQueueCap - qc;
+        const uint32_t take = avail < room ? avail : room;
+        const uint32_t rot = __builtin_amdgcn_alignbit(vals, vals, (head_local & 7u) * 4u);
+        const uint32_t m = (1u << (4u * take)) - 1u;
+        qv |= (rot & m) << (4u * qc);
+        head_local += take;
+        __hip_atomic_store(&lds_head[l], head_local, __ATOMIC_RELAXED, __HIP_MEMORY_SCOPE_WORKGROUP);
+    };
+#if MDPP_LEAN_TU_NOISE == 2
+    typedef typename std::conditional<IRR, uint2, int>::type Act;
+#endif
+    typedef typename std::conditional<IRR, uint4, uint2>::type Col;
+    auto column = [&](Act act, uint32_t &badm, int u) -> Col {
+        int action;
+        if constexpr (IRR) action = (int)act.x; else action = act;
+        uint32_t ua = (uint32_t)action;
+        if (__builtin_expect(__builtin_amdgcn_ballot_w64(ua >= A) != 0, 0)) {
+            ua = (uint32_t)(action + ((action >> 31) & (int)A));
+            const bool bad = ua >= A;
+            if (nextmode) badm |= bad ? (1u << u) : 0u; else status |= bad ? (uint32_t)MDPP_STATUS_BAD_ACTION : 0u;
+            ua = bad ? 0u : ua;
+        }
+        if constexpr (IRR) {
+            const int action1 = (int)act.y;
+            uint32_t ub = (uint32_t)action1;
+            if (__builtin_expect(__builtin_amdgcn_ballot_w64(ub >= A1) != 0, 0)) {
+                ub = (uint32_t)(action1 + ((action1 >> 31) & (int)A1));
+                const bool bad = ub >= A1;
+                if (nextmode) badm |= bad ? (1u << u) : 0u; else status |= bad ? (uint32_t)MDPP_STATUS_BAD_ACTION : 0u;
+                ub = bad ? 0u : ub;
+            }
+            const uint2 ca = lds_col[ua], cb = lds_col1[ub];
+            return make_uint4(ca.x, ca.y, cb.x, cb.y);
+        } else {
+            return lds_col[ua];
+        }
+    };
+    auto stepE = [&](const Col &col, int k, uint32_t badbit) {
+        uint32_t entry = __builtin_amdgcn_perm(col.y, col.x, sel);
+        if constexpr (PN && PHILOX) {
+            const uint32_t nib = (pnc >> (4 * (k % kChunk))) & 0xFu, j = nib & 7u, nx = entry & 7u;
+            const uint32_t ns = nib > 7u ? j + (j >= nx ? 1u : 0u) : nx;
+            entry = __builtin_amdgcn_perm(enc_hi, enc_lo, ns | kSelPad);
+        }
+        if constexpr (NPN) {
+            const uint32_t by = (((k % kChunk) < 4 ? pnc : pnc_hi) >> (8 * (k & 3))) & 0xFFu, nx = entry & 7u;
+            const uint32_t ns = min(by & 15u, nx) + (uint32_t)max((int)(by >> 4) - (int)nx, 0);
+            entry = __builtin_amdgcn_perm(enc_hi, enc_lo, ns | kSelPad);
+        }
+        const uint32_t k2n = (k2 << 4) | entry;
+        bool need = entry > 0x7Fu;
+        uint32_t rc = entry;
+        if (HASMAX) {
+            cnt += 1;
+            need = need || cnt >= 0x10000u;
+            rc = __builtin_amdgcn_perm(cnt, entry, 0x0c060c00u);
+        }
+        need = need && ar;
+        uint32_t rec_a = k2n;
+        if (nextmode) {
+            const bool ended = need && !pend;
+            need = pend;
+            rc = pend ? 0u : rc;
+            rec_a = pend ? 0u : k2n;
+            status |= (badbit != 0u && !pend) ? (uint32_t)MDPP_STATUS_BAD_ACTION : 0u;
+            pend = ended;
+        }
+        uint32_t s0v = PHILOX ? (uint32_t)(s0c >> (kEN * 4 * (k % kChunk))) & (IRR ? 0xFFu : 0xFu) : qv & (IRR ? 0xFFu : 0xFu);
+        if constexpr (NRN) {
+            uint32_t kind = (m0 >> 3) & 3u;
+            if (__builtin_expect(__builtin_amdgcn_ballot_w64(kind >= 2u) != 0, 0)) {
+                uint32_t guard = 0;
+                while (__builtin_amdgcn_ballot_w64(kind == 2u) != 0) {
+                    const bool red = kind == 2u;
+                    ep += red ? 2u : 0u;
+                    uint32_t o0 = m0, o1 = m1, o2 = m2;
+                    double ox = xv;
+                    fetch();
+                    if (!red) { m0 = o0; m1 = o1; m2 = o2; xv = ox; }
+                    kind = (m0 >> 3) & 3u;
+                    if (++guard > 64u) { status |= kStatusInternal; break; }
+                }
+            }
+            uint32_t cntw = kind == 0u ? 1u : 2u, ssm = kind == 0u ? m1 : m2;
+            if (kind == 3u) { cntw = m0 >> 8; ssm = m0 >> 5; }
+            if constexpr (NRX) lds_rx[k % KD][l] = xv;
+            s0v = (ssm & 7u) | 8u;
+            ep += cntw + (need ? 1u : 0u);
+            __hip_atomic_store(&lds_epos[l], ep, __ATOMIC_RELAXED, __HIP_MEMORY_SCOPE_WORKGROUP);
+            fetch();
+        }
+        if (!PHILOX && !NRN && __builtin_expect(__builtin_amdgcn_ballot_w64(need && s0v == 0u) != 0, 0)) {
+            uint32_t spins = 0;
+            while (__builtin_amdgcn_ballot_w64(need && (qv & 0xFu) == 0u) != 0) {
+                pull(-1);
+                __builtin_amdgcn_s_sleep(1);
+                if (++spins > kSpinLimit) { status |= kStatusInternal; qv |= 8u; break; }
+            }
+            s0v = qv & (IRR ? 0xFFu : 0xFu);
+        }
+        if constexpr (IRR) {
+            const uint32_t n1 = __builtin_amdgcn_perm(col.w, col.z, c1 | kSelPad);
+            c1 = need ? ((s0v >> 4) & 7u) : n1;
+            rc |= c1 << 8;
+            s0v &= 0xFu;
+        }
+        k2 = need ? s0v : k2n;
+        if (!PHILOX && !NRN) qv = need ? (qv >> (4 * kEN)) : qv;
+        if (HASMAX) cnt = need ? c0 : cnt;
+        else last_reset = need ? (uint32_t)(k + 1) : last_reset;
+        sel = (k2 & 7u) | kSelPad;
+        lds_rec[0][k % KD][l] = rec_a;
+        lds_rec[1][k % KD][l] = k2;
+        lds_rec[2][k % KD][l] = rc;
+    };
+
+#if MDPP_LEAN_TU_NOISE == 2
+    auto load_act = [&](int k) -> Act {
+        const uint32_t kk = (uint32_t)min(k, K - 1);
+        if constexpr (IRR) {
+            const u32x2 v = __builtin_amdgcn_raw_buffer_load_b64(r_act, v4, kk * N * 8u, MDPP_LEAN_LD_AUX);
+            return make_uint2(v.x, v.y);
+        } else {
+            return __builtin_amdgcn_raw_buffer_load_b32(r_act, v4, kk * N * 4u, MDPP_LEAN_LD_AUX);
+        }
+    };
+    constexpr int kAh = IRR ? 2 : kAhead;
+    static_assert(kAh % 2 == 0, "the column double buffer alternates with the chunk index");
+    Act actq[kAh][kChunk];
+    Col colq[2][kChunk];
+#pragma unroll
+    for (int u = 0; u < kChunk; u++) colq[0][u] = column(load_act(u), badq[0], u);
+#pragma unroll
+    for (int q = 0; q < kAh; q++)
+#pragma unroll
+        for (int u = 0; u < kChunk; u++) actq[q][u] = load_act((q + 1) * kChunk + u);
+
+#else
+    Col colq[2][kChunk];
+#pragma unroll
+    for (int u = 0; u < kChunk; u++) colq[0][u] = column(act0[u], badq[0], u);
+
+#endif
+    const int nfull = K / kChunk;
+    auto wait_room = [&](int kend) {
+        if (kend > KD) {
+            const uint32_t must = (uint32_t)(kend - KD);
+            uint32_t spins = 0;
+            for (;;) {
+                const uint64_t cc = __hip_atomic_load((const uint64_t *)&lds_cons[w][0], __ATOMIC_ACQUIRE,
+                                                      __HIP_MEMORY_SCOPE_WORKGROUP);
+                uint32_t have = min((uint32_t)cc, (uint32_t)(cc >> 32));
+                if (rows) {
+#pragma unroll
+                    for (int j = 0; j < kBlock / 64; j++) have = min(have, wg_load_acq(&lds_cons[j][1]));
+                }
+                if (have >= must) break;
+                __builtin_amdgcn_s_sleep(1);
+                if (++spins > kSpinLimit) { status |= kStatusInternal; break; }
+            }
+        }
+    };
+    auto chunkE = [&](int c, int j, bool refill) {
+        const int kbase = c * kChunk;
+        badq[(j + 1) & 1] = 0u;
+#pragma unroll
+        for (int u = 0; u < kChunk; u++) colq[(j + 1) & 1][u] = column(actq[j][u], badq[(j + 1) & 1], u);
+        if (refill) {
+#pragma unroll
+            for (int u = 0; u < kChunk; u++) actq[j][u] = load_act(kbase + (kAh + 1) * kChunk + u);
+        }
+        wait_room(kbase + kChunk);
+        pull(c);
+#pragma unroll
+        for (int u = 0; u < kChunk; u++) stepE(colq[j & 1][u], kbase + u, (badq[j & 1] >> u) & 1u);
+        if (NRN) __hip_atomic_store(&lds_epos[l], ep, __ATOMIC_RELAXED, __HIP_MEMORY_SCOPE_WORKGROUP);
+        if ((l & 63) == 0) wg_store_rel(&lds_prod[w], (uint32_t)(kbase + kChunk));
+    };
+    const int ngrp = nfull / kAh;
+    for (int g = 0; g < ngrp; g++) {
+#pragma unroll
+        for (int j = 0; j < kAh; j++) chunkE(g * kAh + j, j, true);
+    }
+#pragma unroll
+    for (int j = 0; j < kAh - 1; j++)
+        if (ngrp * kAh + j < nfull) chunkE(ngrp * kAh + j, j, false);
+    if (K % kChunk) {
+        const int kbase = nfull * kChunk;
+        Act ta[kChunk];
+#pragma unroll
+        for (int u = 0; u < kChunk; u++) ta[u] = load_act(kbase + u);
+        wait_room(kbase + kChunk);
+        pull(nfull);
+#pragma unroll
+        for (int u = 0; u < kChunk; u++)
+            if (kbase + u < K) {
+                uint32_t bm = 0;
+                const Col cc = column(ta[u], bm, 0);
+                stepE(cc, kbase + u, bm);
+            }
+        if ((l & 63) == 0) wg_store_rel(&lds_prod[w], (uint32_t)K);
+    }
+
+    uint32_t hist = 0;
+    for (int j = 3; j >= 0; j--) {
+        const uint32_t nb = (k2 >> (4 * j)) & 0xFu;
+        hist = (hist << 8) | ((nb & 8u) ? (nb & 7u) : 0xFFu);
+    }
+    const uint32_t qc = (uint32_t)__builtin_popcount(qv & 0x00888888u);
+    const bool own_q = !PHILOX && !IRR && !nextmode && NZ == 0;
+    if (NRN) __hip_atomic_store(&lds_epos[l], ep, __ATOMIC_RELEASE, __HIP_MEMORY_SCOPE_WORKGROUP);
+    if (!own_q && !PHILOX && !NRN) {
+        __hip_atomic_store(&lds_head[l], head_local - qc, __ATOMIC_RELEASE, __HIP_MEMORY_SCOPE_WORKGROUP);
+    }
+    if (IRR) a.irr_state[i] = c1;
+    uint32_t steps;
+    if (HASMAX) steps = cnt - c0;
+    else steps = last_reset ? (uint32_t)K - last_reset : steps0 + (uint32_t)K;
+    uint32_t *st = (uint32_t *)&a.state[i];
+    st[0] = hist; st[2] = steps | (pend ? 0x80000000u : 0u);
+    if (own_q) st[1] = (qv & 0x00777777u) | (qc << 24);
+    if ((l & 63) == 0) __hip_atomic_fetch_add(&lds_done, 1u, __ATOMIC_RELEASE, __HIP_MEMORY_SCOPE_WORKGROUP);
+    if (status) atomicOr(&a.status[i], status);
diff --git a/mdp_playground_amd/csrc/mdpp_internal.hpp b/mdp_playground_amd/csrc/mdpp_internal.hpp
--- a/mdp_playground_amd/csrc/mdpp_internal.hpp
+++ b/mdp_playground_amd/csrc/mdpp_internal.hpp
@@ -99,7 +99,11 @@
     uint64_t init_thr[16];
     float rsel[4];
     uint64_t minv_lo, minv_hi;
-};
+    const uint4 *lean_blob;
+};
+
+constexpr uint32_t kLeanTabV = 0, kLeanTabCol = 512, kLeanTabT = 520, kLeanTabCol1 = 524, kLeanTabT1 = 532, kLeanTabRsel = 536,
+                   kLeanTabUnits = 600;
 
 #ifndef MDPP_S1_REPLICAS
 #define MDPP_S1_REPLICAS 1
@@ -260,6 +264,7 @@
     mdpp::DiscreteArgs dargs;
     mdpp::Step1Args s1args;
     void *d_s1_blob;
+    void *d_lean_blob;
     void *d_policy_thr;
     uint64_t policy_seed;
     bool policy_ready;
@@ -439,6 +444,7 @@
 bool launch_discrete_quiet(const DiscreteArgs &a, const DiscreteIO &io);
 bool launch_discrete_pipe(const DiscreteArgs &a, const DiscreteIO &io);
 bool launch_discrete_lean(const DiscreteArgs &a, const DiscreteIO &io);
+hipError_t launch_lean_build_tables(const DiscreteArgs &a, void *blob, hipStream_t s);
 bool launch_continuous_fast(const ContinuousArgs &a, const ContinuousIO &io);
 bool launch_continuous_step1(const ContinuousArgs &a, const ContinuousIO &io);
 bool launch_continuous_line(const ContinuousArgs &a, const ContinuousIO &io);
```
